# lzhangbj/ASVA

Hardware: AMD Instinct MI355X
Metric: UNet denoising steps/sec, 12x256x256 bf16, CFG on (higher is better)
Workload: dtype bf16; 1 GPU; BASELINE configs[1]: AVSync15 shape, 1 clip(s) per GPU per forward, 12x256x256 (latent 12x32x32), SD1.5-shaped AudioUNet3D 1.17B params random-init, CFG batch 2 (audio guidance 4.0), DDIM-50 schedule, step = UNet forward + guidance + scheduler update; clips_per_gpu=1, unet_batch=2, frames=12, launch=hipGraph replay, parallelism=dp1 (independent clips)

## Files before the change

### asva_amd/_lib.py

```python
from __future__ import annotations

import ctypes as C
import os

import torch

from . import precision as P

_HERE = os.path.dirname(os.path.abspath(__file__))
LIB_PATH = os.environ.get("AVSD_LIB_PATH") or os.path.join(_HERE, "libavsd_hip.so")
LIB_PATHS = {"bf16": LIB_PATH, "fp16": os.environ.get("AVSD_LIB_PATH_F16") or os.path.join(_HERE, "libavsd_hip_f16.so")}

c_void_p, c_int, c_float, c_int64 = C.c_void_p, C.c_int, C.c_float, C.c_int64


class GemmDesc(C.Structure):

    _fields_ = [
        ("A", c_void_p), ("A2", c_void_p), ("W", c_void_p), ("out", c_void_p),
        ("bias", c_void_p), ("rowvec", c_void_p), ("res1", c_void_p), ("res2", c_void_p),
        ("M", C.c_int32), ("N", C.c_int32), ("K", C.c_int32),
        ("lda", C.c_int32), ("lda2", C.c_int32), ("k_split", C.c_int32), ("ldw", C.c_int32),
        ("ldc", C.c_int32), ("ldr1", C.c_int32), ("ldr2", C.c_int32),
        ("rows_per_vec", C.c_int32), ("ldv", C.c_int32),
        ("alpha", C.c_float),
        ("mode", C.c_int32), ("flags", C.c_int32), ("batch", C.c_int32),
        ("batch_stride_a", C.c_int64), ("batch_stride_w", C.c_int64), ("batch_stride_out", C.c_int64),
        ("hw", C.c_int32), ("frames", C.c_int32), ("cseg", C.c_int32),
        ("hs", C.c_int32), ("ws", C.c_int32), ("ho", C.c_int32), ("wo", C.c_int32),
        ("cin", C.c_int32), ("stride", C.c_int32), ("ups", C.c_int32), ("pad", C.c_int32),
        ("tile", C.c_int32),
        ("split_k", C.c_int32), ("splitk_ws", c_void_p),
        ("rowstats", c_void_p), ("ln_stats", c_void_p), ("ln_colsum", c_void_p), ("ln_nblk", C.c_int32), ("ln_eps", C.c_float),
        ("out_master", c_void_p), ("ldm", C.c_int32), ("raster_g", C.c_int32),
        ("a_lo", C.c_int64), ("a2_lo", C.c_int64), ("w_lo", C.c_int64), ("out_lo", C.c_int64), ("res1_lo", C.c_int64),
        ("res2_lo", C.c_int64),
        ("stats_pos", c_void_p), ("ln_rowvec", c_void_p), ("pos_hw", C.c_int32), ("pos_frames", C.c_int32),
    ]


class XAttnDesc(C.Structure):

    _fields_ = [
        ("h", c_void_p), ("ldh", C.c_int32), ("res_f32", C.c_int32),
        ("res", c_void_p), ("ldres", C.c_int32),
        ("M", C.c_int32), ("C", C.c_int32), ("heads", C.c_int32), ("L", C.c_int32),
        ("ln_stats", c_void_p), ("ln_eps", C.c_float), ("scale", C.c_float),
        ("wq", c_void_p), ("ldwq", C.c_int32), ("lk", C.c_int32),
        ("q_colsum", c_void_p), ("q_bias", c_void_p),
        ("k", c_void_p), ("vt", c_void_p),
        ("lk_pad", C.c_int32), ("q_per_kv", C.c_int32),
        ("wo", c_void_p), ("ldwo", C.c_int32), ("ldo", C.c_int32),
        ("o_bias", c_void_p), ("out", c_void_p),
        ("out_master", c_void_p), ("ldm", C.c_int32), ("reserved0", C.c_int32),
        ("rowstats", c_void_p),
        ("stats_pos", c_void_p), ("pos_hw", C.c_int32), ("pos_frames", C.c_int32),
    ]


SIGNATURES = {
    "avsd_abi_version": (c_int, []),
    "avsd_precision": (C.c_char_p, []),
    "avsd_last_error": (C.c_char_p, []),
    "avsd_device_info": (c_int, [C.c_char_p, c_int, C.POINTER(c_int)]),
    "avsd_gemm_bf16": (c_int, [C.POINTER(GemmDesc), c_void_p]),
    "avsd_sizeof_gemm_desc": (c_int, []),
    "avsd_cross_attention_block": (c_int, [C.POINTER(XAttnDesc), c_void_p]),
    "avsd_gemm_conv3r_supported": (c_int, [c_int, c_int, c_int, c_int]),
    "avsd_gemm_conv3r2d_supported": (c_int, [c_int, c_int, c_int, c_int]),
    "avsd_cross_attention_block_supported": (c_int, [c_int, c_int, c_int]),
    "avsd_sizeof_xattn_desc": (c_int, []),
    "avsd_linear_small_m": (c_int, [c_void_p, c_void_p, c_void_p, c_void_p, c_int, c_int, c_int, c_int, c_int, c_int, c_void_p]),
    "avsd_groupnorm_stats": (c_int, [c_void_p, c_int, c_int, c_void_p, c_int, c_int, c_int, c_int, c_int, c_void_p, c_int, c_void_p]),
    "avsd_groupnorm_apply": (c_int, [c_void_p, c_int, c_int, c_void_p, c_int, c_int, c_int, c_int, c_int, c_void_p, c_void_p, c_float,
                                     c_void_p, c_int, c_int, c_void_p, c_int, c_void_p]),
    "avsd_ln_fold": (c_int, [c_void_p, c_int, c_int, c_void_p, c_void_p]),
    "avsd_groupnorm_fused_supported": (c_int, [c_int, c_int, c_int, c_int, c_int, c_int]),
    "avsd_groupnorm_fused": (c_int, [c_void_p, c_int, c_int, c_void_p, c_int, c_int, c_int, c_int, c_int, c_void_p, c_void_p, c_float,
                                     c_int, c_void_p, c_int, c_void_p]),
    "avsd_groupnorm_nchunks": (c_int, [c_int, c_int, c_int]),
    "avsd_groupnorm_scratch_floats": (c_int, [c_int, c_int, c_int, c_int]),
    "avsd_layernorm": (c_int, [c_void_p, c_int, c_void_p, c_int, c_int, c_int, c_void_p, c_void_p, c_float, c_void_p, c_int, c_int, c_void_p]),
    "avsd_softmax_rows": (c_int, [c_void_p, c_int, c_void_p, c_int, c_int, c_int, c_void_p]),
    "avsd_attention": (c_int, [c_void_p, c_int, c_void_p, c_int, c_void_p, c_int, c_void_p, c_int, c_int, c_int, c_int, c_int,
                               c_int, c_int, c_int, c_void_p, c_int, c_float, c_void_p]),
    "avsd_attention_fp8": (c_int, [c_void_p, c_int, c_void_p, c_int, c_void_p, c_int, c_void_p, c_int, c_int, c_int, c_int, c_int,
                                   c_int, c_int, c_int, c_void_p, c_int, c_float, c_float, c_float, c_float, c_void_p]),
    "avsd_temporal_attention": (c_int, [c_void_p, c_int, c_void_p, c_int, c_int, c_int, c_int, c_int, c_int, c_float, c_void_p]),
    "avsd_ncfhw_to_rows": (c_int, [c_void_p, c_void_p, c_int, c_int, c_int, c_int, c_int, c_int, c_float, c_void_p]),
    "avsd_rows_to_ncfhw": (c_int, [c_void_p, c_int, c_void_p, c_int, c_int, c_int, c_int, c_void_p]),
    "avsd_timestep_embedding": (c_int, [c_void_p, c_void_p, c_int, c_int, c_void_p]),
    "avsd_guided_step": (c_int, [c_void_p, c_int, c_float, c_float, c_void_p, c_int, c_float, C.POINTER(C.c_int32), C.POINTER(C.c_float),
                                 c_int, c_void_p, c_void_p, c_float, c_float, c_int, c_int, c_int, c_int, c_void_p]),
    "avsd_guided_multistep": (c_int, [c_void_p, c_int, c_float, c_float, c_void_p, c_int, C.POINTER(C.c_int32), C.POINTER(C.c_float),
                                      c_int, c_void_p, c_void_p, c_float, c_float, c_float, c_float, c_int, c_int, c_int, c_int, c_void_p]),
    "avsd_vae_postprocess":(c_int, [c_void_p, c_int, c_void_p, c_int, c_int, c_void_p]),
    "avsd_vae_postprocess_u8": (c_int, [c_void_p, c_int, c_void_p, c_int, c_int, c_void_p]),
    "avsd_kaldi_fbank": (c_int, [c_void_p, c_int, c_int, C.c_int64, c_void_p, c_void_p, c_int, c_int, c_int, c_int, c_float, c_int,
                                 c_void_p, c_int, c_float, c_float, c_void_p]),
    "avsd_patchify": (c_int, [c_void_p, c_void_p, c_int, c_int, c_int, c_int, c_int, c_int, c_int, c_void_p]),
    "avsd_vit_tokens": (c_int, [c_void_p, c_void_p, c_void_p, c_void_p, c_int, c_int, c_int, c_int, c_void_p]),
    "avsd_copy": (c_int, [c_void_p, c_void_p, c_int64, c_int, c_void_p]),
    "avsd_xattn_pack_kv": (c_int, [c_void_p, c_int, c_int, c_int, c_void_p, c_int, c_int, c_void_p, c_void_p, c_int, c_void_p]),
    "avsd_linear_small_m_x2": (c_int, [c_void_p, c_void_p, c_int64, c_void_p, c_void_p, c_int, c_int, c_int, c_int, c_int, c_int, c_void_p]),
    "avsd_groupnorm_stats_x2": (c_int, [c_void_p, c_int, c_int, c_int64, c_void_p, c_int, c_int, c_int64, c_int, c_int, c_int, c_void_p,
                                        c_int, c_void_p]),
    "avsd_groupnorm_apply_x2": (c_int, [c_void_p, c_int, c_int, c_int64, c_void_p, c_int, c_int, c_int64, c_int, c_int, c_int, c_void_p,
                                        c_void_p, c_float, c_void_p, c_int, c_int, c_void_p, c_int, c_int64, c_void_p]),
    "avsd_groupnorm_fused_x2": (c_int, [c_void_p, c_int, c_int, c_int64, c_void_p, c_int, c_int, c_int64, c_int, c_int, c_int, c_void_p,
                                        c_void_p, c_float, c_int, c_void_p, c_int, c_int64, c_void_p]),
    "avsd_layernorm_x2": (c_int, [c_void_p, c_int, c_int64, c_void_p, c_int, c_int64, c_int, c_int, c_void_p, c_void_p, c_float, c_void_p,
                                  c_int, c_int, c_void_p]),
    "avsd_attention_x2": (c_int, [c_void_p, c_int, c_int64, c_void_p, c_int, c_int64, c_void_p, c_int, c_int64, c_void_p, c_int, c_int64,
                                  c_int, c_int, c_int, c_int, c_int, c_int, c_int, c_void_p, c_int, c_float, c_void_p]),
    "avsd_temporal_attention_x2": (c_int, [c_void_p, c_int, c_int64, c_void_p, c_int, c_int64, c_int, c_int, c_int, c_int, c_int, c_float,
                                           c_void_p]),
    "avsd_softmax_rows_x2": (c_int, [c_void_p, c_int, c_void_p, c_int, c_int64, c_int, c_int, c_void_p]),
    "avsd_ncfhw_to_rows_x2": (c_int, [c_void_p, c_void_p, c_int64, c_int, c_int, c_int, c_int, c_int, c_int, c_float, c_void_p]),
# ... 82 lines not shown
```

### asva_amd/build.py

```python
from __future__ import annotations

import os
import subprocess
import sys
from concurrent.futures import ThreadPoolExecutor

HERE = os.path.dirname(os.path.abspath(__file__))
CSRC = os.path.join(HERE, "csrc")
OBJ = os.path.join(CSRC, "_obj")
LIB = os.path.join(HERE, "libavsd_hip.so")
VARIANTS = {"bf16": ("", LIB, []), "fp16": ("_f16", os.path.join(HERE, "libavsd_hip_f16.so"), ["-DAVSD_F16=1"])}
SOURCES = ["lib.hip", "attention.hip", "attention_x2.hip", "gemm_f32.hip", "gemm4.hip", "nstream.hip", "conv3r.hip", "norm.hip", "groupnorm_fused.hip", "elementwise.hip", "audio.hip", "xattn.hip", "attention_fp8.hip", "avsync.hip", "clip_text.hip", "imagebind_eval.hip", "plan.hip"]
GEMM_UNITS = 7
HEADERS = [os.path.join(CSRC, "avsd_common.h"), os.path.join(CSRC, "gemm_common.h"), os.path.join(CSRC, "gemm4_loops.inc"),
           os.path.join(HERE, "..", "include", "avsd.h")]
FLAGS = ["--offload-arch=gfx950", "-O3", "-std=c++17", "-fPIC", "-Wall", "-Wno-unused-function"]


PLAN_HOST = os.path.join(HERE, "plan_host")


def _hipcc() -> str:
    for cand in (os.environ.get("HIPCC"), "/opt/rocm/bin/hipcc", "hipcc"):
        if cand and (os.path.isabs(cand) and os.path.exists(cand) or not os.path.isabs(cand)):
            return cand
    raise RuntimeError("hipcc not found")


def _stale(target: str, deps: list[str]) -> bool:
    if not os.path.exists(target):
        return True
    t = os.path.getmtime(target)
    return any(os.path.getmtime(d) > t for d in deps)


def build(verbose: bool = False, force: bool = False, variants=("bf16", "fp16")) -> str:
    hipcc = _hipcc()
    jobs = []
    links = []
    for var in variants:
        suffix, lib, defs = VARIANTS[var]
        objdir = OBJ + suffix
        os.makedirs(objdir, exist_ok=True)
        objs = []
        stale = False
        for src in SOURCES:
            s = os.path.join(CSRC, src)
            o = os.path.join(objdir, src.replace(".hip", ".o"))
            objs.append(o)
            if force or _stale(o, [s] + HEADERS):
                jobs.append([hipcc, *FLAGS, *defs, "-c", s, "-o", o])
                stale = True
        gsrc = os.path.join(CSRC, "gemm.hip")
        for u in range(GEMM_UNITS):
            o = os.path.join(objdir, f"gemm_tu{u}.o")
            objs.append(o)
            if force or _stale(o, [gsrc] + HEADERS):
                jobs.insert(0, [hipcc, *FLAGS, *defs, f"-DAVSD_GEMM_TU={u}", "-c", gsrc, "-o", o])
                stale = True
        links.append((lib, objs, stale))

    def run(cmd):
        if verbose:
            print(" ".join(cmd), flush=True)
        r = subprocess.run(cmd, capture_output=True, text=True)
        if r.returncode != 0:
            raise RuntimeError(f"hipcc failed: {' '.join(cmd)}\n{r.stdout}\n{r.stderr}")
# ... 17 lines not shown
```

### asva_amd/csrc/gemm.hip

```cpp
#include "avsd_common.h"
#include "gemm_common.h"

namespace {

constexpr int LDS_STRIDE = BK + 8;

struct RowInfo {
  int64_t o0, o1, o2;
  int hb, wb;
  bool valid;
};

template <int MODE>
__device__ __forceinline__ RowInfo make_row(const avsd_gemm_desc& p, int m) {
  RowInfo r;
  r.valid = m < p.M;
  r.o0 = r.o1 = r.o2 = 0;
  r.hb = r.wb = 0;
  if (!r.valid) return r;
  if (MODE == AVSD_GEMM_PLAIN) {
    r.o0 = (int64_t)m * p.lda;
    r.o1 = (int64_t)m * p.lda2;
  } else if (MODE == AVSD_GEMM_TMIX) {
    const int f = (m / p.hw) % p.frames;
    r.o0 = (int64_t)(m - f * p.hw) * p.lda;
    r.o1 = (int64_t)(f > 0 ? m - p.hw : m) * p.lda;
    r.o2 = (int64_t)m * p.lda;
  } else {
    const int per = p.ho * p.wo;
    const int n = m / per;
    const int rem = m - n * per;
    const int oh = rem / p.wo;
    const int ow = rem - oh * p.wo;
    r.o0 = n;
    r.hb = oh * p.stride - p.pad;
    r.wb = ow * p.stride - p.pad;
  }
  return r;
}

template <int MODE>
__device__ __forceinline__ uint4 load_a(const avsd_gemm_desc& p, const h16_t* A, const h16_t* A2,
                                        const RowInfo& r, int k0) {
  uint4 z = make_uint4(0, 0, 0, 0);
  if (!r.valid || k0 >= p.K) return z;
  const h16_t* ptr;
  if (MODE == AVSD_GEMM_PLAIN) {
    ptr = (k0 < p.k_split) ? (A + r.o0 + k0) : (A2 + r.o1 + (k0 - p.k_split));
  } else if (MODE == AVSD_GEMM_TMIX) {
    const int seg = k0 / p.cseg;
    const int kk = k0 - seg * p.cseg;
    const int64_t o = r.o2 + (seg == 0 ? r.o0 - r.o2 : 0) + (seg == 1 ? r.o1 - r.o2 : 0);
// ... 160 lines not shown
  r.o0 = r.o1 = r.o2 = r.hb = r.wb = 0;
  if (!r.valid) return r;
  if (MODE == AVSD_GEMM_PLAIN) {
    r.o0 = m * p.lda;
    r.o1 = m * p.lda2;
  } else if (MODE == AVSD_GEMM_TMIX) {
    const int f = (m / p.hw) % p.frames;
    r.o0 = (m - f * p.hw) * p.lda;
    r.o1 = (f > 0 ? m - p.hw : m) * p.lda;
    r.o2 = m * p.lda;
  } else {
    const int per = p.ho * p.wo;
    const int n = m / per;
    const int rem = m - n * per;
    const int oh = rem / p.wo;
    r.o0 = n;
    r.hb = oh * p.stride - p.pad;
    r.wb = (rem - oh * p.wo) * p.stride - p.pad;
  }
  return r;
}

template <int MODE>
__device__ __forceinline__ unsigned a_voffset(const avsd_gemm_desc& p, const RowInfo32& r, int k0) {
  if (!r.valid || k0 >= p.K) return OOB;
  if (MODE == AVSD_GEMM_PLAIN) {
    return (unsigned)((k0 < p.k_split) ? (r.o0 + k0) : (r.o1 + (k0 - p.k_split))) * 2u;
  } else if (MODE == AVSD_GEMM_TMIX) {
    const int seg = k0 / p.cseg;
    const int kk = k0 - seg * p.cseg;
    const int o = r.o2 + (seg == 0 ? r.o0 - r.o2 : 0) + (seg == 1 ? r.o1 - r.o2 : 0);
    return (unsigned)(o + kk) * 2u;
  } else {
    const int tap = k0 / p.cin;
    const int c = k0 - tap * p.cin;
    const int kh = tap / 3;
    const int kw = tap - kh * 3;
    const int hi = r.hb + kh;
    const int wi = r.wb + kw;
    if (tap >= 9 || hi < 0 || hi >= (p.hs << p.ups) || wi < 0 || wi >= (p.ws << p.ups)) return OOB;
    return (unsigned)(((r.o0 * p.hs + (hi >> p.ups)) * p.ws + (wi >> p.ups)) * p.lda + c) * 2u;
  }
}

constexpr int gemm2_min_waves(int bm, int bn, int stages, bool x2, int waves) {
  const int lds = stages * (bm + bn) * 128 * (x2 ? 2 : 1);
  const int wgs = (160 * 1024) / lds < 1 ? 1 : (160 * 1024) / lds;
  const int w = (wgs * waves + 3) / 4;
  return w > 3 ? 3 : w;
}
constexpr int MODE_SUBPIX = 3;
template <int BM, int BN, int WM, int WN, int STAGES, int MODE, int LW = 0, bool X2 = false, int EX = EPI_PLAIN>
__global__ __launch_bounds__(64 * (WM * WN + LW), gemm2_min_waves(BM, BN, STAGES, X2, WM * WN + LW)) void gemm2_kernel(const avsd_gemm_desc p) {
  extern __shared__ __attribute__((aligned(1024))) unsigned char smem2[];
  constexpr int NC = WM * WN;
  constexpr int NWAVES = LW > 0 ? LW : NC;
  constexpr int A_BYTES = BM * 128;
  constexpr int W_BYTES = BN * 128;
  constexpr int PLANE_BYTES = A_BYTES + W_BYTES;
  constexpr int STAGE_BYTES = PLANE_BYTES * (X2 ? 2 : 1);
  constexpr int PA = (BM / 8) / NWAVES;
  constexpr int PW = (BN / 8) / NWAVES;
  static_assert(PA * NWAVES * 8 == BM && PW * NWAVES * 8 == BN, "tile rows must split evenly into 1-KiB pieces per wave");
  constexpr int LPT = (PA + PW) * (X2 ? 2 : 1);
  static_assert((STAGES - 2) * LPT < 64, "vmcnt is a 6-bit counter");
  constexpr int FM = BM / WM / 32;
  constexpr int FN = BN / WN / 32;

  const int tid = threadIdx.x;
  const int lane = tid & 63;
  const int wave_all = __builtin_amdgcn_readfirstlane(tid >> 6);
  const bool is_loader = LW == 0 || wave_all >= NC;
  const int wave = LW == 0 ? wave_all : (wave_all >= NC ? wave_all - NC : 0);
  const int wm = wave_all % WM;
  const int wn = (wave_all / WM) % WN;

  const int ntm = (p.M + BM - 1) / BM;
  const int ntn = (p.N + BN - 1) / BN;
  const int nwg = ntm * ntn;
  const int nsplit = p.split_k > 1 ? p.split_k : 1;
  int wg, ksplit;
  {
    const int total = nwg * nsplit;
    const int bid = blockIdx.y * gridDim.x + blockIdx.x;
    const int q = total >> 3, r = total & 7;
    const int xcd = bid & 7, idx = bid >> 3;
    const int c = (xcd < r ? xcd * (q + 1) : r * (q + 1) + (xcd - r) * q) + idx;
    wg = c / nsplit;
    ksplit = c - wg * nsplit;
  }
  int tm, tn;
  tile_of_item(wg, ntm, ntn, (p.flags & AVSD_GEMM_XCD_N) != 0, p.raster_g, tm, tn);
  const int64_t bz = blockIdx.z;
  const int nk_all = (p.K + BK - 1) / BK;
  const int per_split = (nk_all + nsplit - 1) / nsplit;
  const int kt0 = ksplit * per_split;
  const int kt1 = min(nk_all, kt0 + per_split);

  const h16_t* Ab = reinterpret_cast<const h16_t*>(p.A) + bz * p.batch_stride_a;
  const h16_t* A2b = p.A2 ? reinterpret_cast<const h16_t*>(p.A2) + bz * p.batch_stride_a : Ab;
  const h16_t* Wb = reinterpret_cast<const h16_t*>(p.W) + bz * p.batch_stride_w;
  const __amdgpu_buffer_rsrc_t rsA = __builtin_amdgcn_make_buffer_rsrc((void*)Ab, 0, 0x7fffffff, 0x00020000);
  const __amdgpu_buffer_rsrc_t rsA2 = __builtin_amdgcn_make_buffer_rsrc((void*)A2b, 0, 0x7fffffff, 0x00020000);
  const __amdgpu_buffer_rsrc_t rsW = __builtin_amdgcn_make_buffer_rsrc((void*)Wb, 0, 0x7fffffff, 0x00020000);
  const __amdgpu_buffer_rsrc_t rsAr = __builtin_amdgcn_make_buffer_rsrc((void*)(Ab + (X2 ? p.a_lo : 0)), 0, 0x7fffffff, 0x00020000);
  const __amdgpu_buffer_rsrc_t rsA2r = __builtin_amdgcn_make_buffer_rsrc((void*)(A2b + (X2 ? (p.A2 ? p.a2_lo : p.a_lo) : 0)), 0, 0x7fffffff, 0x00020000);
  const __amdgpu_buffer_rsrc_t rsWr = __builtin_amdgcn_make_buffer_rsrc((void*)(Wb + (X2 ? p.w_lo : 0)), 0, 0x7fffffff, 0x00020000);

  int ro0[PA], ro1[PA], ro2[PA], rhb[PA], rwb[PA], kca[PA];
  bool rvalid[PA];
#pragma unroll
  for (int j = 0; j < PA; ++j) {
    const int L = (wave + j * NWAVES) * 4 + (lane >> 4);
    const int x = (lane & 15) ^ (L & 15);
    const RowInfo32 r = make_row32<MODE>(p, tm * BM + 2 * L + (x >> 3));
    ro0[j] = r.o0; ro1[j] = r.o1; ro2[j] = r.o2; rhb[j] = r.hb; rwb[j] = r.wb; rvalid[j] = r.valid;
    kca[j] = (x & 7) * 8;
  }
  int wo[PW], kcw[PW];
  bool wv[PW];
#pragma unroll
  for (int j = 0; j < PW; ++j) {
    const int L = (wave + j * NWAVES) * 4 + (lane >> 4);
    const int x = (lane & 15) ^ (L & 15);
    const int n = tn * BN + 2 * L + (x >> 3);
    wv[j] = n < p.N;
    kcw[j] = (x & 7) * 8;
    wo[j] = n * p.ldw + kcw[j];
  }

  const bool fast = (MODE == AVSD_GEMM_PLAIN) || (MODE == AVSD_GEMM_TMIX && p.cseg % BK == 0) ||
                    ((MODE == AVSD_GEMM_CONV3 || MODE == MODE_SUBPIX) && p.cin % BK == 0);
  const int nk_slice = max(kt1 - kt0, 0);
  const int krot = ((p.flags & AVSD_GEMM_KROT) && nk_slice > 1 && ntm > 1) ? (int)(((long long)tm * nk_slice) / ntm) : 0;
  constexpr bool subpix = MODE == MODE_SUBPIX;
  constexpr int KS = subpix ? 2 : 3;
  const int ush = subpix ? 0 : p.ups;
  const int sub_par = subpix ? (tn * BN) / (p.N >> 2) : 0;
  const int sub_dy = sub_par >> 1, sub_dx = sub_par & 1;
  int i_kbase = 0;
  int i_c0 = 0;
  int i_kh = 0, i_kw = 0, i_seg = 0;
  bool i_second = false;
  auto seek = [&](int kbase) {
    i_kbase = kbase;
    if (MODE == AVSD_GEMM_PLAIN) {
      i_c0 = i_kbase;
      i_second = p.A2 != nullptr && i_kbase >= p.k_split;
    } else if (MODE == AVSD_GEMM_TMIX) {
      i_seg = i_kbase / p.cseg;
      i_c0 = i_kbase - i_seg * p.cseg;
    } else {
      const int tap = i_kbase / p.cin;
      i_c0 = i_kbase - tap * p.cin;
      i_kh = tap / KS;
      i_kw = tap - i_kh * KS;
    }
  };
  seek((kt0 + krot) * BK);
  const int hin = p.hs << ush, win = p.ws << ush;
  int abase[PA];
  bool aok[PA];

  auto rebase = [&]() {
#pragma unroll
    for (int j = 0; j < PA; ++j) {
      if (MODE == AVSD_GEMM_PLAIN) {
        abase[j] = (i_second ? ro1[j] - p.k_split : ro0[j]) + kca[j];
        aok[j] = rvalid[j];
      } else if (MODE == AVSD_GEMM_TMIX) {
        const int o = ro2[j] + (i_seg == 0 ? ro0[j] - ro2[j] : 0) + (i_seg == 1 ? ro1[j] - ro2[j] : 0);
        abase[j] = o + kca[j];
        aok[j] = rvalid[j] && i_seg < 3;
      } else {
        const int hi = rhb[j] + i_kh + sub_dy;
        const int wi = rwb[j] + i_kw + sub_dx;
        aok[j] = rvalid[j] && i_kh < KS && (unsigned)hi < (unsigned)hin && (unsigned)wi < (unsigned)win;
        abase[j] = ((ro0[j] * p.hs + (hi >> ush)) * p.ws + (wi >> ush)) * p.lda + kca[j];
      }
    }
  };
  rebase();

  auto issue = [&](int stage) {
    unsigned char* sb = smem2 + stage * STAGE_BYTES;
    const int kbase = i_kbase;
#pragma unroll
    for (int j = 0; j < PA; ++j) {
      unsigned vo;
      if (!fast) {
        RowInfo32 r;
        r.o0 = ro0[j]; r.o1 = ro1[j]; r.o2 = ro2[j]; r.hb = rhb[j]; r.wb = rwb[j]; r.valid = rvalid[j];
        vo = a_voffset<MODE>(p, r, kbase + kca[j]);
      } else {
        const bool ok = aok[j] && (kbase + kca[j] < p.K);
        vo = ok ? (unsigned)(abase[j] + i_c0) * 2u : OOB;
      }
      lds_ptr_t dst = (lds_ptr_t)(sb + (wave + j * NWAVES) * 1024);
      if (i_second) __builtin_amdgcn_raw_ptr_buffer_load_lds(rsA2, dst, 16, (int)vo, 0, 0, 0);
      else __builtin_amdgcn_raw_ptr_buffer_load_lds(rsA, dst, 16, (int)vo, 0, 0, 0);
      if constexpr (X2) {
        lds_ptr_t dr = (lds_ptr_t)(sb + PLANE_BYTES + (wave + j * NWAVES) * 1024);
        if (i_second) __builtin_amdgcn_raw_ptr_buffer_load_lds(rsA2r, dr, 16, (int)vo, 0, 0, 0);
        else __builtin_amdgcn_raw_ptr_buffer_load_lds(rsAr, dr, 16, (int)vo, 0, 0, 0);
      }
    }
#pragma unroll
    for (int j = 0; j < PW; ++j) {
      const unsigned vo = (wv[j] && kbase + kcw[j] < p.K) ? (unsigned)(wo[j] + kbase) * 2u : OOB;
      lds_ptr_t dst = (lds_ptr_t)(sb + A_BYTES + (wave + j * NWAVES) * 1024);
      __builtin_amdgcn_raw_ptr_buffer_load_lds(rsW, dst, 16, (int)vo, 0, 0, 0);
      if constexpr (X2) {
        lds_ptr_t dr = (lds_ptr_t)(sb + PLANE_BYTES + A_BYTES + (wave + j * NWAVES) * 1024);
        __builtin_amdgcn_raw_ptr_buffer_load_lds(rsWr, dr, 16, (int)vo, 0, 0, 0);
      }
    }
    i_kbase += BK;
    if (krot != 0 && i_kbase >= kt1 * BK) {
      seek(kt0 * BK);
      rebase();
    } else
    if (MODE == AVSD_GEMM_PLAIN) {
      i_c0 = i_kbase;
      if (!i_second && i_kbase >= p.k_split && i_kbase < p.K) { i_second = true; rebase(); }
    } else if (MODE == AVSD_GEMM_TMIX) {
      i_c0 += BK;
      if (i_c0 >= p.cseg) { i_c0 = 0; ++i_seg; rebase(); }
    } else {
      i_c0 += BK;
      if (i_c0 >= p.cin) {
        i_c0 = 0;
        if (++i_kw == KS) { i_kw = 0; ++i_kh; }
        rebase();
      }
    }
  };

  f32x16 acc[FN][FM];
#pragma unroll
  for (int a = 0; a < FN; ++a)
#pragma unroll
    for (int b = 0; b < FM; ++b)
#pragma unroll
      for (int r = 0; r < 16; ++r) acc[a][b][r] = 0.f;

  int a_line[FM], a_sw[FM], a_hi[FM];
#pragma unroll
  for (int b = 0; b < FM; ++b) {
    const int r = wm * (BM / WM) + b * 32 + (lane & 31);
    a_line[b] = (r >> 1) * 256;
    a_sw[b] = (r >> 1) & 15;
    a_hi[b] = (r & 1) << 3;
  }
  int w_line[FN], w_sw[FN], w_hi[FN];
#pragma unroll
  for (int a = 0; a < FN; ++a) {
    const int r = wn * (BN / WN) + a * 32 + (lane & 31);
    w_line[a] = (r >> 1) * 256;
    w_sw[a] = (r >> 1) & 15;
    w_hi[a] = (r & 1) << 3;
  }
  const int chalf = lane >> 5;

  const int nk = max(kt1 - kt0, 0);
  auto wait_stage = [&](int kt) {
    wait_tiles_ahead<STAGES - 2, LPT>(nk - 1 - kt);
  };
  if (is_loader) {
#pragma unroll
    for (int s = 0; s < STAGES - 1; ++s)
      if (s < nk) issue(s);
  }
  float pre_ln[2 * FM] = {};
  const bool pre = (p.flags & AVSD_GEMM_LNFUSE) != 0 && !(LW > 0 && is_loader);
  if (pre) {
#pragma unroll
    for (int b = 0; b < FM; ++b) {
      const int m = tm * BM + wm * (BM / WM) + b * 32 + (lane & 31);
      pre_ln[2 * b] = 1.f; pre_ln[2 * b + 1] = 0.f;
      if (m < p.M) ln_row_stats(p, m, bz, pre_ln[2 * b], pre_ln[2 * b + 1]);
    }
  }
  if (LW > 0 && is_loader) {
    for (int kt = 0; kt < nk; ++kt) {
      wait_stage(kt);
      __builtin_amdgcn_s_barrier();
      if (kt + STAGES - 1 < nk) issue((kt + STAGES - 1) % STAGES);
    }
    return;
  }

  for (int kt = 0; kt < nk; ++kt) {
    if (LW == 0) wait_stage(kt);
    __builtin_amdgcn_s_barrier();
    if (LW == 0 && kt + STAGES - 1 < nk) issue((kt + STAGES - 1) % STAGES);

    const unsigned char* sA = smem2 + (kt % STAGES) * STAGE_BYTES;
    const unsigned char* sW = sA + A_BYTES;
#pragma unroll
    for (int ks = 0; ks < BK / 16; ++ks) {
      const int c = ks * 2 + chalf;
      h16x8 xf[FM], wf[FN];
#pragma unroll
      for (int b = 0; b < FM; ++b)
        xf[b] = *reinterpret_cast<const h16x8*>(sA + a_line[b] + (((a_hi[b] | c) ^ a_sw[b]) << 4));
#pragma unroll
      for (int a = 0; a < FN; ++a)
        wf[a] = *reinterpret_cast<const h16x8*>(sW + w_line[a] + (((w_hi[a] | c) ^ w_sw[a]) << 4));
      if constexpr (X2) {
        h16x8 xr[FM], wr[FN];
#pragma unroll
        for (int b = 0; b < FM; ++b)
          xr[b] = *reinterpret_cast<const h16x8*>(sA + PLANE_BYTES + a_line[b] + (((a_hi[b] | c) ^ a_sw[b]) << 4));
#pragma unroll
        for (int a = 0; a < FN; ++a)
          wr[a] = *reinterpret_cast<const h16x8*>(sW + PLANE_BYTES + w_line[a] + (((w_hi[a] | c) ^ w_sw[a]) << 4));
        __builtin_amdgcn_s_setprio(1);
#pragma unroll
        for (int a = 0; a < FN; ++a)
#pragma unroll
          for (int b = 0; b < FM; ++b) {
            acc[a][b] = mfma32x32x16(wr[a], xf[b], acc[a][b], 0, 0, 0);
            acc[a][b] = mfma32x32x16(wf[a], xr[b], acc[a][b], 0, 0, 0);
            acc[a][b] = mfma32x32x16(wf[a], xf[b], acc[a][b], 0, 0, 0);
          }
        __builtin_amdgcn_s_setprio(0);
      } else {
      __builtin_amdgcn_s_setprio(1);
#pragma unroll
      for (int a = 0; a < FN; ++a)
#pragma unroll
        for (int b = 0; b < FM; ++b)
          acc[a][b] = mfma32x32x16(wf[a], xf[b], acc[a][b], 0, 0, 0);
      __builtin_amdgcn_s_setprio(0);
      }
    }
  }

  if (p.split_k > 1) {
    float* ws = p.splitk_ws + (int64_t)ksplit * p.M * p.N;
    const int hsel = (lane >> 5) * 4;
#pragma unroll
    for (int b = 0; b < FM; ++b) {
      const int m = tm * BM + wm * (BM / WM) + b * 32 + (lane & 31);
      if (m >= p.M) continue;
#pragma unroll
      for (int a = 0; a < FN; ++a)
#pragma unroll
        for (int q = 0; q < 4; ++q) {
          const int n = tn * BN + wn * (BN / WN) + a * 32 + 8 * q + hsel;
          if (n < p.N)
            *reinterpret_cast<float4*>(ws + (int64_t)m * p.N + n) =
                make_float4(acc[a][b][4 * q], acc[a][b][4 * q + 1], acc[a][b][4 * q + 2], acc[a][b][4 * q + 3]);
        }
    }
    if (p.split_k != 0x7fffffff) return;
#pragma unroll
    for (int a = 0; a < FN; ++a)
#pragma unroll
      for (int b = 0; b < FM; ++b)
#pragma unroll
        for (int r = 0; r < 16; ++r) acc[a][b][r] = 0.f;
    for (int sl = 0; sl < nsplit; ++sl) {
      const float* slab = p.splitk_ws + (int64_t)sl * p.M * p.N;
#pragma unroll
      for (int b = 0; b < FM; ++b) {
        const int m = min(tm * BM + wm * (BM / WM) + b * 32 + (lane & 31), p.M - 1);
#pragma unroll
        for (int a = 0; a < FN; ++a)
#pragma unroll
          for (int q = 0; q < 4; ++q) {
            const int n = min(tn * BN + wn * (BN / WN) + a * 32 + 8 * q + hsel, p.N - 4);
            const float4 v = *reinterpret_cast<const float4*>(slab + (int64_t)m * p.N + n);
            acc[a][b][4 * q] += v.x; acc[a][b][4 * q + 1] += v.y; acc[a][b][4 * q + 2] += v.z; acc[a][b][4 * q + 3] += v.w;
          }
      }
    }
  }
  if constexpr (subpix) {
    if constexpr (X2) epilogue_x2<FN, FM, true>(p, acc, tm * BM + wm * (BM / WM), tn * BN + wn * (BN / WN), lane, bz, pre_ln, pre);
    else epilogue_each<FN, FM, (64 * (WM * WN + LW) > 512), EPI_SHUF>(p, acc, tm * BM + wm * (BM / WM), tn * BN + wn * (BN / WN), lane, bz, pre_ln, pre);
  } else if constexpr (X2) epilogue_x2<FN, FM>(p, acc, tm * BM + wm * (BM / WM), tn * BN + wn * (BN / WN), lane, bz, pre_ln, pre);
  else if constexpr (EX == EPI_REST) {
    if constexpr (FN * FM >= 10) epilogue_each<FN, FM, (64 * (WM * WN + LW) > 512), EPI_REST>(p, acc, tm * BM + wm * (BM / WM), tn * BN + wn * (BN / WN), lane, bz, pre_ln, pre);
    else epilogue<FN, FM, (64 * (WM * WN + LW) > 512), EPI_REST>(p, acc, tm * BM + wm * (BM / WM), tn * BN + wn * (BN / WN), lane, bz, pre_ln, pre);
  } else if constexpr (FN * FM >= 10)
    epilogue_each<FN, FM, (64 * (WM * WN + LW) > 512)>(p, acc, tm * BM + wm * (BM / WM), tn * BN + wn * (BN / WN), lane, bz, pre_ln, pre);
  else epilogue<FN, FM, (64 * (WM * WN + LW) > 512)>(p, acc, tm * BM + wm * (BM / WM), tn * BN + wn * (BN / WN), lane, bz, pre_ln, pre);
}

template <int S, bool EXTRA = false>
__global__ __launch_bounds__(256) void splitk_reduce_kernel(const avsd_gemm_desc p) {
  const int nq = p.N / 4;
  const int64_t total = (int64_t)p.M * nq;
  const h16_t* R1 = reinterpret_cast<const h16_t*>(p.res1);
  const h16_t* R2 = reinterpret_cast<const h16_t*>(p.res2);
  const bool x2 = (p.flags & AVSD_GEMM_X2) != 0;
  const bool out_rest = EXTRA && (p.flags & AVSD_GEMM_OUT_REST) != 0;
  for (int64_t i = blockIdx.x * (int64_t)blockDim.x + threadIdx.x; i < total; i += (int64_t)gridDim.x * blockDim.x) {
    const int m = (int)(i / nq);
    const int n = (int)(i - (int64_t)m * nq) * 4;
    float4 acc = make_float4(0.f, 0.f, 0.f, 0.f);
    float4 pre_bias = make_float4(0.f, 0.f, 0.f, 0.f), pre_vec = pre_bias, pre_r1f = pre_bias, pre_r2f = pre_bias;
    uint2 pre_r1 = make_uint2(0, 0), pre_r1lo = pre_r1, pre_r2 = pre_r1, pre_r2lo = pre_r1;
    if (p.bias) pre_bias = *reinterpret_cast<const float4*>(p.bias + n);
    if (p.rowvec) pre_vec = *reinterpret_cast<const float4*>(p.rowvec + (int64_t)(m / p.rows_per_vec) * p.ldv + n);
    if (R1) {
      if (p.flags & AVSD_GEMM_RES1_F32) {
        pre_r1f = *reinterpret_cast<const float4*>(reinterpret_cast<const float*>(p.res1) + (int64_t)m * p.ldr1 + n);
      } else {
        pre_r1 = *reinterpret_cast<const uint2*>(R1 + (int64_t)m * p.ldr1 + n);
        if (x2) pre_r1lo = *reinterpret_cast<const uint2*>(R1 + p.res1_lo + (int64_t)m * p.ldr1 + n);
      }
    }
    if (R2) {
      if (p.flags & AVSD_GEMM_RES2_F32) {
        pre_r2f = *reinterpret_cast<const float4*>(reinterpret_cast<const float*>(p.res2) + (int64_t)m * p.ldr2 + n);
      } else {
        pre_r2 = *reinterpret_cast<const uint2*>(R2 + (int64_t)m * p.ldr2 + n);
        if (x2) pre_r2lo = *reinterpret_cast<const uint2*>(R2 + p.res2_lo + (int64_t)m * p.ldr2 + n);
      }
    }
    if constexpr (S > 0) {
      float4 sv[S];
#pragma unroll
      for (int s = 0; s < S; ++s) sv[s] = *reinterpret_cast<const float4*>(p.splitk_ws + ((int64_t)s * p.M + m) * p.N + n);
#pragma unroll
      for (int s = 0; s < S; ++s) { acc.x += sv[s].x; acc.y += sv[s].y; acc.z += sv[s].z; acc.w += sv[s].w; }
    } else {
      for (int s = 0; s < p.split_k; ++s) {
        const float4 v = *reinterpret_cast<const float4*>(p.splitk_ws + ((int64_t)s * p.M + m) * p.N + n);
        acc.x += v.x; acc.y += v.y; acc.z += v.z; acc.w += v.w;
      }
    }
    float v[4] = {p.alpha * acc.x, p.alpha * acc.y, p.alpha * acc.z, p.alpha * acc.w};
    if (p.flags & AVSD_GEMM_LNFUSE) {
      const float2* st = reinterpret_cast<const float2*>(p.ln_stats) + (int64_t)m * p.ln_nblk;
      float sm = 0.f, sq = 0.f;
      for (int j = 0; j < p.ln_nblk; ++j) { const float2 t = st[j]; sm += t.x; sq += t.y; }
      const float inv_k = 1.0f / (float)p.K;
      const float mean = sm * inv_k;
// ... 65 lines not shown
          sm += __shfl_xor(sm, off, 64);
          sq += __shfl_xor(sq, off, 64);
        }
        if ((threadIdx.x & 7) == 0)
          reinterpret_cast<float2*>(p.rowstats)[(int64_t)m * (p.N >> 5) + (n >> 5)] = make_float2(sm, sq);
      }
    }
  }
}

template <int BM, int BN, int WM, int WN, int STAGES, int MODE, int LW = 0, bool X2 = false, int EX = EPI_PLAIN>
int launch2(const avsd_gemm_desc& d, hipStream_t s) {
  constexpr size_t lds = (size_t)STAGES * (BM + BN) * 128 * (X2 ? 2 : 1);
  static_assert(lds <= 160 * 1024, "tile does not fit the 160 KB of LDS");
  if (MODE == MODE_SUBPIX && (d.N / 4) % BN != 0) {
    avsd_set_error("gemm/conv3: ups = 2 needs whole column tiles per output-pixel parity: cout (%d) %% %d != 0 for this tile", d.N / 4, BN);
    return AVSD_EINVAL;
  }
  static bool attr_set = false;
  if (!attr_set) {
    hipError_t e = hipFuncSetAttribute(reinterpret_cast<const void*>(&gemm2_kernel<BM, BN, WM, WN, STAGES, MODE, LW, X2, EX>),
                                       hipFuncAttributeMaxDynamicSharedMemorySize, (int)lds);
    if (e != hipSuccess) {
      avsd_set_error("gemm2: hipFuncSetAttribute(%zu B LDS): %s", lds, hipGetErrorString(e));
      return AVSD_ELAUNCH;
    }
    attr_set = true;
  }
  const int ntm = (d.M + BM - 1) / BM, ntn = (d.N + BN - 1) / BN;
  const int nsplit = d.split_k > 1 ? d.split_k : 1;
  dim3 grid((unsigned)(ntm * ntn), (unsigned)nsplit, (unsigned)d.batch);
  hipLaunchKernelGGL((gemm2_kernel<BM, BN, WM, WN, STAGES, MODE, LW, X2, EX>), grid, dim3(64 * (WM * WN + LW)), lds, s, d);
  AVSD_CHECK_LAUNCH("gemm2 launch");
  if (nsplit > 1) {
    const int64_t total = (int64_t)d.M * (d.N / 4);
    int64_t g = (total + 255) / 256;
    if (g > 2048) g = 2048;
    if (MODE == MODE_SUBPIX || (d.flags & AVSD_GEMM_OUT_REST)) {
      hipLaunchKernelGGL((splitk_reduce_kernel<0, true>), dim3((unsigned)g), dim3(256), 0, s, d);
    } else
    switch (nsplit) {
      case 2: hipLaunchKernelGGL(splitk_reduce_kernel<2>, dim3((unsigned)g), dim3(256), 0, s, d); break;
      case 4: hipLaunchKernelGGL(splitk_reduce_kernel<4>, dim3((unsigned)g), dim3(256), 0, s, d); break;
      case 8: hipLaunchKernelGGL(splitk_reduce_kernel<8>, dim3((unsigned)g), dim3(256), 0, s, d); break;
      case 3: hipLaunchKernelGGL(splitk_reduce_kernel<3>, dim3((unsigned)g), dim3(256), 0, s, d); break;
      case 5: hipLaunchKernelGGL(splitk_reduce_kernel<5>, dim3((unsigned)g), dim3(256), 0, s, d); break;
      default: hipLaunchKernelGGL(splitk_reduce_kernel<0>, dim3((unsigned)g), dim3(256), 0, s, d); break;
    }
    AVSD_CHECK_LAUNCH("gemm split-K reduce launch");
  }
  return AVSD_OK;
}

template <int MODE, int EX = EPI_PLAIN>
int dispatch_tile(const avsd_gemm_desc& d, int tile, hipStream_t s) {
  switch (tile) {
    case 1: return launch<128, 128, MODE, EX>(d, s);
    case 2: return launch<128, 64, MODE, EX>(d, s);
    case 3: return launch<64, 64, MODE, EX>(d, s);
    case 4: return launch2<128, 64, 2, 2, 3, MODE, 0, false, EX>(d, s);
    case 6: return launch2<128, 128, 2, 4, 3, MODE, 0, false, EX>(d, s);
    case 7: return launch2<64, 64, 2, 2, 4, MODE, 0, false, EX>(d, s);
    case 9: return launch2<256, 128, 4, 2, 3, MODE, 0, false, EX>(d, s);
    case 11: return launch2<128, 128, 2, 2, 2, MODE, 0, false, EX>(d, s);
    case 12: return launch2<128, 64, 2, 2, 2, MODE, 0, false, EX>(d, s);
    case 13: return launch2<64, 64, 2, 2, 2, MODE, 0, false, EX>(d, s);
    case 14: return launch2<256, 128, 4, 2, 2, MODE, 0, false, EX>(d, s);
    case 17: return launch2<128, 320, 4, 2, 2, MODE, 0, false, EX>(d, s);
    case 19: return launch2<256, 320, 4, 2, 2, MODE, 0, false, EX>(d, s);
    case 20: return launch2<256, 128, 4, 2, 3, MODE, 4, false, EX>(d, s);
    case 24: return launch2<128, 64, 2, 2, 3, MODE, 2, false, EX>(d, s);
    case 25: return launch2<64, 64, 2, 2, 4, MODE, 2, false, EX>(d, s);
    case 30: return launch2<128, 128, 2, 4, 4, MODE, 0, false, EX>(d, s);
    case 31: return launch2<128, 256, 2, 4, 3, MODE, 0, false, EX>(d, s);
    case AVSD_GEMM_TILE_256x160_8W: return launch2<256, 160, 8, 1, 3, MODE, 4, false, EX>(d, s);
    default:
      avsd_set_error("gemm: tile id %d is not built (gemm.hip dispatch_tile)", tile);
      return AVSD_EINVAL;
  }
}

template <int MODE>
int dispatch_tile_x2(const avsd_gemm_desc& d, int tile, hipStream_t s) {
  switch (tile) {
    case 7: return launch2<64, 64, 2, 2, 4, MODE, 0, true>(d, s);
    case 11: return launch2<128, 128, 2, 2, 2, MODE, 0, true>(d, s);
    case 13: return launch2<64, 64, 2, 2, 2, MODE, 0, true>(d, s);
    case 24: return launch2<128, 64, 2, 2, 3, MODE, 2, true>(d, s);
    case 25: return launch2<64, 64, 2, 2, 4, MODE, 2, true>(d, s);
    case 34: return launch2<128, 160, 4, 1, 2, MODE, 0, true>(d, s);
    case 35: return launch2<256, 64, 4, 2, 2, MODE, 0, true>(d, s);
    case 36: return launch2<128, 192, 2, 2, 2, MODE, 0, true>(d, s);
    default:
      avsd_set_error("gemm: AVSD_GEMM_X2 runs on tiles 7, 11, 13, 24, 25, 34, 35, 36 (got %d)", tile);
      return AVSD_EINVAL;
  }
}

int pick_tile(int M, int N, int batch) {
  static int num_cu = 0;
  if (num_cu == 0) {
    hipDeviceProp_t prop;
    int dev = 0;
    if (hipGetDevice(&dev) == hipSuccess && hipGetDeviceProperties(&prop, dev) == hipSuccess)
      num_cu = prop.multiProcessorCount;
    if (num_cu <= 0) num_cu = 256;
  }
  const int bm[3] = {128, 128, 64}, bn[3] = {128, 64, 64};
  const double eff[3] = {1.0, 0.85, 0.62};
  const int slots[3] = {2 * num_cu, 3 * num_cu, 4 * num_cu};
  int best = 3;
  double best_cost = 1e300;
  for (int t = 0; t < 3; ++t) {
    const long blocks = (long)((M + bm[t] - 1) / bm[t]) * ((N + bn[t] - 1) / bn[t]) * batch;
    const long waves = (blocks + slots[t] - 1) / slots[t];
    const double cost = (double)waves * bm[t] * bn[t] / eff[t] * slots[t];
    if (cost < best_cost) { best_cost = cost; best = t + 1; }
  }
  return best;
}

}

int avsd_gemm_dispatch_plain(const avsd_gemm_desc& d, int tile, hipStream_t s);
int avsd_gemm_dispatch_tmix(const avsd_gemm_desc& d, int tile, hipStream_t s);
int avsd_gemm_dispatch_conv3(const avsd_gemm_desc& d, int tile, hipStream_t s);
#ifdef AVSD_F16
#define AVSD_DISPATCH_TILE(MODE) ((d.flags & AVSD_GEMM_OUT_REST) ? dispatch_tile<MODE, EPI_REST>(d, tile, s) : dispatch_tile<MODE>(d, tile, s))
#else
#define AVSD_DISPATCH_TILE(MODE) dispatch_tile<MODE>(d, tile, s)
#endif
#if !defined(AVSD_GEMM_TU) || AVSD_GEMM_TU == 0
int avsd_gemm_dispatch_plain(const avsd_gemm_desc& d, int tile, hipStream_t s) { return AVSD_DISPATCH_TILE(AVSD_GEMM_PLAIN); }
#endif
#if !defined(AVSD_GEMM_TU) || AVSD_GEMM_TU == 1
int avsd_gemm_dispatch_tmix(const avsd_gemm_desc& d, int tile, hipStream_t s) { return AVSD_DISPATCH_TILE(AVSD_GEMM_TMIX); }
#endif
#if !defined(AVSD_GEMM_TU) || AVSD_GEMM_TU == 2
int avsd_gemm_dispatch_conv3(const avsd_gemm_desc& d, int tile, hipStream_t s) { return AVSD_DISPATCH_TILE(AVSD_GEMM_CONV3); }
#endif
int avsd_gemm_dispatch_subpix(const avsd_gemm_desc& d, int tile, hipStream_t s);
int avsd_gemm_dispatch_x2_subpix(const avsd_gemm_desc& d, int tile, hipStream_t s);
#if !defined(AVSD_GEMM_TU) || AVSD_GEMM_TU == 6
int avsd_gemm_dispatch_subpix(const avsd_gemm_desc& d, int tile, hipStream_t s) {
  switch (tile) {
    case 4: return launch2<128, 64, 2, 2, 3, MODE_SUBPIX>(d, s);
    case 6: return launch2<128, 128, 2, 4, 3, MODE_SUBPIX>(d, s);
    case 9: return launch2<256, 128, 4, 2, 3, MODE_SUBPIX>(d, s);
    case 11: return launch2<128, 128, 2, 2, 2, MODE_SUBPIX>(d, s);
    case 13: return launch2<64, 64, 2, 2, 2, MODE_SUBPIX>(d, s);
    case 17: return launch2<128, 320, 4, 2, 2, MODE_SUBPIX>(d, s);
    case 20: return launch2<256, 128, 4, 2, 3, MODE_SUBPIX, 4>(d, s);
    case 24: return launch2<128, 64, 2, 2, 3, MODE_SUBPIX, 2>(d, s);
    case 25: return launch2<64, 64, 2, 2, 4, MODE_SUBPIX, 2>(d, s);
    case 30: return launch2<128, 128, 2, 4, 4, MODE_SUBPIX>(d, s);
    case AVSD_GEMM_TILE_256x160_8W: return launch2<256, 160, 8, 1, 3, MODE_SUBPIX, 4>(d, s);
    default:
      avsd_set_error("gemm/conv3: ups = 2 runs on tiles 4, 6, 9, 11, 13, 17, 20, 24, 25, 30, 38 (got %d)", tile);
      return AVSD_EINVAL;
  }
}
int avsd_gemm_dispatch_x2_subpix(const avsd_gemm_desc& d, int tile, hipStream_t s) {
  switch (tile) {
    case 7: return launch2<64, 64, 2, 2, 4, MODE_SUBPIX, 0, true>(d, s);
    case 11: return launch2<128, 128, 2, 2, 2, MODE_SUBPIX, 0, true>(d, s);
    case 13: return launch2<64, 64, 2, 2, 2, MODE_SUBPIX, 0, true>(d, s);
    case 24: return launch2<128, 64, 2, 2, 3, MODE_SUBPIX, 2, true>(d, s);
    case 25: return launch2<64, 64, 2, 2, 4, MODE_SUBPIX, 2, true>(d, s);
    case 34: return launch2<128, 160, 4, 1, 2, MODE_SUBPIX, 0, true>(d, s);
    case 35: return launch2<256, 64, 4, 2, 2, MODE_SUBPIX, 0, true>(d, s);
    default:
      avsd_set_error("gemm/conv3: ups = 2 with AVSD_GEMM_X2 runs on tiles 7, 11, 13, 24, 25, 34, 35 (got %d)", tile);
      return AVSD_EINVAL;
  }
}
#endif

int avsd_gemm_dispatch_x2_plain(const avsd_gemm_desc& d, int tile, hipStream_t s);
int avsd_gemm_dispatch_x2_tmix(const avsd_gemm_desc& d, int tile, hipStream_t s);
int avsd_gemm_dispatch_x2_conv3(const avsd_gemm_desc& d, int tile, hipStream_t s);
#if !defined(AVSD_GEMM_TU) || AVSD_GEMM_TU == 4
int avsd_gemm_dispatch_x2_plain(const avsd_gemm_desc& d, int tile, hipStream_t s) { return dispatch_tile_x2<AVSD_GEMM_PLAIN>(d, tile, s); }
int avsd_gemm_dispatch_x2_tmix(const avsd_gemm_desc& d, int tile, hipStream_t s) { return dispatch_tile_x2<AVSD_GEMM_TMIX>(d, tile, s); }
#endif
#if !defined(AVSD_GEMM_TU) || AVSD_GEMM_TU == 5
int avsd_gemm_dispatch_x2_conv3(const avsd_gemm_desc& d, int tile, hipStream_t s) { return dispatch_tile_x2<AVSD_GEMM_CONV3>(d, tile, s); }
#endif

#if !defined(AVSD_GEMM_TU) || AVSD_GEMM_TU == 3
int avsd_gemm_dispatch_conv3r(const avsd_gemm_desc& d, hipStream_t s);
int avsd_gemm_dispatch_asm(const avsd_gemm_desc& d, hipStream_t s);
int avsd_gemm_dispatch_nstream(const avsd_gemm_desc& d, hipStream_t s);

int avsd_gemm_splitk_reduce(const avsd_gemm_desc& d, hipStream_t s) {
  const int64_t total = (int64_t)d.M * (d.N / 4);
  int64_t g = (total + 255) / 256;
  if (g > 2048) g = 2048;
  if (d.flags & AVSD_GEMM_OUT_REST) {
    hipLaunchKernelGGL((splitk_reduce_kernel<0, true>), dim3((unsigned)g), dim3(256), 0, s, d);
  } else
  switch (d.split_k) {
    case 2: hipLaunchKernelGGL(splitk_reduce_kernel<2>, dim3((unsigned)g), dim3(256), 0, s, d); break;
    case 4: hipLaunchKernelGGL(splitk_reduce_kernel<4>, dim3((unsigned)g), dim3(256), 0, s, d); break;
    case 8: hipLaunchKernelGGL(splitk_reduce_kernel<8>, dim3((unsigned)g), dim3(256), 0, s, d); break;
    case 3: hipLaunchKernelGGL(splitk_reduce_kernel<3>, dim3((unsigned)g), dim3(256), 0, s, d); break;
    case 5: hipLaunchKernelGGL(splitk_reduce_kernel<5>, dim3((unsigned)g), dim3(256), 0, s, d); break;
    case 10: hipLaunchKernelGGL(splitk_reduce_kernel<10>, dim3((unsigned)g), dim3(256), 0, s, d); break;
    default: hipLaunchKernelGGL(splitk_reduce_kernel<0>, dim3((unsigned)g), dim3(256), 0, s, d); break;
  }
  AVSD_CHECK_LAUNCH("gemm split-K reduce launch");
  return AVSD_OK;
}

extern "C" int avsd_gemm_bf16(const avsd_gemm_desc* dp, void* stream) {
  AVSD_REQUIRE(dp != nullptr, "gemm: null descriptor");
  avsd_gemm_desc d = *dp;
  AVSD_REQUIRE(d.A && d.W && d.out, "gemm: A, W and out must be non-null");
  AVSD_REQUIRE(d.M > 0 && d.N > 0 && d.K > 0, "gemm: M,N,K must be positive (got %d,%d,%d)", d.M, d.N, d.K);
  AVSD_REQUIRE(!(d.flags & AVSD_GEMM_W_FRAG) || d.tile == AVSD_GEMM_TILE_NSTREAM, "gemm: fragment-ordered W (AVSD_GEMM_W_FRAG) is read by tile %d only (got %d)", AVSD_GEMM_TILE_NSTREAM, d.tile);
  if (d.flags & AVSD_GEMM_W_FRAG) d.ldw = d.K;
  AVSD_REQUIRE(d.K % 8 == 0 && d.ldw % 8 == 0 && d.ldw >= d.K, "gemm: K (%d) and ldw (%d) must be multiples of 8, ldw >= K", d.K, d.ldw);
  AVSD_REQUIRE(d.N % 4 == 0 && d.ldc % 4 == 0, "gemm: N (%d) and ldc (%d) must be multiples of 4", d.N, d.ldc);
  AVSD_REQUIRE(d.lda % 8 == 0, "gemm: lda (%d) must be a multiple of 8", d.lda);
  if (d.batch <= 0) d.batch = 1;
  AVSD_REQUIRE(d.raster_g >= 0 && d.raster_g <= 64, "gemm: raster_g (%d) must be 0 (library default) .. 64", d.raster_g);
  if (d.flags & AVSD_GEMM_GEGLU) AVSD_REQUIRE(d.N % 32 == 0, "gemm: GEGLU needs N %% 32 == 0 (got %d)", d.N);
  AVSD_REQUIRE(!((d.flags & AVSD_GEMM_GEGLU) && (d.flags & AVSD_GEMM_GELU)), "gemm: GEGLU and GELU are exclusive");
  if (d.flags & AVSD_GEMM_ROWSTATS) {
    AVSD_REQUIRE(d.rowstats, "gemm: ROWSTATS without a rowstats buffer");
    AVSD_REQUIRE(!(d.flags & (AVSD_GEMM_GEGLU | AVSD_GEMM_OUT_F32)) && d.N % 32 == 0 && d.ldc % 8 == 0 &&
                     (!d.res1 || d.ldr1 % 8 == 0) && (!d.res2 || d.ldr2 % 8 == 0),
                 "gemm: ROWSTATS needs bf16 output, N %% 32 == 0 and 16-byte-aligned rows");
  }
  if (d.flags & AVSD_GEMM_LNFUSE) {
    AVSD_REQUIRE(d.ln_stats && d.ln_colsum && d.ln_nblk > 0 && d.mode == AVSD_GEMM_PLAIN && !d.A2,
                 "gemm: LNFUSE needs ln_stats, ln_colsum, ln_nblk and a single-source PLAIN operand");
    AVSD_REQUIRE(d.ln_nblk * 32 == d.K || d.ln_nblk == 1, "gemm: LNFUSE statistics are K / 32 pairs per row or one pre-folded pair (got %d for K = %d)", d.ln_nblk, d.K);
    AVSD_REQUIRE(d.batch == 1 || d.batch_stride_a % d.lda == 0, "gemm: LNFUSE batch stride must be whole rows");
  }
  if (d.stats_pos || d.ln_rowvec) {
    AVSD_REQUIRE(d.pos_hw > 0 && d.pos_frames > 0 && d.batch == 1 && !(d.flags & AVSD_GEMM_X2),
                 "gemm: stats_pos / ln_rowvec need pos_hw > 0, pos_frames > 0, batch 1 and no AVSD_GEMM_X2 (got hw %d, frames %d)", d.pos_hw, d.pos_frames);
    AVSD_REQUIRE(!d.stats_pos || (d.flags & AVSD_GEMM_ROWSTATS), "gemm: stats_pos without AVSD_GEMM_ROWSTATS");
    AVSD_REQUIRE(!d.ln_rowvec || (d.flags & AVSD_GEMM_LNFUSE), "gemm: ln_rowvec without AVSD_GEMM_LNFUSE");
  }
  if (d.res1) AVSD_REQUIRE(d.ldr1 % 4 == 0, "gemm: ldr1 must be a multiple of 4");
  if (d.res2) AVSD_REQUIRE(d.ldr2 % 4 == 0, "gemm: ldr2 must be a multiple of 4");
  if (d.out_master) AVSD_REQUIRE(d.ldm % 4 == 0 && d.ldm >= ((d.mode == AVSD_GEMM_CONV3 && d.ups == 2) ? d.N / 4 : d.N) && !(d.flags & AVSD_GEMM_GEGLU),
                                 "gemm: out_master needs ldm %% 4 == 0, ldm >= N (ups = 2: cout) and no GEGLU");
  if (d.rowvec) AVSD_REQUIRE(d.rows_per_vec > 0 && d.ldv % 4 == 0, "gemm: rowvec needs rows_per_vec > 0 and ldv %% 4 == 0");
  if (d.flags & AVSD_GEMM_OUT_REST) {
#ifndef AVSD_F16
    AVSD_REQUIRE(d.mode == AVSD_GEMM_CONV3 && d.ups == 2,
                 "gemm: OUT_REST is compiled into the IEEE-half build only (libavsd_hip_f16.so: the per-layer precision plan is fp16 storage)");
#endif
    AVSD_REQUIRE(!(d.flags & (AVSD_GEMM_X2 | AVSD_GEMM_OUT_F32 | AVSD_GEMM_GEGLU)) && d.out_lo != 0 && (d.out_lo & 7) == 0 && d.batch == 1 &&
                     d.tile != AVSD_GEMM_TILE_NSTREAM && !(d.tile >= AVSD_GEMM_TILE_CONV3R_FIRST && d.tile <= AVSD_GEMM_TILE_CONV3R2D_LAST),
                 "gemm: OUT_REST is for one-pass 16-bit outputs (no X2 / OUT_F32 / GEGLU / batch, not on tiles 40..54 / 70) and needs out_lo %% 8 == 0, != 0");
  }
  if (d.mode == AVSD_GEMM_PLAIN) {
    if (!d.A2) d.k_split = d.K;
    AVSD_REQUIRE(d.k_split % 8 == 0 && d.k_split <= d.K, "gemm: k_split (%d) must be a multiple of 8 and <= K", d.k_split);
    if (d.A2) AVSD_REQUIRE(d.lda2 % 8 == 0, "gemm: lda2 must be a multiple of 8");
  } else if (d.mode == AVSD_GEMM_TMIX) {
    AVSD_REQUIRE(d.cseg > 0 && d.cseg % 8 == 0 && d.K == 3 * d.cseg, "gemm/tmix: K (%d) must equal 3*cseg (%d)", d.K, d.cseg);
    AVSD_REQUIRE(d.hw > 0 && d.frames > 0 && d.M % (d.hw * d.frames) == 0, "gemm/tmix: M (%d) must be a multiple of frames*hw (%d*%d)", d.M, d.frames, d.hw);
  } else if (d.mode == AVSD_GEMM_CONV3) {
    AVSD_REQUIRE(d.stride == 1 || d.stride == 2, "gemm/conv3: stride must be 1 or 2");
    if (d.ups == 2) {
      AVSD_REQUIRE(d.cin > 0 && d.cin % 64 == 0 && d.K == 4 * d.cin, "gemm/conv3: ups = 2 needs K (%d) == 4*cin (%d), cin %% 64 == 0", d.K, d.cin);
      AVSD_REQUIRE(d.stride == 1 && d.pad == 1 && d.hs > 0 && d.ws > 0 && d.ho == d.hs && d.wo == d.ws && d.M % (d.hs * d.ws) == 0,
                   "gemm/conv3: ups = 2 needs stride 1, pad 1, (ho, wo) = (hs, ws) and whole images");
      AVSD_REQUIRE(d.N % 4 == 0 && (d.N / 4) % 64 == 0 && d.ldc >= d.N / 4, "gemm/conv3: ups = 2 needs N = 4 * cout, cout %% 64 == 0, ldc >= cout");
      AVSD_REQUIRE(!d.A2 && !d.res1 && !d.res2 && !d.rowvec && !(d.flags & (AVSD_GEMM_GEGLU | AVSD_GEMM_GELU | AVSD_GEMM_ROWSTATS | AVSD_GEMM_LNFUSE)) && d.batch == 1,
                   "gemm/conv3: ups = 2 takes bias / out_master / the rest plane only");
      AVSD_REQUIRE((double)d.M * 4.0 * d.ldc < 2147483648.0, "gemm/conv3: ups = 2 output too large");
      AVSD_REQUIRE(d.tile >= 4 && !(d.tile >= AVSD_GEMM_TILE_CONV3R_FIRST && d.tile <= AVSD_GEMM_TILE_CONV3R2D_LAST) && !(d.tile >= AVSD_GEMM_TILE_ASM_FIRST),
                   "gemm/conv3: ups = 2 runs on the LDS-direct tiles (4..38), got %d", d.tile);
    } else {
    AVSD_REQUIRE(d.cin > 0 && d.cin % 8 == 0 && d.K == 9 * d.cin, "gemm/conv3: K (%d) must equal 9*cin (%d), cin %% 8 == 0", d.K, d.cin);
    AVSD_REQUIRE(d.ups == 0 || d.ups == 1, "gemm/conv3: ups must be 0, 1 or 2");
    AVSD_REQUIRE(d.pad == 0 || d.pad == 1, "gemm/conv3: pad must be 0 or 1");
    AVSD_REQUIRE(d.hs > 0 && d.ws > 0 && d.ho > 0 && d.wo > 0 && d.M % (d.ho * d.wo) == 0, "gemm/conv3: bad image geometry");
    const int hin = d.hs << d.ups, win = d.ws << d.ups;
    AVSD_REQUIRE(d.ho == (hin + 2 - 3) / d.stride + 1 && d.wo == (win + 2 - 3) / d.stride + 1, "gemm/conv3: (ho,wo)=(%d,%d) inconsistent with input (%d,%d) stride %d", d.ho, d.wo, hin, win, d.stride);
    }
  } else {
    AVSD_REQUIRE(false, "gemm: unknown mode %d", d.mode);
  }
  if ((d.tile >= AVSD_GEMM_TILE_CONV3R_FIRST && d.tile <= AVSD_GEMM_TILE_CONV3R_LAST) ||
      (d.tile >= AVSD_GEMM_TILE_CONV3R2D_FIRST && d.tile <= AVSD_GEMM_TILE_CONV3R2D_LAST)) {
    if (d.split_k > 1) AVSD_REQUIRE(d.splitk_ws != nullptr, "gemm: split_k needs a workspace");
    return avsd_gemm_dispatch_conv3r(d, reinterpret_cast<hipStream_t>(stream));
  }
  AVSD_REQUIRE(d.mode == AVSD_GEMM_PLAIN || !d.A2, "gemm: a two-source A needs the PLAIN mode or a resident convolution tile (40..54), got mode %d tile %d", d.mode, d.tile);
  if (d.tile == AVSD_GEMM_TILE_NSTREAM) return avsd_gemm_dispatch_nstream(d, reinterpret_cast<hipStream_t>(stream));
  const bool asm_tile = d.tile >= AVSD_GEMM_TILE_ASM_FIRST && d.tile <= AVSD_GEMM_TILE_ASM_LAST;
  if (asm_tile && !(d.flags & AVSD_GEMM_X2)) return avsd_gemm_dispatch_asm(d, reinterpret_cast<hipStream_t>(stream));
  if (d.split_k > 1 && !asm_tile) {
    AVSD_REQUIRE(d.splitk_ws != nullptr, "gemm: split_k needs a workspace");
    AVSD_REQUIRE(!(d.flags & AVSD_GEMM_GEGLU) && d.batch == 1, "gemm: split_k cannot be combined with GEGLU or batching");
    AVSD_REQUIRE((d.tile >= 4 && d.tile <= ((d.flags & AVSD_GEMM_X2) ? AVSD_GEMM_MAX_TILE_X2 : AVSD_GEMM_MAX_TILE)) ||
                     (!(d.flags & AVSD_GEMM_X2) && d.tile == AVSD_GEMM_TILE_256x160_8W),
                 "gemm: split_k needs an LDS-direct tile (4..33; split precision: ..36), got %d", d.tile);
    AVSD_REQUIRE(d.split_k <= (d.K + 63) / 64, "gemm: split_k (%d) exceeds the number of K tiles", d.split_k);
  }
  if (d.flags & AVSD_GEMM_X2) {
    AVSD_REQUIRE(d.a_lo != 0 && d.w_lo != 0 && (!d.A2 || d.a2_lo != 0), "gemm/x2: A, A2 and W need their rest-plane offsets");
    AVSD_REQUIRE((d.flags & AVSD_GEMM_OUT_F32) || d.out_lo != 0, "gemm/x2: a 16-bit output needs out_lo");
    AVSD_REQUIRE(!d.res1 || (d.flags & AVSD_GEMM_RES1_F32) || d.res1_lo != 0, "gemm/x2: a 16-bit res1 needs res1_lo");
    AVSD_REQUIRE(!d.res2 || (d.flags & AVSD_GEMM_RES2_F32) || d.res2_lo != 0, "gemm/x2: a 16-bit res2 needs res2_lo");
    AVSD_REQUIRE(((d.a_lo | d.a2_lo | d.w_lo | d.out_lo | d.res1_lo | d.res2_lo) & 7) == 0, "gemm/x2: plane offsets must be multiples of 8 elements");
    AVSD_REQUIRE(d.mode != AVSD_GEMM_PLAIN || !d.A2 || d.k_split % 64 == 0, "gemm/x2: a two-source A needs k_split %% 64 == 0 (got %d)", d.k_split);
    const double a_rows = d.mode == AVSD_GEMM_CONV3 ? (double)(d.M / (d.ho * d.wo)) * d.hs * d.ws : (double)d.M;
    AVSD_REQUIRE(a_rows * d.lda * 2.0 < 2147483648.0 && (double)d.N * d.ldw * 2.0 < 2147483648.0, "gemm/x2: operands must be < 2 GiB per plane");
    hipStream_t sx = reinterpret_cast<hipStream_t>(stream);
    if (asm_tile) return avsd_gemm_dispatch_asm(d, sx);
    switch (d.mode) {
      case AVSD_GEMM_PLAIN: return avsd_gemm_dispatch_x2_plain(d, d.tile, sx);
      case AVSD_GEMM_TMIX: return avsd_gemm_dispatch_x2_tmix(d, d.tile, sx);
      default: return d.ups == 2 ? avsd_gemm_dispatch_x2_subpix(d, d.tile, sx) : avsd_gemm_dispatch_x2_conv3(d, d.tile, sx);
    }
  }
  int tile = d.tile;
  {
    const double a_rows = d.mode == AVSD_GEMM_CONV3 ? (double)(d.M / (d.ho * d.wo)) * d.hs * d.ws : (double)d.M;
    const bool big = a_rows * d.lda * 2.0 >= 2147483648.0 || (double)d.N * d.ldw * 2.0 >= 2147483648.0 ||
                     (d.A2 && (double)d.M * d.lda2 * 2.0 >= 2147483648.0);
    AVSD_REQUIRE(!(big && d.mode == AVSD_GEMM_CONV3 && d.ups == 2), "gemm/conv3: ups = 2 needs operands < 2 GiB");
    if (big && (tile < 1 || tile > 3)) tile = (d.N > 64 && d.M > 2048) ? 1 : 3;
    if (d.mode == AVSD_GEMM_PLAIN && d.A2 && d.k_split % 64 != 0 && (tile < 1 || tile > 3)) {
      AVSD_REQUIRE(d.split_k <= 1, "gemm: split_k with a two-source A needs k_split %% 64 == 0 (got %d)", d.k_split);
      tile = (d.N > 64 && d.M > 2048) ? 2 : 3;
    }
  }
  if (tile < 1 || (tile > AVSD_GEMM_MAX_TILE && tile != AVSD_GEMM_TILE_256x160_8W)) tile = pick_tile(d.M, (d.flags & AVSD_GEMM_GEGLU) ? d.N : d.N, d.batch);
  hipStream_t s = reinterpret_cast<hipStream_t>(stream);
  switch (d.mode) {
    case AVSD_GEMM_PLAIN: return avsd_gemm_dispatch_plain(d, tile, s);
    case AVSD_GEMM_TMIX: return avsd_gemm_dispatch_tmix(d, tile, s);
    default: return d.ups == 2 ? avsd_gemm_dispatch_subpix(d, tile, s) : avsd_gemm_dispatch_conv3(d, tile, s);
  }
}
#endif
```

### asva_amd/csrc/gemm4.hip

```cpp
#include <utility>

#include "gemm_common.h"

int avsd_gemm_splitk_reduce(const avsd_gemm_desc& d, hipStream_t s);

namespace {

typedef unsigned u32x4 __attribute__((ext_vector_type(4)));

constexpr int ROWB = 144;

#ifdef AVSD_F16
#define AVSD_MFMA_OP "v_mfma_f32_32x32x16_f16"
#else
#define AVSD_MFMA_OP "v_mfma_f32_32x32x16_bf16"
#endif

#include "gemm4_loops.inc"

__device__ __forceinline__ f32x16 from_agpr(const f32x16& a) {
  f32x16 v;
#pragma unroll
  for (int r = 0; r < 16; ++r) {
    float f;
    asm("v_accvgpr_read_b32 %0, %1" : "=v"(f) : "a"(a[r]));
    v[r] = f;
  }
  return v;
}

template <int FM, int FN, int MODE, bool X2 = false, int NS = 2, int EX = EPI_PLAIN>
__global__ __launch_bounds__(256, 1) void gemm4_kernel(const avsd_gemm_desc p) {
  extern __shared__ __attribute__((aligned(1024))) unsigned char smem4[];
  constexpr int BM = 64 * FM, BN = 64 * FN;
  constexpr int A_BYTES = BM * ROWB;
  static_assert(MODE == AVSD_GEMM_PLAIN || MODE == AVSD_GEMM_TMIX, "gemm4: PLAIN or TMIX operands");
  constexpr int NA = BM / 32;
  constexpr int STAGE = (BM + BN) * ROWB * (X2 ? 2 : 1);

  const int tid = threadIdx.x;
  const int lane = tid & 63;
  const int wave = __builtin_amdgcn_readfirstlane(tid >> 6);
  const int wm = wave & 1, wn = wave >> 1;

  const int ntm = (p.M + BM - 1) / BM;
  const int ntn = (p.N + BN - 1) / BN;
  const int nwg = ntm * ntn;
  const int nsplit = p.split_k > 1 ? p.split_k : 1;
  int wg, ksplit;
  {
    const int total = nwg * nsplit;
    const int bid = blockIdx.y * gridDim.x + blockIdx.x;
    const int q = total >> 3, r = total & 7;
    const int xcd = bid & 7, idx = bid >> 3;
    const int c = (xcd < r ? xcd * (q + 1) : r * (q + 1) + (xcd - r) * q) + idx;
    wg = c / nsplit;
    ksplit = c - wg * nsplit;
  }
  int tm, tn;
  tile_of_item(wg, ntm, ntn, (p.flags & AVSD_GEMM_XCD_N) != 0, p.raster_g, tm, tn);
  const int nk_all = p.K / BK;
  const int per_split = (nk_all + nsplit - 1) / nsplit;
  const int kt0 = ksplit * per_split;
  const int nk = max(min(nk_all, kt0 + per_split) - kt0, 0);

  const unsigned long long pa = (unsigned long long)p.A, pw = (unsigned long long)p.W;
  const u32x4 rsA = {(unsigned)pa, (unsigned)(pa >> 32) & 0xffffu, (unsigned)p.M * (unsigned)p.lda * 2u, 0x00020000u};
  const u32x4 rsW = {(unsigned)pw, (unsigned)(pw >> 32) & 0xffffu, (unsigned)p.N * (unsigned)p.ldw * 2u, 0x00020000u};
  const unsigned long long par = pa + (X2 ? (unsigned long long)p.a_lo * 2ull : 0ull), pwr = pw + (X2 ? (unsigned long long)p.w_lo * 2ull : 0ull);
  const u32x4 rsAr = {(unsigned)par, (unsigned)(par >> 32) & 0xffffu, rsA[2], 0x00020000u};
  const u32x4 rsWr = {(unsigned)pwr, (unsigned)(pwr >> 32) & 0xffffu, rsW[2], 0x00020000u};

  using Loop = G4Loop<FM, FN, NS, MODE == AVSD_GEMM_TMIX, X2>;
  const int kst = (Loop::rot && (p.flags & AVSD_GEMM_KROT) && nk > 1 && ntm > 1) ? (int)(((long long)tm * nk) / ntm) : 0;
  const int kfirst = kt0 + kst;
  const int srow = tid >> 3, sch = tid & 7;
  G4Args ga;
  ga.va0 = (unsigned)((tm * BM + srow) * p.lda + kfirst * BK + sch * 8) * 2u;
  ga.vw0 = (unsigned)((tn * BN + srow) * p.ldw + kfirst * BK + sch * 8) * 2u;
  ga.wr0 = (unsigned)(srow * ROWB + sch * 16);
  ga.rda0 = (unsigned)((wm * 32 * FM + (lane & 31)) * ROWB + (lane >> 5) * 16);
  ga.rdw0 = (unsigned)(A_BYTES + (wn * 32 * FN + (lane & 31)) * ROWB + (lane >> 5) * 16);
  ga.rsA = rsA; ga.rsW = rsW; ga.rsAr = rsAr; ga.rsWr = rsWr;
  ga.kst = (unsigned)kst; ga.winc = 128u - 128u * (unsigned)nk;
  ga.sa = 32u * (unsigned)p.lda * 2u; ga.sw = 32u * (unsigned)p.ldw * 2u;
  ga.nk = (unsigned)nk; ga.kt0 = (unsigned)kt0; ga.tps = 0u; ga.tps2 = 0u;

  const bool ln_pre = (p.flags & AVSD_GEMM_LNFUSE) != 0 && p.ln_nblk == 1;
  float2 ln_raw[FM];
#pragma unroll
  for (int b = 0; b < FM; ++b) {
    ln_raw[b] = make_float2(0.f, 0.f);
    const int m = tm * BM + wm * 32 * FM + b * 32 + (lane & 31);
    if (ln_pre && m < p.M) ln_raw[b] = reinterpret_cast<const float2*>(p.ln_stats)[m];
  }

  f32x16 acc[FN][FM];
  if constexpr (MODE == AVSD_GEMM_TMIX) {
    const int tps = p.cseg / BK;
    const int seg0 = min(kfirst / tps, 2), col0 = (kfirst - seg0 * tps) * BK;
    const int ke = kt0 + nk - 1;
    const int seg_e = min(max(ke, 0) / tps, 2), col_e = (ke - seg_e * tps) * BK;
    const int seg_s = min(kt0 / tps, 2), col_s = (kt0 - seg_s * tps) * BK;
    unsigned* tbl = reinterpret_cast<unsigned*>(smem4 + STAGE) + tid * (4 * NA);
#pragma unroll
// ... 10 lines not shown
        dw = (unsigned)(o[seg_s] + col_s - o[seg_e] - col_e - BK) * 2u;
      }
      tbl[i] = v; tbl[NA + i] = d01; tbl[2 * NA + i] = d12; tbl[3 * NA + i] = dw;
    }
    ga.va0 = (unsigned)(STAGE + tid * (4 * NA) * 4);
    ga.tps = (unsigned)tps; ga.tps2 = 2u * (unsigned)tps;
  }
  Loop::run(acc, ga);

  const int m_base = tm * BM + wm * 32 * FM, n_base = tn * BN + wn * 32 * FN;
  if (p.split_k > 1) {
    float* ws = p.splitk_ws + (int64_t)ksplit * p.M * p.N;
    const int hsel = (lane >> 5) * 4;
#pragma unroll
    for (int b = 0; b < FM; ++b) {
      const int m = m_base + b * 32 + (lane & 31);
      if (m >= p.M) continue;
#pragma unroll
      for (int a = 0; a < FN; ++a) {
        const f32x16 v = from_agpr(acc[a][b]);
#pragma unroll
        for (int q = 0; q < 4; ++q) {
          const int n = n_base + a * 32 + 8 * q + hsel;
          if (n < p.N)
            *reinterpret_cast<float4*>(ws + (int64_t)m * p.N + n) = make_float4(v[4 * q], v[4 * q + 1], v[4 * q + 2], v[4 * q + 3]);
        }
      }
    }
    return;
  }
  static_for<FM>([&p, &acc, &ln_raw, ln_pre, m_base, n_base, lane](auto b_c) {
    constexpr int B = decltype(b_c)::value;
    __builtin_amdgcn_sched_barrier(0);
    f32x16 band[FN][1];
#pragma unroll
    for (int a = 0; a < FN; ++a) band[a][0] = from_agpr(acc[a][B]);
    float pre_ln[2] = {1.f, 0.f};
    if (ln_pre) {
      float sm = ln_raw[B].x, sq = ln_raw[B].y;
      asm volatile("" : "+v"(sm), "+v"(sq));
      const float inv_k = 1.0f / (float)p.K;
      const float mean = sm * inv_k;
      const float var = fmaxf(sq * inv_k - mean * mean, 0.f);
      pre_ln[0] = rsqrtf(var + p.ln_eps);
      pre_ln[1] = mean * pre_ln[0];
    }
    if constexpr (X2) epilogue_x2<FN, 1>(p, band, m_base + 32 * B, n_base, lane, 0, pre_ln, ln_pre);
    else if constexpr (FN == 5) epilogue_by_term<FN, 1, EX>(p, band, m_base + 32 * B, n_base, lane, 0, pre_ln, ln_pre);
    else epilogue<FN, 1, false, EX>(p, band, m_base + 32 * B, n_base, lane, 0, pre_ln, ln_pre);
  });
}

template <int FM, int FN, int MODE, bool X2 = false, int NS = 2, int EX = EPI_PLAIN>
int launch4_ex(const avsd_gemm_desc& d, hipStream_t s) {
  constexpr int BM = 64 * FM, BN = 64 * FN;
  constexpr size_t lds = (size_t)2 * (BM + BN) * ROWB * (X2 ? 2 : 1);
  static_assert(lds <= 160 * 1024, "tile does not fit the 160 KB of LDS");
  static bool attr_set = false;
  if (!attr_set) {
    hipError_t e = hipFuncSetAttribute(reinterpret_cast<const void*>(&gemm4_kernel<FM, FN, MODE, X2, NS, EX>), hipFuncAttributeMaxDynamicSharedMemorySize, (int)lds);
    if (e != hipSuccess) {
      avsd_set_error("gemm4: hipFuncSetAttribute(%zu B LDS): %s", lds, hipGetErrorString(e));
      return AVSD_ELAUNCH;
    }
    attr_set = true;
  }
  const int ntm = (d.M + BM - 1) / BM, ntn = (d.N + BN - 1) / BN;
  const int nsplit = d.split_k > 1 ? d.split_k : 1;
  dim3 grid((unsigned)(ntm * ntn), (unsigned)nsplit, 1);
  hipLaunchKernelGGL((gemm4_kernel<FM, FN, MODE, X2, NS, EX>), grid, dim3(256), lds, s, d);
  AVSD_CHECK_LAUNCH("gemm4 launch");
  if (nsplit > 1) return avsd_gemm_splitk_reduce(d, s);
  return AVSD_OK;
}
template <int FM, int FN, int MODE, bool X2 = false, int NS = 2>
int launch4(const avsd_gemm_desc& d, hipStream_t s) {
#ifdef AVSD_F16
  if constexpr (!X2) {
    if (d.flags & AVSD_GEMM_OUT_REST) return launch4_ex<FM, FN, MODE, X2, NS, EPI_REST>(d, s);
  }
#endif
  return launch4_ex<FM, FN, MODE, X2, NS>(d, s);
}

}

int avsd_gemm_dispatch_asm(const avsd_gemm_desc& d, hipStream_t s) {
  AVSD_REQUIRE((d.mode == AVSD_GEMM_PLAIN || d.mode == AVSD_GEMM_TMIX) && !d.A2 && d.batch == 1 && d.K % 64 == 0,
               "gemm/asm tiles: PLAIN single-source or TMIX operands with K %% 64 == 0 (got mode %d, K %d)", d.mode, d.K);
  AVSD_REQUIRE((double)d.M * d.lda * 2.0 < 1073741824.0 && (double)d.N * d.ldw * 2.0 < 1073741824.0, "gemm/asm tiles: operands must be < 1 GiB");
  AVSD_REQUIRE(d.split_k <= 1 || (d.splitk_ws && d.split_k <= d.K / 64 && !(d.flags & AVSD_GEMM_GEGLU)), "gemm/asm tiles: bad split_k %d", d.split_k);
  if (d.split_k > 1) {
    const int nk_all = d.K / 64, per = (nk_all + d.split_k - 1) / d.split_k;
    AVSD_REQUIRE((d.split_k - 1) * per < nk_all, "gemm/asm tiles: split_k %d leaves an empty slice of the %d K tiles", d.split_k, nk_all);
  }
  const int k = d.tile - AVSD_GEMM_TILE_ASM_FIRST;
  const bool tmix = d.mode == AVSD_GEMM_TMIX;
  if (tmix) AVSD_REQUIRE(d.cseg % 64 == 0 && !(d.flags & AVSD_GEMM_LNFUSE), "gemm/asm tiles: TMIX needs cseg %% 64 == 0 (got %d)", d.cseg);
  if (d.flags & AVSD_GEMM_X2) {
    switch (k) {
      case 3: return tmix ? launch4<2, 2, AVSD_GEMM_TMIX, true>(d, s) : launch4<2, 2, AVSD_GEMM_PLAIN, true>(d, s);
      case 4: return tmix ? launch4<2, 1, AVSD_GEMM_TMIX, true>(d, s) : launch4<2, 1, AVSD_GEMM_PLAIN, true>(d, s);
      case 5: return tmix ? launch4<1, 2, AVSD_GEMM_TMIX, true>(d, s) : launch4<1, 2, AVSD_GEMM_PLAIN, true>(d, s);
      case 6: return tmix ? launch4<1, 1, AVSD_GEMM_TMIX, true>(d, s) : launch4<1, 1, AVSD_GEMM_PLAIN, true>(d, s);
      default: AVSD_REQUIRE(false, "gemm/asm tiles: tile %d has no split-precision form (63..66 do)", d.tile);
    }
  }
  if (tmix) {
    switch (k) {
      case 1: return launch4<4, 2, AVSD_GEMM_TMIX>(d, s);
      case 2: return launch4<2, 4, AVSD_GEMM_TMIX>(d, s);
      case 3: return launch4<2, 2, AVSD_GEMM_TMIX>(d, s);
      case 4: return launch4<2, 1, AVSD_GEMM_TMIX>(d, s);
      case 5: return launch4<1, 2, AVSD_GEMM_TMIX>(d, s);
      case 6: return launch4<1, 1, AVSD_GEMM_TMIX>(d, s);
      case 7: return launch4<2, 5, AVSD_GEMM_TMIX>(d, s);
      default: AVSD_REQUIRE(false, "gemm/asm tiles: tile %d has no TMIX form (61..67 do)", d.tile);
    }
  }
  switch (k) {
    case 0: return launch4<4, 4, AVSD_GEMM_PLAIN>(d, s);
    case 1: return launch4<4, 2, AVSD_GEMM_PLAIN>(d, s);
    case 2: return launch4<2, 4, AVSD_GEMM_PLAIN>(d, s);
    case 3: return launch4<2, 2, AVSD_GEMM_PLAIN>(d, s);
    case 4: return launch4<2, 1, AVSD_GEMM_PLAIN>(d, s);
    case 5: return launch4<1, 2, AVSD_GEMM_PLAIN>(d, s);
    case 6: return launch4<1, 1, AVSD_GEMM_PLAIN>(d, s);
    case 7: return launch4<2, 5, AVSD_GEMM_PLAIN>(d, s);
    default: AVSD_REQUIRE(false, "gemm/asm tiles: unknown tile %d", d.tile);
  }
}
```

### asva_amd/csrc/gemm_common.h

```cpp
#pragma once
#include <utility>

#include "avsd_common.h"

namespace {

constexpr int BK = 64;

template <class F, int... I>
__device__ __forceinline__ void static_for_impl(F&& f, std::integer_sequence<int, I...>) {
  (f(std::integral_constant<int, I>{}), ...);
}
template <int N, class F>
__device__ __forceinline__ void static_for(F&& f) {
  static_for_impl(f, std::make_integer_sequence<int, N>{});
}

__device__ __forceinline__ void ln_row_stats(const avsd_gemm_desc& p, int m, int64_t bz, float& rstd, float& mr) {
  const float2* st = reinterpret_cast<const float2*>(p.ln_stats) + ((int64_t)bz * (p.batch_stride_a / p.lda) + m) * p.ln_nblk;
  float sm = 0.f, sq = 0.f;
  int j = 0;
  for (; j + 10 <= p.ln_nblk; j += 10) {
    float2 t[10];
#pragma unroll
    for (int u = 0; u < 10; ++u) t[u] = st[j + u];
#pragma unroll
    for (int u = 0; u < 10; ++u) { sm += t[u].x; sq += t[u].y; }
  }
  for (; j < p.ln_nblk; ++j) {
    const float2 t = st[j];
    sm += t.x;
    sq += t.y;
  }
  const float inv_k = 1.0f / (float)p.K;
  const float mean = sm * inv_k;
  const float var = fmaxf(sq * inv_k - mean * mean, 0.f);
  rstd = rsqrtf(var + p.ln_eps);
  mr = mean * rstd;
}

__device__ __forceinline__ const float* pos_row(const avsd_gemm_desc& p, const float* table, int m) {
  return table + (int64_t)((m / p.pos_hw) % p.pos_frames) * p.N;
}

__device__ __forceinline__ void rowstats16(const unsigned (&w8)[8], const float* pos16, float& sm, float& sq) {
  float pv[16];
#pragma unroll
  for (int i = 0; i < 16; ++i) pv[i] = 0.f;
  if (pos16) {
#pragma unroll
    for (int j = 0; j < 4; ++j) {
      const float4 t = *reinterpret_cast<const float4*>(pos16 + 4 * j);
      pv[4 * j] = t.x; pv[4 * j + 1] = t.y; pv[4 * j + 2] = t.z; pv[4 * j + 3] = t.w;
    }
  }
  sm = 0.f;
// ... 652 lines not shown
#pragma unroll
        for (int q = 0; q < 2; ++q) {
          float v[4], gate[4];
          head(a, q, nb + 8 * q + hsel, v);
          head(a, q + 2, nb + 8 * q + hsel + 16, gate);
#pragma unroll
          for (int i = 0; i < 4; ++i) v[i] *= gelu_erf_f(gate[i]);
          const int64_t o = orow + (nb >> 1) + hsel + 8 * q;
          float sm = 0.f, sq = 0.f;
          if (out_f32) *reinterpret_cast<float4*>(reinterpret_cast<float*>(p.out) + o) = make_float4(v[0], v[1], v[2], v[3]);
          else store4(o, v, sm, sq);
        }
      }
    }
  }
}

template <int N>
__device__ __forceinline__ void wait_vmcnt() {
  static_assert(N >= 0 && N < 64, "vmcnt is a 6-bit counter");
  __builtin_amdgcn_s_waitcnt((N & 15) | ((N >> 4) << 14) | (7 << 4) | (15 << 8));
  asm volatile("" ::: "memory");
}

template <int MAXA, int LPT>
__device__ __forceinline__ void wait_tiles_ahead(int ahead) {
  if constexpr (MAXA <= 0) {
    wait_vmcnt<0>();
  } else {
    if (ahead >= MAXA) wait_vmcnt<MAXA * LPT>();
    else wait_tiles_ahead<MAXA - 1, LPT>(ahead);
  }
}

typedef __attribute__((address_space(3))) void* lds_ptr_t;

__device__ __forceinline__ void tile_of_item(int wg, int ntm, int ntn, bool nmaj, int g_override, int& tm, int& tn) {
  const int nmajor = nmaj ? ntn : ntm, nminor = nmaj ? ntm : ntn;
  int tmaj, tmin;
  if (nminor >= 16 && nmajor >= 8) {
    const int G = g_override > 0 ? g_override : 8;
    const int gsize = G * nminor, grp = wg / gsize, first = grp * G, in = wg - grp * gsize;
    const int gm = min(nmajor - first, G);
    tmaj = first + in % gm;
    tmin = in / gm;
  } else {
    tmaj = wg / nminor;
    tmin = wg - tmaj * nminor;
  }
  tn = nmaj ? tmaj : tmin;
  tm = nmaj ? tmin : tmaj;
}


__device__ __forceinline__ void piece_row_chunk(int piece, int lane, int& row, int& kchunk) {
  const int L = piece * 4 + (lane >> 4);
  const int x = (lane & 15) ^ (L & 15);
  row = 2 * L + (x >> 3);
  kchunk = (x & 7) * 8;
}
__device__ __forceinline__ int frag_offset(int r, int c) {
  return (r >> 1) * 256 + ((((r & 1) << 3) | c) ^ ((r >> 1) & 15)) * 16;
}

}
```

### asva_amd/csrc/plan.hip

```cpp
#include "avsd_common.h"

#include <stdio.h>
#include <string.h>

#include <string>
#include <type_traits>
#include <utility>
#include <vector>

namespace {

struct RArg {
  int64_t i = 0;
  double f = 0.0;
  void* p = nullptr;
};

template <class T>
T conv(const RArg& a) {
  if constexpr (std::is_pointer_v<T>) return reinterpret_cast<T>(a.p);
  else if constexpr (std::is_floating_point_v<T>) return static_cast<T>(a.f);
  else return static_cast<T>(a.i);
}
template <class... A, size_t... I>
int call_impl(int (*fn)(A...), const RArg* a, std::index_sequence<I...>) {
  return fn(conv<A>(a[I])...);
}
template <class... A>
int call(int (*fn)(A...), const RArg* a, int n, const char* name) {
  if (n != (int)sizeof...(A)) {
    avsd_set_error("plan: %s recorded with %d arguments, this library takes %d", name, n, (int)sizeof...(A));
    return AVSD_EINVAL;
  }
  return call_impl(fn, a, std::index_sequence_for<A...>{});
}

typedef int (*thunk_t)(const RArg*, int);
struct Entry {
  const char* name;
  thunk_t thunk;
  size_t desc_bytes;
};
#define AVSD_PLAN_ENTRY(fn) {#fn, [](const RArg* a, int n) { return call(&fn, a, n, #fn); }, 0}
#define AVSD_PLAN_ENTRY_DESC(fn, T) {#fn, [](const RArg* a, int n) { return call(&fn, a, n, #fn); }, sizeof(T)}
const Entry kEntries[] = {
    AVSD_PLAN_ENTRY_DESC(avsd_gemm_bf16, avsd_gemm_desc), AVSD_PLAN_ENTRY_DESC(avsd_cross_attention_block, avsd_xattn_desc), AVSD_PLAN_ENTRY(avsd_linear_small_m),
    AVSD_PLAN_ENTRY(avsd_groupnorm_stats),  AVSD_PLAN_ENTRY(avsd_groupnorm_apply),       AVSD_PLAN_ENTRY(avsd_layernorm),
    AVSD_PLAN_ENTRY(avsd_softmax_rows),     AVSD_PLAN_ENTRY(avsd_attention),             AVSD_PLAN_ENTRY(avsd_attention_fp8),
    AVSD_PLAN_ENTRY(avsd_temporal_attention), AVSD_PLAN_ENTRY(avsd_ncfhw_to_rows),       AVSD_PLAN_ENTRY(avsd_rows_to_ncfhw),
    AVSD_PLAN_ENTRY(avsd_timestep_embedding), AVSD_PLAN_ENTRY(avsd_guided_step),         AVSD_PLAN_ENTRY(avsd_vae_postprocess),
    AVSD_PLAN_ENTRY(avsd_vae_postprocess_u8), AVSD_PLAN_ENTRY(avsd_kaldi_fbank),         AVSD_PLAN_ENTRY(avsd_patchify),
    AVSD_PLAN_ENTRY(avsd_vit_tokens),       AVSD_PLAN_ENTRY(avsd_copy),                  AVSD_PLAN_ENTRY(avsd_xattn_pack_kv),
    AVSD_PLAN_ENTRY(avsd_linear_small_m_x2), AVSD_PLAN_ENTRY(avsd_groupnorm_stats_x2),   AVSD_PLAN_ENTRY(avsd_groupnorm_apply_x2),
    AVSD_PLAN_ENTRY(avsd_layernorm_x2),     AVSD_PLAN_ENTRY(avsd_attention_x2),          AVSD_PLAN_ENTRY(avsd_temporal_attention_x2),
    AVSD_PLAN_ENTRY(avsd_ncfhw_to_rows_x2), AVSD_PLAN_ENTRY(avsd_split_f32),             AVSD_PLAN_ENTRY(avsd_vae_postprocess_x2),
    AVSD_PLAN_ENTRY(avsd_vae_postprocess_u8_x2), AVSD_PLAN_ENTRY(avsd_softmax_rows_x2),
    AVSD_PLAN_ENTRY(avsd_groupnorm_fused),  AVSD_PLAN_ENTRY(avsd_groupnorm_fused_x2),
    AVSD_PLAN_ENTRY(avsd_ln_fold),          AVSD_PLAN_ENTRY(avsd_guided_multistep),
    AVSD_PLAN_ENTRY(avsd_convnd_f32),       AVSD_PLAN_ENTRY(avsd_maxpool_hw_f32),        AVSD_PLAN_ENTRY(avsd_mean_rows_f32),
    AVSD_PLAN_ENTRY(avsd_resize_aa_normalize_f32),
    AVSD_PLAN_ENTRY(avsd_convnd_ld_f32),    AVSD_PLAN_ENTRY(avsd_pool3_hw_f32),
    AVSD_PLAN_ENTRY(avsd_embed_tokens_f32), AVSD_PLAN_ENTRY(avsd_layernorm_f32),         AVSD_PLAN_ENTRY(avsd_attention_causal_f32),
    AVSD_PLAN_ENTRY(avsd_quick_gelu_f32),
    AVSD_PLAN_ENTRY(avsd_attention_f32),    AVSD_PLAN_ENTRY(avsd_gelu_f32),              AVSD_PLAN_ENTRY(avsd_vit_tokens_f32),
    AVSD_PLAN_ENTRY(avsd_cosine_rows_f32),   AVSD_PLAN_ENTRY(avsd_normalize_rows_f32),
};

struct Reloc {
  uint32_t field_off;
  int32_t buf;
  int64_t off;
};
struct Arg {
  uint8_t tag = 0;
  int64_t i = 0;
  double f = 0.0;
  int32_t buf = -1;
  int64_t off = 0;
  std::vector<unsigned char> blob;
  std::vector<Reloc> relocs;
};
struct Call {
  thunk_t thunk = nullptr;
  std::string fn;
  std::vector<Arg> args;
  std::vector<RArg> resolved;
};
struct Buffer {
  int64_t bytes = 0;
  void* ptr = nullptr;
};
struct Region {
  std::string name;
  int32_t buf = -1;
  int64_t off = 0, bytes = 0;
  int kind = 0;
};
struct Plan {
  std::string name;
// ... 94 lines not shown

static int plan_bundle_load_impl(const char* path, avsd_plan_bundle** out) {
  AVSD_REQUIRE(path && out, "plan_bundle_load: null argument");
  *out = nullptr;
  FILE* f = fopen(path, "rb");
  AVSD_REQUIRE(f != nullptr, "plan_bundle_load: cannot open %s", path);
  Reader rd{f};
  char magic[8];
  rd.raw(magic, 8);
  const uint32_t abi = rd.get<uint32_t>();
  char prec[8];
  rd.raw(prec, 8);
  prec[7] = 0;
  struct Guard {
    FILE* f; avsd_plan_bundle* b;
    ~Guard() { if (f) fclose(f); delete b; }
  } guard{f, new avsd_plan_bundle()};
  avsd_plan_bundle* b = guard.b;
  auto fail = [&](const char* why) {
    avsd_set_error("plan_bundle_load: %s: %s", path, why);
    return AVSD_EINVAL;
  };
  if (!rd.ok || memcmp(magic, "AVSDPLN1", 8) != 0) return fail("not a plan bundle");
  if (abi != AVSD_ABI_VERSION) return fail("recorded against another ABI version of the library");
  if (strcmp(prec, AVSD_PRECISION_NAME) != 0) return fail("recorded for the other storage precision (bf16 / fp16 library)");
  const uint32_t nb = rd.get<uint32_t>();
  if (!rd.ok || nb > (1u << 20)) return fail("bad buffer table");
  b->buffers.resize(nb);
  for (Buffer& bf : b->buffers) bf.bytes = rd.get<int64_t>();
  const uint32_t nr = rd.get<uint32_t>();
  if (!rd.ok || nr > (1u << 20)) return fail("bad region table");
  b->regions.resize(nr);
  for (Region& r : b->regions) {
    r.name = rd.str();
    r.buf = rd.get<int32_t>();
    r.off = rd.get<int64_t>();
    r.bytes = rd.get<int64_t>();
    r.kind = (int)rd.get<uint32_t>();
    if (!rd.ok || r.buf < 0 || r.buf >= (int)nb || r.off < 0 || r.bytes < 0 || r.off > b->buffers[r.buf].bytes ||
        r.bytes > b->buffers[r.buf].bytes - r.off)
      return fail("a region lies outside its buffer");
  }
  const uint32_t np = rd.get<uint32_t>();
  if (!rd.ok || np > (1u << 16)) return fail("bad plan table");
  b->plans.resize(np);
  for (Plan& p : b->plans) {
    p.name = rd.str();
    const uint32_t nc = rd.get<uint32_t>();
    if (!rd.ok || nc > (1u << 20)) return fail("bad call count");
    p.calls.resize(nc);
    for (Call& c : p.calls) {
      c.fn = rd.str();
      size_t desc_bytes = 0;
      for (const Entry& e : kEntries)
        if (c.fn == e.name) { c.thunk = e.thunk; desc_bytes = e.desc_bytes; }
      if (!rd.ok || !c.thunk) return fail("a call names an entry point this library does not record");
      const uint32_t na = rd.get<uint32_t>();
      if (!rd.ok || na > 64) return fail("bad argument count");
      c.args.resize(na);
      for (Arg& a : c.args) {
        a.tag = rd.get<uint8_t>();
        if (!rd.ok) return fail("truncated file");
        if (a.tag == 'i') a.i = rd.get<int64_t>();
        else if (a.tag == 'f') a.f = rd.get<double>();
        else if (a.tag == 'p') { a.buf = rd.get<int32_t>(); a.off = rd.get<int64_t>(); }
        else if (a.tag == 'h' || a.tag == 's') {
          const uint32_t n = rd.get<uint32_t>();
          if (!rd.ok || n > (1u << 20)) return fail("bad blob");
          a.blob.resize(n);
          rd.raw(a.blob.data(), n);
          if (a.tag == 's') {
            if (n != desc_bytes) return fail("a descriptor argument does not have the size its entry point reads");
            const uint32_t nr = rd.get<uint32_t>();
            if (!rd.ok || nr > 256) return fail("bad relocation count");
            a.relocs.resize(nr);
            for (Reloc& rl : a.relocs) {
              rl.field_off = rd.get<uint32_t>(); rl.buf = rd.get<int32_t>(); rl.off = rd.get<int64_t>();
              if (!rd.ok || (size_t)rl.field_off + sizeof(void*) > (size_t)n) return fail("a descriptor relocation lies outside the descriptor");
            }
          } else if (c.fn == "avsd_guided_step" && n != 0 && n != 16) {
            return fail("avsd_guided_step history tables are 4 entries of 4 bytes");
          } else if (c.fn == "avsd_guided_multistep" && n != 0 && n != 16) {
            return fail("avsd_guided_multistep history tables are 4 entries of 4 bytes");
          }
        } else if (a.tag != 'S') return fail("unknown argument tag");
      }
    }
  }
  if (!rd.ok) return fail("truncated file");
  guard.b = nullptr;
  *out = b;
  return AVSD_OK;
}

extern "C" void avsd_plan_bundle_free(avsd_plan_bundle* b) { delete b; }

extern "C" int avsd_plan_bundle_num_buffers(const avsd_plan_bundle* b) { return b ? (int)b->buffers.size() : 0; }

extern "C" int64_t avsd_plan_bundle_buffer_bytes(const avsd_plan_bundle* b, int i) {
  return (b && i >= 0 && i < (int)b->buffers.size()) ? b->buffers[i].bytes : -1;
}

extern "C" int avsd_plan_bundle_bind(avsd_plan_bundle* b, int i, void* device_ptr) {
  AVSD_REQUIRE(b && i >= 0 && i < (int)b->buffers.size(), "plan_bundle_bind: bad index");
  AVSD_REQUIRE(device_ptr != nullptr && (uintptr_t)device_ptr % 256 == 0, "plan_bundle_bind: buffer %d needs a 256-byte-aligned device pointer", i);
  b->buffers[i].ptr = device_ptr;
  for (Plan& p : b->plans) p.resolved = false;
  return AVSD_OK;
}

extern "C" int avsd_plan_bundle_num_regions(const avsd_plan_bundle* b) { return b ? (int)b->regions.size() : 0; }

extern "C" int avsd_plan_bundle_region(const avsd_plan_bundle* b, int j, const char** name, int* buffer, int64_t* offset, int64_t* bytes,
                                       int* kind) {
  AVSD_REQUIRE(b && j >= 0 && j < (int)b->regions.size(), "plan_bundle_region: bad index");
  const Region& r = b->regions[j];
  if (name) *name = r.name.c_str();
  if (buffer) *buffer = r.buf;
  if (offset) *offset = r.off;
  if (bytes) *bytes = r.bytes;
  if (kind) *kind = r.kind;
  return AVSD_OK;
}

extern "C" int avsd_plan_bundle_find_region(const avsd_plan_bundle* b, const char* name) {
  if (!b || !name) return -1;
  for (size_t j = 0; j < b->regions.size(); ++j)
    if (b->regions[j].name == name) return (int)j;
  return -1;
}

extern "C" int avsd_plan_bundle_num_plans(const avsd_plan_bundle* b) { return b ? (int)b->plans.size() : 0; }

extern "C" const char* avsd_plan_bundle_plan_name(const avsd_plan_bundle* b, int k) {
  return (b && k >= 0 && k < (int)b->plans.size()) ? b->plans[k].name.c_str() : nullptr;
}

extern "C" int avsd_plan_bundle_find_plan(const avsd_plan_bundle* b, const char* name) {
  if (!b || !name) return -1;
// ... 103 lines not shown
```

### asva_amd/ops.py

```python
from __future__ import annotations

import os
import ctypes as C
from typing import Optional

import torch

from . import _lib
from . import precision as P
from ._lib import GemmDesc, XAttnDesc, check

PLAIN, TMIX, CONV3 = 0, 1, 2
GEGLU, OUT_F32, GELU, XCD_N, ROWSTATS, LNFUSE, RES1_F32, RES2_F32, X2, KROT, W_FRAG, OUT_REST = 1, 2, 4, 8, 16, 32, 64, 128, 256, 512, 1024, 2048
_XCD_MODE = "auto"
F32 = torch.float32


class KernelTimer:

    def __init__(self):
        self.records = []
        self.replays = []

    def start(self):
# ... 404 lines not shown
    off = rest.data_ptr() - main.data_ptr()
    if off == 0 or off % 16:
        raise ValueError("rest plane must be a distinct tensor, a multiple of 8 elements away from its main plane")
    return off // 2


def _req(t: torch.Tensor, dtype, name: str):
    if t.dtype != dtype:
        raise TypeError(f"{name}: expected {dtype}, got {t.dtype}")
    if not t.is_cuda:
        raise ValueError(f"{name}: expected a device tensor (libavsd_hip.so has no host path)")
    if t.dim() >= 1 and t.stride(-1) != 1:
        raise ValueError(f"{name}: innermost dimension must be contiguous")


def _ld(t: torch.Tensor) -> int:
    return t.stride(0) if t.dim() == 2 else t.stride(-2)


def gemm(
    a: torch.Tensor,
    w: torch.Tensor,
    *,
    n: Optional[int] = None,
    k: Optional[int] = None,
    a2: Optional[torch.Tensor] = None,
    bias: Optional[torch.Tensor] = None,
    rowvec: Optional[torch.Tensor] = None,
    rows_per_vec: int = 0,
    res1: Optional[torch.Tensor] = None,
    res2: Optional[torch.Tensor] = None,
    alpha: float = 1.0,
    geglu: bool = False,
    gelu: bool = False,
    rowstats: Optional[torch.Tensor] = None,
    ln: Optional[tuple] = None,
    stats_pos: Optional[tuple] = None,
    ln_pos: Optional[tuple] = None,
    out_f32: bool = False,
    out: Optional[torch.Tensor] = None,
    master: Optional[torch.Tensor] = None,
    mode: int = PLAIN,
    tmix: Optional[tuple] = None,
    conv: Optional[tuple] = None,
    m: Optional[int] = None,
    tile: int = 0,
    split_k: int = 1,
    a_rest: Optional[torch.Tensor] = None,
    a2_rest: Optional[torch.Tensor] = None,
    w_rest: Optional[torch.Tensor] = None,
    out_rest: Optional[torch.Tensor] = None,
    w_frag: Optional[torch.Tensor] = None,
) -> torch.Tensor:
    _req(a, P.ACT, "a")
    _req(w, P.ACT, "w")
    planes = w_rest is not None
    if planes:
        if P.SPLIT:
            raise ValueError("gemm: explicit rest planes are for the non-split modes (split precision carries them implicitly)")
        if a_rest is None or (a2 is not None) != (a2_rest is not None) or rowstats is not None or ln is not None:
            raise ValueError("gemm: a three-pass product needs a_rest and w_rest (a2_rest with a2), no rowstats / LayerNorm fold")
        if out_f32 == (out_rest is not None) or (out_f32 and master is not None):
            raise ValueError("gemm: a three-pass product writes f32 (out_f32) or a (main, rest) pair of planes (out=, out_rest=; optional f32 master)")
        if any(r is not None and r.dtype != F32 for r in (res1, res2)):
            raise ValueError("gemm: a three-pass product reads f32 residuals")
    elif a_rest is not None or a2_rest is not None:
        raise ValueError("gemm: a_rest / a2_rest without w_rest")
    if out_rest is not None and (P.SPLIT or out_f32 or geglu or out is None):
        raise ValueError("gemm: out_rest goes with an explicit 16-bit `out` outside split precision (no GEGLU)")
    x2 = P.SPLIT or planes
    if x2 and mode == PLAIN and a2 is not None and a.shape[1] % 64 != 0:
        if res1 is not None and res2 is not None:
            raise ValueError("gemm: split precision with an unaligned two-source A supports one residual")
        if gelu or geglu or rowstats is not None or ln is not None or stats_pos is not None or ln_pos is not None or (master is not None and not planes) or n is not None \
                or k is not None or m is not None or tile or split_k != 1:
            raise ValueError("gemm: split precision with an unaligned two-source A takes bias / rowvec / one residual / alpha only")
        k1 = a.shape[1]
        part = gemm(a, w[:, :k1], alpha=alpha, out_f32=True, a_rest=a_rest, w_rest=None if w_rest is None else w_rest[:, :k1])
        return gemm(a2, w[:, k1:], bias=bias, rowvec=rowvec, rows_per_vec=rows_per_vec, res1=part, res2=res1 if res1 is not None else res2,
                    alpha=alpha, out_f32=out_f32, out=out, out_rest=out_rest, master=master, a_rest=a2_rest, w_rest=None if w_rest is None else w_rest[:, k1:])
    d = GemmDesc()
    N = w.shape[0] if n is None else n
    lda = _ld(a)
    if mode == PLAIN:
        M = a.shape[0] if m is None else m
        K1 = a.shape[1]
        K = K1 + (a2.shape[1] if a2 is not None else 0)
        if a2 is not None:
            _req(a2, P.ACT, "a2")
            d.A2, d.lda2, d.k_split = _p(a2), _ld(a2), K1
        else:
            d.k_split = K
        if k is not None:
            K = k
    elif mode == TMIX:
        hw, frames = tmix
        M = a.shape[0]
        cseg = a.shape[1]
        K = 3 * cseg
        d.hw, d.frames, d.cseg = hw, frames, cseg
    elif mode == CONV3:
        n_img, hs, ws, stride, ups = conv[:5]
        pad = conv[5] if len(conv) > 5 else 1
        cin = a.shape[1]
        if a2 is not None:
            _req(a2, P.ACT, "a2")
            d.A2, d.lda2, d.k_split = _p(a2), _ld(a2), cin
            cin += a2.shape[1]
        if ups == 2:
            if stride != 1 or pad != 1 or a2 is not None or N % 4 or w.shape[1] != 4 * cin or cin % 64 or (N // 4) % 64:
                raise ValueError("gemm: ups = 2 (sub-pixel upsample convolution) needs stride 1, pad 1, one source, w [4 cout, 4 cin], cin % 64 == 0, cout % 64 == 0")
            if geglu or gelu or rowstats is not None or ln is not None or res1 is not None or res2 is not None or rowvec is not None:
                raise ValueError("gemm: ups = 2 takes bias / master / out_rest only")
            ho, wo = hs, ws
            M = n_img * hs * ws
            K = 4 * cin
        else:
            hin, win = hs << ups, ws << ups
            ho, wo = (hin + 2 - 3) // stride + 1, (win + 2 - 3) // stride + 1
            M = n_img * ho * wo
            K = 9 * cin
        d.hs, d.ws, d.ho, d.wo, d.cin, d.stride, d.ups, d.pad = hs, ws, ho, wo, cin, stride, ups, pad
    else:
        raise ValueError(f"unknown gemm mode {mode}")
    n_out = N // 2 if geglu else N
    m_out = M
    if mode == CONV3 and d.ups == 2:
        m_out, n_out = 4 * M, N // 4
    if out is None:
        out = torch.empty((m_out, n_out), dtype=F32, device=a.device) if out_f32 else alloc16((m_out, n_out), a.device)
    else:
        _req(out, F32 if out_f32 else P.ACT, "out")
        if tuple(out.shape) != (m_out, n_out) and mode == CONV3 and d.ups == 2:
# ... 105 lines not shown
        def _launch(t, sk):
            _set(t, sk)
            check(_lib.lib().avsd_gemm_bf16(C.byref(d), _stream()), "avsd_gemm_bf16")

        cands = X2_TILE_CANDIDATES if x2 else TILE_CANDIDATES
        nk = (K + 63) // 64
        two_src_unaligned = a2 is not None and (a.shape[1] % 64 != 0)
        if not geglu and not two_src_unaligned and ((M + 127) // 128) * ((N + 127) // 128) < 256 and nk >= 16:
            cands = cands + tuple(c for c in (X2_SPLITK_CANDIDATES if x2 else SPLITK_CANDIDATES) if nk // c[1] >= 4)
        splitk_ok = not geglu and not two_src_unaligned
        if mode == CONV3 and d.ups == 2:
            ok_tiles = SUBPIX_X2_TILES if x2 else SUBPIX_TILES
            cands = tuple(c for c in cands if c[0] in ok_tiles and (N // 4) % TILE_BN[c[0]] == 0)
        two_src_conv = mode == CONV3 and a2 is not None
        if two_src_conv:
            cands = conv3r_candidates(d.hs, d.ws, d.cin, M, N)
            if not cands:
                raise ValueError("gemm: no LDS-resident convolution tile takes this two-source geometry")
        elif (_CONV3R and mode == CONV3 and not x2 and d.stride == 1 and d.ups == 0 and d.pad == 1 and ln is None and out_rest is None):
            cands = cands + conv3r_candidates(d.hs, d.ws, d.cin, M, N)
        key = (mode, M, N, K, d.flags if key_flags is None else key_flags, d.stride, d.ups, d.pad, key_master)
        if mode == CONV3 and not x2:
            key = key + (d.hs, d.ws)
        if two_src_conv:
            key = key + ("a2", d.k_split)
        asm = ()
        if (_ASM_TILES and a2 is None and K % 64 == 0 and M * lda < (1 << 29) and N * _ld(w) < (1 << 29) and
                (mode == PLAIN or (mode == TMIX and d.cseg % 64 == 0 and ln is None))):
            asm = ASM_X2_CANDIDATES if x2 else tuple(c for c in ASM_CANDIDATES if mode == PLAIN or c[0] != 60)
            if splitk_ok and ((M + 127) // 128) * ((N + 127) // 128) < 256 and nk >= 8:
                asm = asm + tuple(c for c in (ASM_X2_SPLITK_CANDIDATES if x2 else ASM_SPLITK_CANDIDATES)
                                  if nk // c[1] >= 4 and (c[1] - 1) * -(-nk // c[1]) < nk)
        if RECORD_KEYS is not None:
            rec = RECORD_KEYS.setdefault(key, {"n": 0, "cands": tuple(dict.fromkeys(tuple(cands) + tuple(asm))), "flops": 2.0 * M * N * K})
            rec["n"] += 1
        picked = _pick_tile(key, _launch, cands, warm=(a, a2, res1, res2), challengers=asm)
        if picked is not None and picked[0] in ASM_TILES and not asm:
            picked = None
        if picked is not None and picked[0] in CONV3R_TILES and not ((_CONV3R or two_src_conv) and _lib.lib().avsd_gemm_conv3r_supported(picked[0], d.hs, d.ws, d.cin)):
            picked = None
        if picked is not None and picked[0] in CONV3R2D_TILES and not ((_CONV3R or two_src_conv) and _lib.lib().avsd_gemm_conv3r2d_supported(picked[0], d.hs, d.ws, d.cin)):
            picked = None
        if picked is not None and two_src_conv and picked not in cands:
            picked = None
        if picked is not None and out_rest is not None and not planes and (picked[0] in CONV3R_TILES or picked[0] in CONV3R2D_TILES):
            picked = None
        heur = _heuristic_tile_x2 if x2 else _heuristic_tile
        if picked is None and two_src_conv:
            picked = _heuristic_conv3r(cands, M, N)
        tile, split_k = picked if picked is not None else heur(M, N, K, geglu, splitk_ok)
        if mode == CONV3 and d.ups == 2:
            tile = _subpix_tile(tile, N // 4, x2)
    _set(tile, split_k)
    ev = _TIMER.start() if _TIMER is not None else None
    check(_lib.lib().avsd_gemm_bf16(C.byref(d), _stream()), "avsd_gemm_bf16")
    if ev is not None:
        fam = ("gemm_plain", "gemm_tmix", "gemm_conv3")[mode]
        dc = GemmDesc.from_buffer_copy(d)
        _TIMER.add_replay(fam, lambda dc=dc: check(_lib.lib().avsd_gemm_bf16(C.byref(dc), _stream()), "avsd_gemm_bf16"),
                          (a, a2, w, out, bias, rowvec, res1, res2, ws, rowstats, ln, master, stats_pos, ln_pos, a_rest, a2_rest, w_rest, w_frag, out_rest))
        subpix = mode == CONV3 and d.ups == 2
        _TIMER.stop(ev, fam, 2.0 * M * N * K * (3 if x2 else 1), 2.0 * M * K * (1.0 / (4 if subpix else 9) if mode == CONV3 else 1.0 / 3 if mode == TMIX else 1.0)
                    + 2.0 * N * K + _nbytes(out, res1, res2), flops_once=2.0 * M * N * K, flops_ref=2.0 * M * N * K * (2.25 if subpix else 1.0))
    return out


def gemm_f32(a: torch.Tensor, w: torch.Tensor, bias: Optional[torch.Tensor] = None) -> torch.Tensor:
    _req(a, F32, "a")
    _req(w, F32, "w")
    M, K = a.shape
    N = w.shape[0]
    out = torch.empty((M, N), dtype=F32, device=a.device)
    check(_lib.lib().avsd_gemm_f32(_p(a), _ld(a), _p(w), _ld(w), _p(bias), _p(out), _ld(out), M, N, K, _stream()), "avsd_gemm_f32")
    return out


def gemm_batched(a: torch.Tensor, w: torch.Tensor, *, alpha: float = 1.0, out_f32: bool = False,
                 bias: Optional[torch.Tensor] = None, tile: int = 0, ln: Optional[tuple] = None) -> torch.Tensor:
    _req(a, P.ACT, "a")
    _req(w, P.ACT, "w")
    B, M, K = a.shape
    N = w.shape[1]
    out = torch.empty((B, M, N), dtype=F32, device=a.device) if out_f32 else alloc16((B, M, N), a.device)
    d = GemmDesc()
    d.A, d.W, d.out = _p(a), _p(w), _p(out)
    d.M, d.N, d.K, d.k_split = M, N, K, K
    d.lda, d.ldw, d.ldc = a.stride(1), w.stride(1), out.stride(1)
    d.alpha, d.mode, d.flags, d.batch, d.tile = alpha, PLAIN, (OUT_F32 if out_f32 else 0), B, tile
    d.batch_stride_a, d.batch_stride_w, d.batch_stride_out = a.stride(0), w.stride(0), out.stride(0)
    if bias is not None:
        _req(bias, F32, "bias")
        d.bias = _p(bias)
    if ln is not None:
        st, colsum, eps = ln
        _req(st, F32, "ln stats")
        _req(colsum, F32, "ln colsum")
        d.ln_stats, d.ln_colsum, d.ln_nblk, d.ln_eps = _p(st), _p(colsum), K // 32, float(eps)
        d.flags |= LNFUSE
    if P.SPLIT:
        d.flags |= X2
        d.a_lo, d.w_lo, d.out_lo = _lo(a), _lo(w), (0 if out_f32 else _lo(out))
    if tile == 0:
        def _launch(t):
            d.tile = t
            check(_lib.lib().avsd_gemm_bf16(C.byref(d), _stream()), "avsd_gemm_bf16(batched)")

        picked = _pick_tile(("batched", B, M, N, K, d.flags), lambda t, sk: _launch(t), X2_TILE_CANDIDATES if P.SPLIT else TILE_CANDIDATES)
        d.tile = picked[0] if picked is not None else (_heuristic_tile_x2 if P.SPLIT else _heuristic_tile)(B * M, N, K, False, False)[0]
    dc = GemmDesc.from_buffer_copy(d) if _TIMER is not None else d
    _timed("gemm_plain", 2.0 * B * M * N * K * (3 if P.SPLIT else 1), 2.0 * B * (M * K + N * K) + _nbytes(out), (a, w, out, bias, ln),
           lambda: check(_lib.lib().avsd_gemm_bf16(C.byref(dc), _stream()), "avsd_gemm_bf16(batched)"))
    return out


def linear_small_m(x: torch.Tensor, w: torch.Tensor, bias: Optional[torch.Tensor], *, act_in: bool = False,
                   act_out: bool = False, out: Optional[torch.Tensor] = None) -> torch.Tensor:
    _req(x, F32, "x")
# ... 655 lines not shown
```

### asva_amd/plan.py

```python
from __future__ import annotations

import contextlib
import ctypes as C
import os
import struct
from typing import Dict, List, Optional, Tuple

import torch

from . import _lib
from . import precision as P

CONST, INPUT, OUTPUT = 1, 2, 3
MAGIC = b"AVSDPLN1"
_NOT_RECORDED = {"avsd_abi_version", "avsd_precision", "avsd_last_error", "avsd_device_info", "avsd_sizeof_gemm_desc",
                 "avsd_sizeof_xattn_desc", "avsd_cross_attention_block_supported", "avsd_groupnorm_nchunks",
                 "avsd_groupnorm_scratch_floats", "avsd_groupnorm_fused_supported", "avsd_gemm_conv3r_supported", "avsd_gemm_conv3r2d_supported"}


def _ptr_fields(struct_type) -> List[Tuple[str, int]]:
    return [(name, getattr(struct_type, name).offset) for name, tp in struct_type._fields_ if tp is C.c_void_p]


class _Proxy:

    def __init__(self, real, sink):
        self._real, self._sink = real, sink

    def __getattr__(self, name):
        fn = getattr(self._real, name)
        if (name in _NOT_RECORDED or name.startswith("avsd_plan_") or name.startswith("avsd_unet_") or name == "avsd_vae_decode"
                or name not in _lib.SIGNATURES):
            return fn
        argtypes = _lib.SIGNATURES[name][1]

        def call(*args):
            rc = fn(*args)
            if rc == 0:
                self._sink.append((name, self._convert(name, argtypes, args)))
            return rc

        return call

    @staticmethod
    def _convert(name, argtypes, args):
        out = []
        last = len(argtypes) - 1
        for k, (tp, a) in enumerate(zip(argtypes, args)):
            if tp is C.c_void_p:
                out.append(("S",) if k == last else ("p", 0 if a is None else int(a)))
            elif tp in (C.c_int, C.c_int64, C.c_int32):
                out.append(("i", int(a)))
            elif tp is C.c_float:
                out.append(("f", float(a)))
            elif isinstance(tp, type) and issubclass(tp, C._Pointer):
                target = tp._type_
                if issubclass(target, C.Structure):
                    desc = a._obj
                    relocs = [(off, int(getattr(desc, f) or 0)) for f, off in _ptr_fields(target)]
                    out.append(("s", bytes(desc), relocs))
                else:
                    out.append(("h", b"" if a is None else bytes(a)))
            else:
                raise TypeError(f"{name}: cannot record an argument of type {tp}")
        return out


class Recorder:
    def __init__(self):
        self.named: List[dict] = []
        self.plans: Dict[str, list] = {}
        self._live: Optional[list] = None

    def region(self, name: str, tensor: torch.Tensor, kind: int, data: Optional[bool] = None) -> None:
        if not tensor.is_cuda or not tensor.is_contiguous():
            raise ValueError(f"{name}: plan regions are contiguous device tensors")
        if any(b["name"] == name for b in self.named):
            raise ValueError(f"region {name} declared twice")
        self.named.append(dict(name=name, ptr=tensor.data_ptr(), bytes=tensor.numel() * tensor.element_size(), kind=kind,
                               tensor=tensor, data=(kind == CONST) if data is None else data))

    @contextlib.contextmanager
    def record(self, plan: str):
        if torch.cuda.is_current_stream_capturing():
            raise RuntimeError("record a plan eagerly, not under graph capture")
        if self._live is None:
            self._live = []
            for seg in torch.cuda.memory_snapshot():
                addr = seg["address"]
                for blk in seg["blocks"]:
                    if blk["state"] == "active_allocated":
                        self._live.append((addr, blk["size"]))
                    addr += blk["size"]
        real = _lib.lib()
        sink = self.plans.setdefault(plan, [])
        _lib._libs[P.NAME] = _Proxy(real, sink)
        try:
            yield self
        finally:
            _lib._libs[P.NAME] = real
        torch.cuda.synchronize()

    def _resolve(self):
        segs = sorted((s["address"], s["total_size"]) for s in torch.cuda.memory_snapshot())
        starts = [a for a, _ in segs]
        used: Dict[int, int] = {}
        import bisect

        def find(ptr: int) -> Tuple[int, int]:
            if ptr == 0:
                return -1, 0
            k = bisect.bisect_right(starts, ptr) - 1
# ... 144 lines not shown
```

### asva_amd/unet.py

```python
from __future__ import annotations

import inspect
import json
import math
import os
from typing import Any, Dict, Optional, Tuple, Union

import torch
from torch import nn

from . import precision as P

from . import ops
from .conditioning import mask_to_key_index
from .weights import Blob, _Pk, _Ref, from_act, pack_conv1x1, pack_device, pack_frag, pack_geglu, pack_linear, subpixel_ups, to_act, to_planes

CONFIG_NAME = "config.json"
SAFETENSORS_NAME = "diffusion_pytorch_model.safetensors"
BIN_NAME = "diffusion_pytorch_model.bin"

DOWN_TYPES = ("FFSpatioAudioTempCrossAttnDownBlock3D", "FFSpatioTempCrossAttnDownBlock3D", "FFSpatioTempResDownBlock3D")
UP_TYPES = ("FFSpatioAudioTempCrossAttnUpBlock3D", "FFSpatioTempCrossAttnUpBlock3D", "FFSpatioTempResUpBlock3D")
MID_TYPES = ("FFSpatioAudioTempCrossAttnUNetMidBlock3D", "FFSpatioTempCrossAttnUNetMidBlock3D")

# ... 794 lines not shown
                 fp8=(tuple(getattr(self, "fp8_scales", (1.0, 1.0, 1.0))) if getattr(self, "fp8_attention", _ATTN_FP8) else None))

        pre = rep if (_SHARE_PREFIX and rep > 1 and t.numel() == 1 and getattr(cond, "share", {}).get(rep, False)
                      and pk.down[0].attentions and pk.down[0].attentions[0].audio) else 1
        st.B = B // pre
        if pk.conv_in.w_r is not None:
            hm, hr = ops.ncfhw_to_rows_planes(x32, cpad=pk.conv_in.cin, rep=rep // pre)
            h = _Act(hm, None, hr)
        else:
            h = _Act(ops.ncfhw_to_rows(x32, cpad=pk.conv_in.cin, rep=rep // pre))
        hw = (H, W)
        pr = P.PLAN is not None
        h = _ffconv(st, h, pk.conv_in, hw, rest=pr)
        skips = [h]
        for i, blk in enumerate(pk.down):
            for j, r in enumerate(blk.resnets):
                h = _resblock(st, h, None, r, hw, rest=pr and not blk.attentions)
                if blk.attentions:
                    h = _transformer(st, h, blk.attentions[j], hw, st.heads[i], split=pre, rest=pr)
                    if pre > 1:
                        skips[0] = _replicate(skips[0], pre)
                        pre = 1
                skips.append(h)
            if blk.down is not None:
                h = _ffconv(st, h, blk.down, hw, stride=2, rest=pr)
                hw = (hw[0] // 2, hw[1] // 2)
                skips.append(h)
        h = _resblock(st, h, None, pk.mid.resnets[0], hw)
        h = _transformer(st, h, pk.mid.attentions[0], hw, st.heads[-1])
        h = _resblock(st, h, None, pk.mid.resnets[1], hw, rest=pr)
        rheads = st.heads[::-1]
        for i, blk in enumerate(pk.up):
            for j, r in enumerate(blk.resnets):
                h = _resblock(st, h, skips.pop(), r, hw, rest=pr and not blk.attentions)
                if blk.attentions:
                    h = _transformer(st, h, blk.attentions[j], hw, rheads[i], rest=pr)
            if blk.up is not None:
                h = _ffconv(st, h, blk.up, hw, ups=1, rest=pr)
                hw = (hw[0] * 2, hw[1] * 2)
        rows_b = Fr * hw[0] * hw[1]
        if pk.conv_out.w_r is not None:
            am, ar = ops.groupnorm_planes(*h.planes(), B, rows_b, st.groups, pk.norm_out.g, pk.norm_out.b, st.eps, True)
            a = _Act(am, None, ar)
        else:
            a = _Act(ops.groupnorm(h.lo, None, B, rows_b, st.groups, pk.norm_out.g, pk.norm_out.b, st.eps, True))
        o = _ffconv(st, a, pk.conv_out, hw, out_f32=True)
        return ops.rows_to_ncfhw(o.lo, B, self.config.out_channels, Fr, H, W)


def _master(st, like: torch.Tensor, cols: int):
    return torch.empty((like.shape[0], cols), dtype=torch.float32, device=like.device) if st.f32_stream else None


def _ffconv(st, x: _Act, p, hw, stride=1, ups=0, temb=None, res: Optional[_Act] = None, out_f32=False,
            x2: Optional[_Act] = None, master=True, rest=False) -> _Act:
    n_img = st.B * st.F
    if p.k == 3:
        ho = ((hw[0] << ups) + 2 - 3) // stride + 1
        wo = ((hw[1] << ups) + 2 - 3) // stride + 1
        rows = n_img * ho * wo
    else:
        ho, wo = hw
        rows = x.lo.shape[0]
    dev = x.lo.device
    x3, x3t = getattr(p, "w_r", None) is not None, getattr(p, "wt_r", None) is not None
    if ups and getattr(p, "subpixel", False):
        ups = 2
    ym = torch.empty((rows, p.cout), dtype=torch.float32, device=dev) if (st.f32_stream and _F32_CONV_Y) or x3 or x3t else None
    yr = None
    if x3:
        xm, xr = x.planes()
        y, yr = ops.alloc_planes((rows, p.cout), dev)
        if p.k == 3:
            ops.gemm(xm, p.w, bias=p.b, mode=ops.CONV3, conv=(n_img, hw[0], hw[1], stride, ups), out=y, out_rest=yr, master=ym, a_rest=xr, w_rest=p.w_r)
        else:
            x2m, x2r = (None, None) if x2 is None else x2.planes()
            ops.gemm(xm, p.w, a2=x2m, bias=p.b, out=y, out_rest=yr, master=ym, a_rest=xr, a2_rest=x2r, w_rest=p.w_r)
    else:
        if x3t:
            y, yr = ops.alloc_planes((rows, p.cout), dev)
        else:
            y = None
        if p.k == 3:
            y = ops.gemm(x.lo, p.w, bias=p.b, mode=ops.CONV3, conv=(n_img, hw[0], hw[1], stride, ups), master=ym, out=y, out_rest=yr)
        else:
            y = ops.gemm(x.lo, p.w, a2=None if x2 is None else x2.lo, bias=p.b, master=ym, out=y, out_rest=yr)
    if x3t:
        if res is not None and res.hi is None:
            raise RuntimeError("a three-pass temporal mix adds f32 residuals only")
        kw = dict(bias=p.bt, res1=ym, res2=None if res is None else res.hi, rowvec=temb, rows_per_vec=(st.temb_rows * ho * wo) if temb is not None else 0,
                  mode=ops.TMIX, tmix=(ho * wo, st.F), a_rest=yr, w_rest=p.wt_r)
        if out_f32:
            return _Act(ops.gemm(y, p.wt, out_f32=True, **kw))
        o16, o16r = ops.alloc_planes((rows, p.cout), dev)
        outm = torch.empty((rows, p.cout), dtype=torch.float32, device=dev) if master else None
        ops.gemm(y, p.wt, out=o16, out_rest=o16r, master=outm, **kw)
        return _Act(o16, outm, o16r)
    m = _master(st, y, p.cout) if (master and not out_f32) else None
    o16 = o16r = None
    if rest and m is not None:
        o16, o16r = ops.alloc_planes((rows, p.cout), dev)
    out = ops.gemm(y, p.wt, bias=p.bt, res1=y if ym is None else ym, res2=None if res is None else res.res, rowvec=temb,
                   rows_per_vec=(st.temb_rows * ho * wo) if temb is not None else 0,
                   mode=ops.TMIX, tmix=(ho * wo, st.F), out_f32=out_f32, master=m, out=o16, out_rest=o16r)
    return _Act(out, m, o16r)


def _resblock(st, x: _Act, skip: Optional[_Act], p, hw, rest=False) -> _Act:
    rows_b = st.F * hw[0] * hw[1]
    if p.shortcut is not None:
        s = _ffconv(st, x, p.shortcut, hw, x2=skip, out_f32=getattr(p.shortcut, "wt_r", None) is not None)
    else:
        assert skip is None
        s = x
    tv = st.temb[:, p.temb_off:p.temb_off + p.cout]
    a = ops.groupnorm(x.lo, None if skip is None else skip.lo, st.B, rows_b, st.groups, p.norm1.g, p.norm1.b, st.eps, True)
    h = _ffconv(st, _Act(a), p.conv1, hw, temb=tv, master=False)
    a2 = ops.groupnorm(h.lo, None, st.B, rows_b, st.groups, p.norm2.g, p.norm2.b, st.eps, True)
    return _ffconv(st, _Act(a2), p.conv2, hw, res=s, rest=rest)


def _transformer(st, x: _Act, p, hw, heads, split: int = 1, rest=False) -> _Act:
    B, Fr = st.B, st.F
    L = hw[0] * hw[1]
    C = p.dim
    c = st.cond.blocks[st.tr_i]
    st.tr_i += 1
    n = ops.groupnorm(x.lo, None, B * Fr, L, st.groups, p.norm.g, p.norm.b, 1e-6, False)
    fused = C % 32 == 0 and st.fuse_ln
    eps = 1e-5
    M = B * Fr * L
    stats = [torch.empty((M, C // 32, 2), dtype=torch.float32, device=n.device) for _ in range(2)] if fused else None
    si = 0

    def stream(a, w, bias, res, want_stats=True, stats_pos=None, rest=False):
        nonlocal si
        m = _master(st, a, w.shape[0])
        if fused and want_stats:
            si ^= 1
            return _Act(ops.gemm(a, w, bias=bias, res1=None if res is None else res.res, rowstats=stats[si], master=m, stats_pos=stats_pos), m)
        o16 = o16r = None
        if rest and m is not None:
            o16, o16r = ops.alloc_planes((a.shape[0], w.shape[0]), a.device)
        return _Act(ops.gemm(a, w, bias=bias, res1=None if res is None else res.res, master=m, out=o16, out_rest=o16r), m, o16r)

    def cross(h, a, norm, xa, want_stats, unfused, stats_pos=None):
        nonlocal si
        if fused and st.fp8 is None and xa is not None and ops.cross_attention_block_supported(C, heads, xa.k.shape[1], M, L):
            m = _master(st, h.lo, C)
            s_in = stats[si]
            s_out = None
            if want_stats:
                si ^= 1
                s_out = stats[si]
            out = ops.cross_attention_block(h.lo, s_in, a.wq_ln, a.sq_ln, a.bq_ln, xa.k, xa.vt, xa.lk, a.wo, a.bo, res=h.res,
                                            heads=heads, L=L, q_per_kv=xa.q_per_kv, eps=eps, rowstats=s_out, master=m, stats_pos=stats_pos)
            return _Act(out, m)
        return stream(unfused(), a.wo, a.bo, h, want_stats=want_stats, stats_pos=stats_pos)

    def proj(h, norm, wl, bl, sl, w_plain):
        if fused:
            return ops.gemm(h.lo, wl, bias=bl, ln=(stats[si], sl, eps))
# ... 66 lines not shown
```

### include/avsd.h

```cpp
#ifndef AVSD_H
#define AVSD_H

#include <stddef.h>
#include <stdint.h>

#ifdef __cplusplus
extern "C" {
#endif

#define AVSD_OK 0
#define AVSD_EINVAL (-1)
#define AVSD_ELAUNCH (-2)
#define AVSD_ENODEV (-3)

#define AVSD_ABI_VERSION 10

int avsd_abi_version(void);
const char* avsd_precision(void);
const char* avsd_last_error(void);
int avsd_device_info(char* name_host, int len, int* num_cu_host);

enum { AVSD_GEMM_PLAIN = 0, AVSD_GEMM_TMIX = 1, AVSD_GEMM_CONV3 = 2 };
enum { AVSD_GEMM_GEGLU = 1, AVSD_GEMM_OUT_F32 = 2, AVSD_GEMM_GELU = 4, AVSD_GEMM_XCD_N = 8, AVSD_GEMM_ROWSTATS = 16,
       AVSD_GEMM_LNFUSE = 32, AVSD_GEMM_RES1_F32 = 64, AVSD_GEMM_RES2_F32 = 128, AVSD_GEMM_X2 = 256, AVSD_GEMM_KROT = 512, AVSD_GEMM_W_FRAG = 1024,
       AVSD_GEMM_OUT_REST = 2048 };
#define AVSD_GEMM_MAX_TILE 33
#define AVSD_GEMM_MAX_TILE_X2 36
#define AVSD_GEMM_TILE_256x160_8W 38
#define AVSD_GEMM_TILE_ASM_FIRST 60
#define AVSD_GEMM_TILE_ASM_LAST 67
#define AVSD_GEMM_TILE_NSTREAM 70
#define AVSD_GEMM_TILE_CONV3R_FIRST 40
#define AVSD_GEMM_TILE_CONV3R_LAST 49
#define AVSD_GEMM_TILE_CONV3R2D_FIRST 51
#define AVSD_GEMM_TILE_CONV3R2D_LAST 54
typedef struct avsd_gemm_desc {
  const void* A;
  const void* A2;
  const void* W;
  void* out;
  const float* bias;
  const float* rowvec;
  const void* res1;
  const void* res2;
  int32_t M, N, K;
  int32_t lda, lda2, k_split, ldw, ldc, ldr1, ldr2;
  int32_t rows_per_vec, ldv;
  float alpha;
  int32_t mode, flags;
  int32_t batch;
  int64_t batch_stride_a, batch_stride_w, batch_stride_out;
  int32_t hw, frames, cseg;
  int32_t hs, ws, ho, wo, cin, stride, ups;
  int32_t pad;
  int32_t tile;
  int32_t split_k;
  float* splitk_ws;
  float* rowstats;
  const float* ln_stats;
  const float* ln_colsum;
  int32_t ln_nblk;
  float ln_eps;
  float* out_master;
  int32_t ldm;
  int32_t raster_g;
  int64_t a_lo, a2_lo, w_lo, out_lo, res1_lo, res2_lo;
  const float* stats_pos;
  const float* ln_rowvec;
  int32_t pos_hw, pos_frames;
} avsd_gemm_desc;

int avsd_gemm_bf16(const avsd_gemm_desc* desc_host, void* stream);
int avsd_gemm_conv3r_supported(int tile, int hs, int ws, int cin);
int avsd_gemm_conv3r2d_supported(int tile, int hs, int ws, int cin);
int avsd_sizeof_gemm_desc(void);

typedef struct avsd_xattn_desc {
  const void* h;        int32_t ldh;
  int32_t res_f32;
  const void* res;      int32_t ldres;
  int32_t M, C, heads, L;
  const float* ln_stats; float ln_eps;
  float scale;
  const void* wq;       int32_t ldwq;  int32_t lk;
  const float* q_colsum;
  const float* q_bias;
  const void* k;        const void* vt;
  int32_t lk_pad, q_per_kv;
  const void* wo;       int32_t ldwo;  int32_t ldo;
  const float* o_bias;
  void* out;
  float* out_master;    int32_t ldm;   int32_t reserved0;
  float* rowstats;
  const float* stats_pos;
  int32_t pos_hw, pos_frames;
} avsd_xattn_desc;
int avsd_cross_attention_block_supported(int C, int heads, int lk_pad);
int avsd_cross_attention_block(const avsd_xattn_desc* desc_host, void* stream);
int avsd_sizeof_xattn_desc(void);

int avsd_linear_small_m(const float* x, const void* W_bf16, const float* bias, float* out,
                        int M, int N, int K, int ldw, int act_in, int act_out, void* stream);

int avsd_groupnorm_stats(const void* x1, int ld1, int c1, const void* x2, int ld2, int c2,
                         int nb, int rows_per_batch, int groups, float* scratch, int nchunks, void* stream);
int avsd_groupnorm_apply(const void* x1, int ld1, int c1, const void* x2, int ld2, int c2,
                         int nb, int rows_per_batch, int groups, const float* gamma, const float* beta, float eps,
                         const float* scratch, int nchunks, int act, void* y, int ldy, void* stream);
int avsd_groupnorm_fused_supported(int nb, int rows_per_batch, int groups, int c1, int c2, int split);
int avsd_groupnorm_fused(const void* x1, int ld1, int c1, const void* x2, int ld2, int c2, int nb, int rows_per_batch,
                         int groups, const float* gamma, const float* beta, float eps, int act, void* y, int ldy, void* stream);
int avsd_groupnorm_nchunks(int nb, int rows_per_batch, int channels);
int avsd_groupnorm_scratch_floats(int nb, int nchunks, int groups, int channels);

int avsd_ln_fold(const float* stats, int M, int nblk, float* out, void* stream);
int avsd_layernorm(const void* x, int ldx, void* y, int ldy, int M, int C,
                   const float* gamma, const float* beta, float eps,
                   const float* pos, int hw, int frames, void* stream);

int avsd_softmax_rows(const float* S, int lds, void* P, int ldp, int rows, int L, void* stream);

int avsd_attention(const void* Q, int ldq, const void* K, int ldk, const void* V, int ldv,
                   void* O, int ldo, int Bq, int Lq, int Lk, int kv_rows, int heads, int d,
                   int q_per_kv, const int32_t* key_index, int frames, float scale, void* stream);

// ... 124 lines not shown
```

Measured before the change: 88.51 steps/s.

## Add grouped GEMM launch to run resblock shortcut and conv1 GEMMs together

Moves the gemm2 kernel body into a shared include and adds a grouped kernel that runs up to eight independent GEMM descriptors in one launch, each block finding its member from a start table. In resblocks that have a shortcut, the shortcut temporal-mix GEMM and the conv1 temporal-mix GEMM are deferred and issued as one group when their tiles and modes match. The goal is to fill the GPU better and cut launch count for small GEMMs that would otherwise run back to back. This adds member-lookup overhead and restricts grouping to a subset of tile configs, falling back to separate launches otherwise.

```diff
diff --git a/asva_amd/_lib.py b/asva_amd/_lib.py
--- a/asva_amd/_lib.py
+++ b/asva_amd/_lib.py
@@ -12,6 +12,7 @@
 LIB_PATHS = {"bf16": LIB_PATH, "fp16": os.environ.get("AVSD_LIB_PATH_F16") or os.path.join(_HERE, "libavsd_hip_f16.so")}
 
 c_void_p, c_int, c_float, c_int64 = C.c_void_p, C.c_int, C.c_float, C.c_int64
+GEMM_GROUP_MAX = 8
 
 
 class GemmDesc(C.Structure):
@@ -64,6 +65,7 @@
     "avsd_last_error": (C.c_char_p, []),
     "avsd_device_info": (c_int, [C.c_char_p, c_int, C.POINTER(c_int)]),
     "avsd_gemm_bf16": (c_int, [C.POINTER(GemmDesc), c_void_p]),
+    "avsd_gemm_group": (c_int, [C.POINTER(GemmDesc), c_int, c_void_p]),
     "avsd_sizeof_gemm_desc": (c_int, []),
     "avsd_cross_attention_block": (c_int, [C.POINTER(XAttnDesc), c_void_p]),
     "avsd_gemm_conv3r_supported": (c_int, [c_int, c_int, c_int, c_int]),
diff --git a/asva_amd/build.py b/asva_amd/build.py
--- a/asva_amd/build.py
+++ b/asva_amd/build.py
@@ -12,7 +12,7 @@
 VARIANTS = {"bf16": ("", LIB, []), "fp16": ("_f16", os.path.join(HERE, "libavsd_hip_f16.so"), ["-DAVSD_F16=1"])}
 SOURCES = ["lib.hip", "attention.hip", "attention_x2.hip", "gemm_f32.hip", "gemm4.hip", "nstream.hip", "conv3r.hip", "norm.hip", "groupnorm_fused.hip", "elementwise.hip", "audio.hip", "xattn.hip", "attention_fp8.hip", "avsync.hip", "clip_text.hip", "imagebind_eval.hip", "plan.hip"]
 GEMM_UNITS = 7
-HEADERS = [os.path.join(CSRC, "avsd_common.h"), os.path.join(CSRC, "gemm_common.h"), os.path.join(CSRC, "gemm4_loops.inc"),
+HEADERS = [os.path.join(CSRC, "avsd_common.h"), os.path.join(CSRC, "gemm_common.h"), os.path.join(CSRC, "gemm4_loops.inc"), os.path.join(CSRC, "gemm2_body.inc"),
            os.path.join(HERE, "..", "include", "avsd.h")]
 FLAGS = ["--offload-arch=gfx950", "-O3", "-std=c++17", "-fPIC", "-Wall", "-Wno-unused-function"]
 
diff --git a/asva_amd/csrc/gemm.hip b/asva_amd/csrc/gemm.hip
--- a/asva_amd/csrc/gemm.hip
+++ b/asva_amd/csrc/gemm.hip
@@ -1,3 +1,5 @@
+#include <string.h>
+
 #include "avsd_common.h"
 #include "gemm_common.h"
 
@@ -264,341 +266,21 @@
 constexpr int MODE_SUBPIX = 3;
 template <int BM, int BN, int WM, int WN, int STAGES, int MODE, int LW = 0, bool X2 = false, int EX = EPI_PLAIN>
 __global__ __launch_bounds__(64 * (WM * WN + LW), gemm2_min_waves(BM, BN, STAGES, X2, WM * WN + LW)) void gemm2_kernel(const avsd_gemm_desc p) {
-  extern __shared__ __attribute__((aligned(1024))) unsigned char smem2[];
-  constexpr int NC = WM * WN;
-  constexpr int NWAVES = LW > 0 ? LW : NC;
-  constexpr int A_BYTES = BM * 128;
-  constexpr int W_BYTES = BN * 128;
-  constexpr int PLANE_BYTES = A_BYTES + W_BYTES;
-  constexpr int STAGE_BYTES = PLANE_BYTES * (X2 ? 2 : 1);
-  constexpr int PA = (BM / 8) / NWAVES;
-  constexpr int PW = (BN / 8) / NWAVES;
-  static_assert(PA * NWAVES * 8 == BM && PW * NWAVES * 8 == BN, "tile rows must split evenly into 1-KiB pieces per wave");
-  constexpr int LPT = (PA + PW) * (X2 ? 2 : 1);
-  static_assert((STAGES - 2) * LPT < 64, "vmcnt is a 6-bit counter");
-  constexpr int FM = BM / WM / 32;
-  constexpr int FN = BN / WN / 32;
-
-  const int tid = threadIdx.x;
-  const int lane = tid & 63;
-  const int wave_all = __builtin_amdgcn_readfirstlane(tid >> 6);
-  const bool is_loader = LW == 0 || wave_all >= NC;
-  const int wave = LW == 0 ? wave_all : (wave_all >= NC ? wave_all - NC : 0);
-  const int wm = wave_all % WM;
-  const int wn = (wave_all / WM) % WN;
-
-  const int ntm = (p.M + BM - 1) / BM;
-  const int ntn = (p.N + BN - 1) / BN;
-  const int nwg = ntm * ntn;
-  const int nsplit = p.split_k > 1 ? p.split_k : 1;
-  int wg, ksplit;
-  {
-    const int total = nwg * nsplit;
-    const int bid = blockIdx.y * gridDim.x + blockIdx.x;
-    const int q = total >> 3, r = total & 7;
-    const int xcd = bid & 7, idx = bid >> 3;
-    const int c = (xcd < r ? xcd * (q + 1) : r * (q + 1) + (xcd - r) * q) + idx;
-    wg = c / nsplit;
-    ksplit = c - wg * nsplit;
-  }
-  int tm, tn;
-  tile_of_item(wg, ntm, ntn, (p.flags & AVSD_GEMM_XCD_N) != 0, p.raster_g, tm, tn);
+  const int bid = blockIdx.y * gridDim.x + blockIdx.x;
   const int64_t bz = blockIdx.z;
-  const int nk_all = (p.K + BK - 1) / BK;
-  const int per_split = (nk_all + nsplit - 1) / nsplit;
-  const int kt0 = ksplit * per_split;
-  const int kt1 = min(nk_all, kt0 + per_split);
-
-  const h16_t* Ab = reinterpret_cast<const h16_t*>(p.A) + bz * p.batch_stride_a;
-  const h16_t* A2b = p.A2 ? reinterpret_cast<const h16_t*>(p.A2) + bz * p.batch_stride_a : Ab;
-  const h16_t* Wb = reinterpret_cast<const h16_t*>(p.W) + bz * p.batch_stride_w;
-  const __amdgpu_buffer_rsrc_t rsA = __builtin_amdgcn_make_buffer_rsrc((void*)Ab, 0, 0x7fffffff, 0x00020000);
-  const __amdgpu_buffer_rsrc_t rsA2 = __builtin_amdgcn_make_buffer_rsrc((void*)A2b, 0, 0x7fffffff, 0x00020000);
-  const __amdgpu_buffer_rsrc_t rsW = __builtin_amdgcn_make_buffer_rsrc((void*)Wb, 0, 0x7fffffff, 0x00020000);
-  const __amdgpu_buffer_rsrc_t rsAr = __builtin_amdgcn_make_buffer_rsrc((void*)(Ab + (X2 ? p.a_lo : 0)), 0, 0x7fffffff, 0x00020000);
-  const __amdgpu_buffer_rsrc_t rsA2r = __builtin_amdgcn_make_buffer_rsrc((void*)(A2b + (X2 ? (p.A2 ? p.a2_lo : p.a_lo) : 0)), 0, 0x7fffffff, 0x00020000);
-  const __amdgpu_buffer_rsrc_t rsWr = __builtin_amdgcn_make_buffer_rsrc((void*)(Wb + (X2 ? p.w_lo : 0)), 0, 0x7fffffff, 0x00020000);
-
-  int ro0[PA], ro1[PA], ro2[PA], rhb[PA], rwb[PA], kca[PA];
-  bool rvalid[PA];
-#pragma unroll
-  for (int j = 0; j < PA; ++j) {
-    const int L = (wave + j * NWAVES) * 4 + (lane >> 4);
-    const int x = (lane & 15) ^ (L & 15);
-    const RowInfo32 r = make_row32<MODE>(p, tm * BM + 2 * L + (x >> 3));
-    ro0[j] = r.o0; ro1[j] = r.o1; ro2[j] = r.o2; rhb[j] = r.hb; rwb[j] = r.wb; rvalid[j] = r.valid;
-    kca[j] = (x & 7) * 8;
-  }
-  int wo[PW], kcw[PW];
-  bool wv[PW];
-#pragma unroll
-  for (int j = 0; j < PW; ++j) {
-    const int L = (wave + j * NWAVES) * 4 + (lane >> 4);
-    const int x = (lane & 15) ^ (L & 15);
-    const int n = tn * BN + 2 * L + (x >> 3);
-    wv[j] = n < p.N;
-    kcw[j] = (x & 7) * 8;
-    wo[j] = n * p.ldw + kcw[j];
-  }
-
-  const bool fast = (MODE == AVSD_GEMM_PLAIN) || (MODE == AVSD_GEMM_TMIX && p.cseg % BK == 0) ||
-                    ((MODE == AVSD_GEMM_CONV3 || MODE == MODE_SUBPIX) && p.cin % BK == 0);
-  const int nk_slice = max(kt1 - kt0, 0);
-  const int krot = ((p.flags & AVSD_GEMM_KROT) && nk_slice > 1 && ntm > 1) ? (int)(((long long)tm * nk_slice) / ntm) : 0;
-  constexpr bool subpix = MODE == MODE_SUBPIX;
-  constexpr int KS = subpix ? 2 : 3;
-  const int ush = subpix ? 0 : p.ups;
-  const int sub_par = subpix ? (tn * BN) / (p.N >> 2) : 0;
-  const int sub_dy = sub_par >> 1, sub_dx = sub_par & 1;
-  int i_kbase = 0;
-  int i_c0 = 0;
-  int i_kh = 0, i_kw = 0, i_seg = 0;
-  bool i_second = false;
-  auto seek = [&](int kbase) {
-    i_kbase = kbase;
-    if (MODE == AVSD_GEMM_PLAIN) {
-      i_c0 = i_kbase;
-      i_second = p.A2 != nullptr && i_kbase >= p.k_split;
-    } else if (MODE == AVSD_GEMM_TMIX) {
-      i_seg = i_kbase / p.cseg;
-      i_c0 = i_kbase - i_seg * p.cseg;
-    } else {
-      const int tap = i_kbase / p.cin;
-      i_c0 = i_kbase - tap * p.cin;
-      i_kh = tap / KS;
-      i_kw = tap - i_kh * KS;
-    }
-  };
-  seek((kt0 + krot) * BK);
-  const int hin = p.hs << ush, win = p.ws << ush;
-  int abase[PA];
-  bool aok[PA];
-
-  auto rebase = [&]() {
-#pragma unroll
-    for (int j = 0; j < PA; ++j) {
-      if (MODE == AVSD_GEMM_PLAIN) {
-        abase[j] = (i_second ? ro1[j] - p.k_split : ro0[j]) + kca[j];
-        aok[j] = rvalid[j];
-      } else if (MODE == AVSD_GEMM_TMIX) {
-        const int o = ro2[j] + (i_seg == 0 ? ro0[j] - ro2[j] : 0) + (i_seg == 1 ? ro1[j] - ro2[j] : 0);
-        abase[j] = o + kca[j];
-        aok[j] = rvalid[j] && i_seg < 3;
-      } else {
-        const int hi = rhb[j] + i_kh + sub_dy;
-        const int wi = rwb[j] + i_kw + sub_dx;
-        aok[j] = rvalid[j] && i_kh < KS && (unsigned)hi < (unsigned)hin && (unsigned)wi < (unsigned)win;
-        abase[j] = ((ro0[j] * p.hs + (hi >> ush)) * p.ws + (wi >> ush)) * p.lda + kca[j];
-      }
-    }
-  };
-  rebase();
-
-  auto issue = [&](int stage) {
-    unsigned char* sb = smem2 + stage * STAGE_BYTES;
-    const int kbase = i_kbase;
-#pragma unroll
-    for (int j = 0; j < PA; ++j) {
-      unsigned vo;
-      if (!fast) {
-        RowInfo32 r;
-        r.o0 = ro0[j]; r.o1 = ro1[j]; r.o2 = ro2[j]; r.hb = rhb[j]; r.wb = rwb[j]; r.valid = rvalid[j];
-        vo = a_voffset<MODE>(p, r, kbase + kca[j]);
-      } else {
-        const bool ok = aok[j] && (kbase + kca[j] < p.K);
-        vo = ok ? (unsigned)(abase[j] + i_c0) * 2u : OOB;
-      }
-      lds_ptr_t dst = (lds_ptr_t)(sb + (wave + j * NWAVES) * 1024);
-      if (i_second) __builtin_amdgcn_raw_ptr_buffer_load_lds(rsA2, dst, 16, (int)vo, 0, 0, 0);
-      else __builtin_amdgcn_raw_ptr_buffer_load_lds(rsA, dst, 16, (int)vo, 0, 0, 0);
-      if constexpr (X2) {
-        lds_ptr_t dr = (lds_ptr_t)(sb + PLANE_BYTES + (wave + j * NWAVES) * 1024);
-        if (i_second) __builtin_amdgcn_raw_ptr_buffer_load_lds(rsA2r, dr, 16, (int)vo, 0, 0, 0);
-        else __builtin_amdgcn_raw_ptr_buffer_load_lds(rsAr, dr, 16, (int)vo, 0, 0, 0);
-      }
-    }
-#pragma unroll
-    for (int j = 0; j < PW; ++j) {
-      const unsigned vo = (wv[j] && kbase + kcw[j] < p.K) ? (unsigned)(wo[j] + kbase) * 2u : OOB;
-      lds_ptr_t dst = (lds_ptr_t)(sb + A_BYTES + (wave + j * NWAVES) * 1024);
-      __builtin_amdgcn_raw_ptr_buffer_load_lds(rsW, dst, 16, (int)vo, 0, 0, 0);
-      if constexpr (X2) {
-        lds_ptr_t dr = (lds_ptr_t)(sb + PLANE_BYTES + A_BYTES + (wave + j * NWAVES) * 1024);
-        __builtin_amdgcn_raw_ptr_buffer_load_lds(rsWr, dr, 16, (int)vo, 0, 0, 0);
-      }
-    }
-    i_kbase += BK;
-    if (krot != 0 && i_kbase >= kt1 * BK) {
-      seek(kt0 * BK);
-      rebase();
-    } else
-    if (MODE == AVSD_GEMM_PLAIN) {
-      i_c0 = i_kbase;
-      if (!i_second && i_kbase >= p.k_split && i_kbase < p.K) { i_second = true; rebase(); }
-    } else if (MODE == AVSD_GEMM_TMIX) {
-      i_c0 += BK;
-      if (i_c0 >= p.cseg) { i_c0 = 0; ++i_seg; rebase(); }
-    } else {
-      i_c0 += BK;
-      if (i_c0 >= p.cin) {
-        i_c0 = 0;
-        if (++i_kw == KS) { i_kw = 0; ++i_kh; }
-        rebase();
-      }
-    }
-  };
-
-  f32x16 acc[FN][FM];
-#pragma unroll
-  for (int a = 0; a < FN; ++a)
-#pragma unroll
-    for (int b = 0; b < FM; ++b)
-#pragma unroll
-      for (int r = 0; r < 16; ++r) acc[a][b][r] = 0.f;
-
-  int a_line[FM], a_sw[FM], a_hi[FM];
-#pragma unroll
-  for (int b = 0; b < FM; ++b) {
-    const int r = wm * (BM / WM) + b * 32 + (lane & 31);
-    a_line[b] = (r >> 1) * 256;
-    a_sw[b] = (r >> 1) & 15;
-    a_hi[b] = (r & 1) << 3;
-  }
-  int w_line[FN], w_sw[FN], w_hi[FN];
-#pragma unroll
-  for (int a = 0; a < FN; ++a) {
-    const int r = wn * (BN / WN) + a * 32 + (lane & 31);
-    w_line[a] = (r >> 1) * 256;
-    w_sw[a] = (r >> 1) & 15;
-    w_hi[a] = (r & 1) << 3;
-  }
-  const int chalf = lane >> 5;
-
-  const int nk = max(kt1 - kt0, 0);
-  auto wait_stage = [&](int kt) {
-    wait_tiles_ahead<STAGES - 2, LPT>(nk - 1 - kt);
-  };
-  if (is_loader) {
-#pragma unroll
-    for (int s = 0; s < STAGES - 1; ++s)
-      if (s < nk) issue(s);
-  }
-  float pre_ln[2 * FM] = {};
-  const bool pre = (p.flags & AVSD_GEMM_LNFUSE) != 0 && !(LW > 0 && is_loader);
-  if (pre) {
-#pragma unroll
-    for (int b = 0; b < FM; ++b) {
-      const int m = tm * BM + wm * (BM / WM) + b * 32 + (lane & 31);
-      pre_ln[2 * b] = 1.f; pre_ln[2 * b + 1] = 0.f;
-      if (m < p.M) ln_row_stats(p, m, bz, pre_ln[2 * b], pre_ln[2 * b + 1]);
-    }
-  }
-  if (LW > 0 && is_loader) {
-    for (int kt = 0; kt < nk; ++kt) {
-      wait_stage(kt);
-      __builtin_amdgcn_s_barrier();
-      if (kt + STAGES - 1 < nk) issue((kt + STAGES - 1) % STAGES);
-    }
-    return;
-  }
-
-  for (int kt = 0; kt < nk; ++kt) {
-    if (LW == 0) wait_stage(kt);
-    __builtin_amdgcn_s_barrier();
-    if (LW == 0 && kt + STAGES - 1 < nk) issue((kt + STAGES - 1) % STAGES);
-
-    const unsigned char* sA = smem2 + (kt % STAGES) * STAGE_BYTES;
-    const unsigned char* sW = sA + A_BYTES;
-#pragma unroll
-    for (int ks = 0; ks < BK / 16; ++ks) {
-      const int c = ks * 2 + chalf;
-      h16x8 xf[FM], wf[FN];
-#pragma unroll
-      for (int b = 0; b < FM; ++b)
-        xf[b] = *reinterpret_cast<const h16x8*>(sA + a_line[b] + (((a_hi[b] | c) ^ a_sw[b]) << 4));
-#pragma unroll
-      for (int a = 0; a < FN; ++a)
-        wf[a] = *reinterpret_cast<const h16x8*>(sW + w_line[a] + (((w_hi[a] | c) ^ w_sw[a]) << 4));
-      if constexpr (X2) {
-        h16x8 xr[FM], wr[FN];
-#pragma unroll
-        for (int b = 0; b < FM; ++b)
-          xr[b] = *reinterpret_cast<const h16x8*>(sA + PLANE_BYTES + a_line[b] + (((a_hi[b] | c) ^ a_sw[b]) << 4));
-#pragma unroll
-        for (int a = 0; a < FN; ++a)
-          wr[a] = *reinterpret_cast<const h16x8*>(sW + PLANE_BYTES + w_line[a] + (((w_hi[a] | c) ^ w_sw[a]) << 4));
-        __builtin_amdgcn_s_setprio(1);
-#pragma unroll
-        for (int a = 0; a < FN; ++a)
-#pragma unroll
-          for (int b = 0; b < FM; ++b) {
-            acc[a][b] = mfma32x32x16(wr[a], xf[b], acc[a][b], 0, 0, 0);
-            acc[a][b] = mfma32x32x16(wf[a], xr[b], acc[a][b], 0, 0, 0);
-            acc[a][b] = mfma32x32x16(wf[a], xf[b], acc[a][b], 0, 0, 0);
-          }
-        __builtin_amdgcn_s_setprio(0);
-      } else {
-      __builtin_amdgcn_s_setprio(1);
-#pragma unroll
-      for (int a = 0; a < FN; ++a)
-#pragma unroll
-        for (int b = 0; b < FM; ++b)
-          acc[a][b] = mfma32x32x16(wf[a], xf[b], acc[a][b], 0, 0, 0);
-      __builtin_amdgcn_s_setprio(0);
-      }
-    }
-  }
-
-  if (p.split_k > 1) {
-    float* ws = p.splitk_ws + (int64_t)ksplit * p.M * p.N;
-    const int hsel = (lane >> 5) * 4;
-#pragma unroll
-    for (int b = 0; b < FM; ++b) {
-      const int m = tm * BM + wm * (BM / WM) + b * 32 + (lane & 31);
-      if (m >= p.M) continue;
-#pragma unroll
-      for (int a = 0; a < FN; ++a)
-#pragma unroll
-        for (int q = 0; q < 4; ++q) {
-          const int n = tn * BN + wn * (BN / WN) + a * 32 + 8 * q + hsel;
-          if (n < p.N)
-            *reinterpret_cast<float4*>(ws + (int64_t)m * p.N + n) =
-                make_float4(acc[a][b][4 * q], acc[a][b][4 * q + 1], acc[a][b][4 * q + 2], acc[a][b][4 * q + 3]);
-        }
-    }
-    if (p.split_k != 0x7fffffff) return;
-#pragma unroll
-    for (int a = 0; a < FN; ++a)
-#pragma unroll
-      for (int b = 0; b < FM; ++b)
-#pragma unroll
-        for (int r = 0; r < 16; ++r) acc[a][b][r] = 0.f;
-    for (int sl = 0; sl < nsplit; ++sl) {
-      const float* slab = p.splitk_ws + (int64_t)sl * p.M * p.N;
-#pragma unroll
-      for (int b = 0; b < FM; ++b) {
-        const int m = min(tm * BM + wm * (BM / WM) + b * 32 + (lane & 31), p.M - 1);
-#pragma unroll
-        for (int a = 0; a < FN; ++a)
-#pragma unroll
-          for (int q = 0; q < 4; ++q) {
-            const int n = min(tn * BN + wn * (BN / WN) + a * 32 + 8 * q + hsel, p.N - 4);
-            const float4 v = *reinterpret_cast<const float4*>(slab + (int64_t)m * p.N + n);
-            acc[a][b][4 * q] += v.x; acc[a][b][4 * q + 1] += v.y; acc[a][b][4 * q + 2] += v.z; acc[a][b][4 * q + 3] += v.w;
-          }
-      }
-    }
-  }
-  if constexpr (subpix) {
-    if constexpr (X2) epilogue_x2<FN, FM, true>(p, acc, tm * BM + wm * (BM / WM), tn * BN + wn * (BN / WN), lane, bz, pre_ln, pre);
-    else epilogue_each<FN, FM, (64 * (WM * WN + LW) > 512), EPI_SHUF>(p, acc, tm * BM + wm * (BM / WM), tn * BN + wn * (BN / WN), lane, bz, pre_ln, pre);
-  } else if constexpr (X2) epilogue_x2<FN, FM>(p, acc, tm * BM + wm * (BM / WM), tn * BN + wn * (BN / WN), lane, bz, pre_ln, pre);
-  else if constexpr (EX == EPI_REST) {
-    if constexpr (FN * FM >= 10) epilogue_each<FN, FM, (64 * (WM * WN + LW) > 512), EPI_REST>(p, acc, tm * BM + wm * (BM / WM), tn * BN + wn * (BN / WN), lane, bz, pre_ln, pre);
-    else epilogue<FN, FM, (64 * (WM * WN + LW) > 512), EPI_REST>(p, acc, tm * BM + wm * (BM / WM), tn * BN + wn * (BN / WN), lane, bz, pre_ln, pre);
-  } else if constexpr (FN * FM >= 10)
-    epilogue_each<FN, FM, (64 * (WM * WN + LW) > 512)>(p, acc, tm * BM + wm * (BM / WM), tn * BN + wn * (BN / WN), lane, bz, pre_ln, pre);
-  else epilogue<FN, FM, (64 * (WM * WN + LW) > 512)>(p, acc, tm * BM + wm * (BM / WM), tn * BN + wn * (BN / WN), lane, bz, pre_ln, pre);
+#include "gemm2_body.inc"
+}
+
+template <int BM, int BN, int WM, int WN, int STAGES, int MODE, int LW = 0>
+__global__ __launch_bounds__(64 * (WM * WN + LW), gemm2_min_waves(BM, BN, STAGES, false, WM * WN + LW)) void gemm2_group_kernel(const avsd_gemm_group_args g) {
+  const int mbr = group_member(g, (int)blockIdx.x);
+  const avsd_gemm_desc& p = g.d[mbr];
+  const int bid = (int)blockIdx.x - g.start[mbr];
+  if (bid >= group_items<BM, BN>(p)) return;
+  constexpr bool X2 = false;
+  constexpr int EX = EPI_PLAIN;
+  const int64_t bz = 0;
+#include "gemm2_body.inc"
 }
 
 template <int S, bool EXTRA = false>
@@ -770,6 +452,42 @@
   return AVSD_OK;
 }
 
+template <int BM, int BN, int WM, int WN, int STAGES, int MODE, int LW = 0>
+int launch2_group(avsd_gemm_group_args& g, hipStream_t s) {
+  constexpr size_t lds = (size_t)STAGES * (BM + BN) * 128;
+  static bool attr_set = false;
+  if (!attr_set) {
+    hipError_t e = hipFuncSetAttribute(reinterpret_cast<const void*>(&gemm2_group_kernel<BM, BN, WM, WN, STAGES, MODE, LW>),
+                                       hipFuncAttributeMaxDynamicSharedMemorySize, (int)lds);
+    if (e != hipSuccess) {
+      avsd_set_error("gemm2 group: hipFuncSetAttribute(%zu B LDS): %s", lds, hipGetErrorString(e));
+      return AVSD_ELAUNCH;
+    }
+    attr_set = true;
+  }
+  long long at = 0;
+  for (int i = 0; i < g.count; ++i) {
+    g.start[i] = (int)at;
+    at += (group_items<BM, BN>(g.d[i]) + 7) & ~7;
+    AVSD_REQUIRE(at < 2147483647LL, "gemm_group: the grid overflows (%lld blocks)", at);
+  }
+  for (int i = g.count; i <= AVSD_GEMM_GROUP_MAX; ++i) g.start[i] = (int)at;
+  hipLaunchKernelGGL((gemm2_group_kernel<BM, BN, WM, WN, STAGES, MODE, LW>), dim3((unsigned)at), dim3(64 * (WM * WN + LW)), lds, s, g);
+  AVSD_CHECK_LAUNCH("gemm2 group launch");
+  return AVSD_OK;
+}
+template <int MODE>
+int dispatch_group_tile(avsd_gemm_group_args& g, hipStream_t s) {
+  switch (g.d[0].tile) {
+    case 7: return launch2_group<64, 64, 2, 2, 4, MODE>(g, s);
+    case 13: return launch2_group<64, 64, 2, 2, 2, MODE>(g, s);
+    case 25: return launch2_group<64, 64, 2, 2, 4, MODE, 2>(g, s);
+    default:
+      avsd_set_error("gemm_group: tile %d has no grouped form (7, 13, 25, 63..66 do)", g.d[0].tile);
+      return AVSD_EINVAL;
+  }
+}
+
 template <int MODE, int EX = EPI_PLAIN>
 int dispatch_tile(const avsd_gemm_desc& d, int tile, hipStream_t s) {
   switch (tile) {
@@ -848,6 +566,14 @@
 #else
 #define AVSD_DISPATCH_TILE(MODE) dispatch_tile<MODE>(d, tile, s)
 #endif
+int avsd_gemm_group_dispatch_plain(avsd_gemm_group_args& g, hipStream_t s);
+int avsd_gemm_group_dispatch_tmix(avsd_gemm_group_args& g, hipStream_t s);
+#if !defined(AVSD_GEMM_TU) || AVSD_GEMM_TU == 0
+int avsd_gemm_group_dispatch_plain(avsd_gemm_group_args& g, hipStream_t s) { return dispatch_group_tile<AVSD_GEMM_PLAIN>(g, s); }
+#endif
+#if !defined(AVSD_GEMM_TU) || AVSD_GEMM_TU == 1
+int avsd_gemm_group_dispatch_tmix(avsd_gemm_group_args& g, hipStream_t s) { return dispatch_group_tile<AVSD_GEMM_TMIX>(g, s); }
+#endif
 #if !defined(AVSD_GEMM_TU) || AVSD_GEMM_TU == 0
 int avsd_gemm_dispatch_plain(const avsd_gemm_desc& d, int tile, hipStream_t s) { return AVSD_DISPATCH_TILE(AVSD_GEMM_PLAIN); }
 #endif
@@ -930,9 +656,7 @@
   return AVSD_OK;
 }
 
-extern "C" int avsd_gemm_bf16(const avsd_gemm_desc* dp, void* stream) {
-  AVSD_REQUIRE(dp != nullptr, "gemm: null descriptor");
-  avsd_gemm_desc d = *dp;
+static int gemm_check_desc(avsd_gemm_desc& d) {
   AVSD_REQUIRE(d.A && d.W && d.out, "gemm: A, W and out must be non-null");
   AVSD_REQUIRE(d.M > 0 && d.N > 0 && d.K > 0, "gemm: M,N,K must be positive (got %d,%d,%d)", d.M, d.N, d.K);
   AVSD_REQUIRE(!(d.flags & AVSD_GEMM_W_FRAG) || d.tile == AVSD_GEMM_TILE_NSTREAM, "gemm: fragment-ordered W (AVSD_GEMM_W_FRAG) is read by tile %d only (got %d)", AVSD_GEMM_TILE_NSTREAM, d.tile);
@@ -1006,6 +730,16 @@
   } else {
     AVSD_REQUIRE(false, "gemm: unknown mode %d", d.mode);
   }
+  return AVSD_OK;
+}
+
+extern "C" int avsd_gemm_bf16(const avsd_gemm_desc* dp, void* stream) {
+  AVSD_REQUIRE(dp != nullptr, "gemm: null descriptor");
+  avsd_gemm_desc d = *dp;
+  {
+    const int rc = gemm_check_desc(d);
+    if (rc != AVSD_OK) return rc;
+  }
   if ((d.tile >= AVSD_GEMM_TILE_CONV3R_FIRST && d.tile <= AVSD_GEMM_TILE_CONV3R_LAST) ||
       (d.tile >= AVSD_GEMM_TILE_CONV3R2D_FIRST && d.tile <= AVSD_GEMM_TILE_CONV3R2D_LAST)) {
     if (d.split_k > 1) AVSD_REQUIRE(d.splitk_ws != nullptr, "gemm: split_k needs a workspace");
@@ -1060,4 +794,49 @@
     default: return d.ups == 2 ? avsd_gemm_dispatch_subpix(d, tile, s) : avsd_gemm_dispatch_conv3(d, tile, s);
   }
 }
-#endif
+
+int avsd_gemm_group_dispatch_asm(avsd_gemm_group_args& g, hipStream_t s);
+
+extern "C" int avsd_gemm_group(const avsd_gemm_desc* descs, int count, void* stream) {
+  AVSD_REQUIRE(descs != nullptr, "gemm_group: null descriptor array");
+  AVSD_REQUIRE(count >= 1 && count <= AVSD_GEMM_GROUP_MAX, "gemm_group: 1..%d members (got %d)", AVSD_GEMM_GROUP_MAX, count);
+  avsd_gemm_group_args g;
+  memset(&g, 0, sizeof(g));
+  g.count = count;
+  for (int i = 0; i < count; ++i) {
+    avsd_gemm_desc& d = g.d[i];
+    d = descs[i];
+    const int rc = gemm_check_desc(d);
+    if (rc != AVSD_OK) return rc;
+    AVSD_REQUIRE(d.mode == AVSD_GEMM_PLAIN || d.mode == AVSD_GEMM_TMIX, "gemm_group: member %d: PLAIN or TMIX products only (mode %d)", i, d.mode);
+    AVSD_REQUIRE(!d.A2 && d.batch == 1 && d.K % 64 == 0, "gemm_group: member %d: one source, no batching, K %% 64 == 0 (got K %d, batch %d)", i, d.K, d.batch);
+    AVSD_REQUIRE(!(d.flags & (AVSD_GEMM_X2 | AVSD_GEMM_OUT_REST | AVSD_GEMM_W_FRAG)), "gemm_group: member %d: one-pass products without a rest plane only (flags %#x)", i, d.flags);
+    AVSD_REQUIRE(d.mode != AVSD_GEMM_TMIX || d.cseg % 64 == 0, "gemm_group: member %d: TMIX needs cseg %% 64 == 0 (got %d)", i, d.cseg);
+    AVSD_REQUIRE(d.tile == g.d[0].tile && d.mode == g.d[0].mode && (d.split_k > 1 ? d.split_k : 1) == (g.d[0].split_k > 1 ? g.d[0].split_k : 1),
+                 "gemm_group: member %d differs from member 0 in tile (%d / %d), mode (%d / %d) or split_k (%d / %d)", i, d.tile, g.d[0].tile, d.mode,
+                 g.d[0].mode, d.split_k, g.d[0].split_k);
+    const bool asm_tile = d.tile >= AVSD_GEMM_TILE_ASM_FIRST && d.tile <= AVSD_GEMM_TILE_ASM_LAST;
+    AVSD_REQUIRE((asm_tile && d.tile >= AVSD_GEMM_TILE_ASM_FIRST + 3 && d.tile <= AVSD_GEMM_TILE_ASM_FIRST + 6) || d.tile == 7 || d.tile == 13 || d.tile == 25,
+                 "gemm_group: tile %d has no grouped form (7, 13, 25, 63..66 do)", d.tile);
+    AVSD_REQUIRE((double)d.M * d.lda * 2.0 < 1073741824.0 && (double)d.N * d.ldw * 2.0 < 1073741824.0, "gemm_group: member %d: operands must be < 1 GiB", i);
+    AVSD_REQUIRE(!(asm_tile && d.mode == AVSD_GEMM_TMIX && (d.flags & AVSD_GEMM_LNFUSE)), "gemm_group: member %d: no LNFUSE on a TMIX asm tile", i);
+    if (d.split_k > 1) {
+      const int nk_all = d.K / 64, per = (nk_all + d.split_k - 1) / d.split_k;
+      AVSD_REQUIRE(d.splitk_ws && d.split_k <= nk_all && !(d.flags & AVSD_GEMM_GEGLU), "gemm_group: member %d: bad split_k %d (workspace, <= K tiles, no GEGLU)", i, d.split_k);
+      AVSD_REQUIRE((d.split_k - 1) * per < nk_all, "gemm_group: member %d: split_k %d leaves an empty slice of the %d K tiles", i, d.split_k, nk_all);
+    }
+    AVSD_REQUIRE((double)((d.M + 63) / 64) * ((d.N + 63) / 64) * (d.split_k > 1 ? d.split_k : 1) < 2147483647.0, "gemm_group: member %d: the grid overflows", i);
+  }
+  hipStream_t s = reinterpret_cast<hipStream_t>(stream);
+  const bool asm_tile = g.d[0].tile >= AVSD_GEMM_TILE_ASM_FIRST;
+  const int rc = asm_tile ? avsd_gemm_group_dispatch_asm(g, s)
+                          : (g.d[0].mode == AVSD_GEMM_TMIX ? avsd_gemm_group_dispatch_tmix(g, s) : avsd_gemm_group_dispatch_plain(g, s));
+  if (rc != AVSD_OK) return rc;
+  if (g.d[0].split_k > 1)
+    for (int i = 0; i < count; ++i) {
+      const int r2 = avsd_gemm_splitk_reduce(g.d[i], s);
+      if (r2 != AVSD_OK) return r2;
+    }
+  return AVSD_OK;
+}
+#endif
diff --git a/asva_amd/csrc/gemm2_body.inc b/asva_amd/csrc/gemm2_body.inc
--- /dev/null
+++ b/asva_amd/csrc/gemm2_body.inc
@@ -0,0 +1,333 @@
+  extern __shared__ __attribute__((aligned(1024))) unsigned char smem2[];
+  constexpr int NC = WM * WN;
+  constexpr int NWAVES = LW > 0 ? LW : NC;
+  constexpr int A_BYTES = BM * 128;
+  constexpr int W_BYTES = BN * 128;
+  constexpr int PLANE_BYTES = A_BYTES + W_BYTES;
+  constexpr int STAGE_BYTES = PLANE_BYTES * (X2 ? 2 : 1);
+  constexpr int PA = (BM / 8) / NWAVES;
+  constexpr int PW = (BN / 8) / NWAVES;
+  static_assert(PA * NWAVES * 8 == BM && PW * NWAVES * 8 == BN, "tile rows must split evenly into 1-KiB pieces per wave");
+  constexpr int LPT = (PA + PW) * (X2 ? 2 : 1);
+  static_assert((STAGES - 2) * LPT < 64, "vmcnt is a 6-bit counter");
+  constexpr int FM = BM / WM / 32;
+  constexpr int FN = BN / WN / 32;
+
+  const int tid = threadIdx.x;
+  const int lane = tid & 63;
+  const int wave_all = __builtin_amdgcn_readfirstlane(tid >> 6);
+  const bool is_loader = LW == 0 || wave_all >= NC;
+  const int wave = LW == 0 ? wave_all : (wave_all >= NC ? wave_all - NC : 0);
+  const int wm = wave_all % WM;
+  const int wn = (wave_all / WM) % WN;
+
+  const int ntm = (p.M + BM - 1) / BM;
+  const int ntn = (p.N + BN - 1) / BN;
+  const int nwg = ntm * ntn;
+  const int nsplit = p.split_k > 1 ? p.split_k : 1;
+  int wg, ksplit;
+  {
+    const int total = nwg * nsplit;
+    const int q = total >> 3, r = total & 7;
+    const int xcd = bid & 7, idx = bid >> 3;
+    const int c = (xcd < r ? xcd * (q + 1) : r * (q + 1) + (xcd - r) * q) + idx;
+    wg = c / nsplit;
+    ksplit = c - wg * nsplit;
+  }
+  int tm, tn;
+  tile_of_item(wg, ntm, ntn, (p.flags & AVSD_GEMM_XCD_N) != 0, p.raster_g, tm, tn);
+  const int nk_all = (p.K + BK - 1) / BK;
+  const int per_split = (nk_all + nsplit - 1) / nsplit;
+  const int kt0 = ksplit * per_split;
+  const int kt1 = min(nk_all, kt0 + per_split);
+
+  const h16_t* Ab = reinterpret_cast<const h16_t*>(p.A) + bz * p.batch_stride_a;
+  const h16_t* A2b = p.A2 ? reinterpret_cast<const h16_t*>(p.A2) + bz * p.batch_stride_a : Ab;
+  const h16_t* Wb = reinterpret_cast<const h16_t*>(p.W) + bz * p.batch_stride_w;
+  const __amdgpu_buffer_rsrc_t rsA = __builtin_amdgcn_make_buffer_rsrc((void*)Ab, 0, 0x7fffffff, 0x00020000);
+  const __amdgpu_buffer_rsrc_t rsA2 = __builtin_amdgcn_make_buffer_rsrc((void*)A2b, 0, 0x7fffffff, 0x00020000);
+  const __amdgpu_buffer_rsrc_t rsW = __builtin_amdgcn_make_buffer_rsrc((void*)Wb, 0, 0x7fffffff, 0x00020000);
+  const __amdgpu_buffer_rsrc_t rsAr = __builtin_amdgcn_make_buffer_rsrc((void*)(Ab + (X2 ? p.a_lo : 0)), 0, 0x7fffffff, 0x00020000);
+  const __amdgpu_buffer_rsrc_t rsA2r = __builtin_amdgcn_make_buffer_rsrc((void*)(A2b + (X2 ? (p.A2 ? p.a2_lo : p.a_lo) : 0)), 0, 0x7fffffff, 0x00020000);
+  const __amdgpu_buffer_rsrc_t rsWr = __builtin_amdgcn_make_buffer_rsrc((void*)(Wb + (X2 ? p.w_lo : 0)), 0, 0x7fffffff, 0x00020000);
+
+  int ro0[PA], ro1[PA], ro2[PA], rhb[PA], rwb[PA], kca[PA];
+  bool rvalid[PA];
+#pragma unroll
+  for (int j = 0; j < PA; ++j) {
+    const int L = (wave + j * NWAVES) * 4 + (lane >> 4);
+    const int x = (lane & 15) ^ (L & 15);
+    const RowInfo32 r = make_row32<MODE>(p, tm * BM + 2 * L + (x >> 3));
+    ro0[j] = r.o0; ro1[j] = r.o1; ro2[j] = r.o2; rhb[j] = r.hb; rwb[j] = r.wb; rvalid[j] = r.valid;
+    kca[j] = (x & 7) * 8;
+  }
+  int wo[PW], kcw[PW];
+  bool wv[PW];
+#pragma unroll
+  for (int j = 0; j < PW; ++j) {
+    const int L = (wave + j * NWAVES) * 4 + (lane >> 4);
+    const int x = (lane & 15) ^ (L & 15);
+    const int n = tn * BN + 2 * L + (x >> 3);
+    wv[j] = n < p.N;
+    kcw[j] = (x & 7) * 8;
+    wo[j] = n * p.ldw + kcw[j];
+  }
+
+  const bool fast = (MODE == AVSD_GEMM_PLAIN) || (MODE == AVSD_GEMM_TMIX && p.cseg % BK == 0) ||
+                    ((MODE == AVSD_GEMM_CONV3 || MODE == MODE_SUBPIX) && p.cin % BK == 0);
+  const int nk_slice = max(kt1 - kt0, 0);
+  const int krot = ((p.flags & AVSD_GEMM_KROT) && nk_slice > 1 && ntm > 1) ? (int)(((long long)tm * nk_slice) / ntm) : 0;
+  constexpr bool subpix = MODE == MODE_SUBPIX;
+  constexpr int KS = subpix ? 2 : 3;
+  const int ush = subpix ? 0 : p.ups;
+  const int sub_par = subpix ? (tn * BN) / (p.N >> 2) : 0;
+  const int sub_dy = sub_par >> 1, sub_dx = sub_par & 1;
+  int i_kbase = 0;
+  int i_c0 = 0;
+  int i_kh = 0, i_kw = 0, i_seg = 0;
+  bool i_second = false;
+  auto seek = [&](int kbase) {
+    i_kbase = kbase;
+    if (MODE == AVSD_GEMM_PLAIN) {
+      i_c0 = i_kbase;
+      i_second = p.A2 != nullptr && i_kbase >= p.k_split;
+    } else if (MODE == AVSD_GEMM_TMIX) {
+      i_seg = i_kbase / p.cseg;
+      i_c0 = i_kbase - i_seg * p.cseg;
+    } else {
+      const int tap = i_kbase / p.cin;
+      i_c0 = i_kbase - tap * p.cin;
+      i_kh = tap / KS;
+      i_kw = tap - i_kh * KS;
+    }
+  };
+  seek((kt0 + krot) * BK);
+  const int hin = p.hs << ush, win = p.ws << ush;
+  int abase[PA];
+  bool aok[PA];
+
+  auto rebase = [&]() {
+#pragma unroll
+    for (int j = 0; j < PA; ++j) {
+      if (MODE == AVSD_GEMM_PLAIN) {
+        abase[j] = (i_second ? ro1[j] - p.k_split : ro0[j]) + kca[j];
+        aok[j] = rvalid[j];
+      } else if (MODE == AVSD_GEMM_TMIX) {
+        const int o = ro2[j] + (i_seg == 0 ? ro0[j] - ro2[j] : 0) + (i_seg == 1 ? ro1[j] - ro2[j] : 0);
+        abase[j] = o + kca[j];
+        aok[j] = rvalid[j] && i_seg < 3;
+      } else {
+        const int hi = rhb[j] + i_kh + sub_dy;
+        const int wi = rwb[j] + i_kw + sub_dx;
+        aok[j] = rvalid[j] && i_kh < KS && (unsigned)hi < (unsigned)hin && (unsigned)wi < (unsigned)win;
+        abase[j] = ((ro0[j] * p.hs + (hi >> ush)) * p.ws + (wi >> ush)) * p.lda + kca[j];
+      }
+    }
+  };
+  rebase();
+
+  auto issue = [&](int stage) {
+    unsigned char* sb = smem2 + stage * STAGE_BYTES;
+    const int kbase = i_kbase;
+#pragma unroll
+    for (int j = 0; j < PA; ++j) {
+      unsigned vo;
+      if (!fast) {
+        RowInfo32 r;
+        r.o0 = ro0[j]; r.o1 = ro1[j]; r.o2 = ro2[j]; r.hb = rhb[j]; r.wb = rwb[j]; r.valid = rvalid[j];
+        vo = a_voffset<MODE>(p, r, kbase + kca[j]);
+      } else {
+        const bool ok = aok[j] && (kbase + kca[j] < p.K);
+        vo = ok ? (unsigned)(abase[j] + i_c0) * 2u : OOB;
+      }
+      lds_ptr_t dst = (lds_ptr_t)(sb + (wave + j * NWAVES) * 1024);
+      if (i_second) __builtin_amdgcn_raw_ptr_buffer_load_lds(rsA2, dst, 16, (int)vo, 0, 0, 0);
+      else __builtin_amdgcn_raw_ptr_buffer_load_lds(rsA, dst, 16, (int)vo, 0, 0, 0);
+      if constexpr (X2) {
+        lds_ptr_t dr = (lds_ptr_t)(sb + PLANE_BYTES + (wave + j * NWAVES) * 1024);
+        if (i_second) __builtin_amdgcn_raw_ptr_buffer_load_lds(rsA2r, dr, 16, (int)vo, 0, 0, 0);
+        else __builtin_amdgcn_raw_ptr_buffer_load_lds(rsAr, dr, 16, (int)vo, 0, 0, 0);
+      }
+    }
+#pragma unroll
+    for (int j = 0; j < PW; ++j) {
+      const unsigned vo = (wv[j] && kbase + kcw[j] < p.K) ? (unsigned)(wo[j] + kbase) * 2u : OOB;
+      lds_ptr_t dst = (lds_ptr_t)(sb + A_BYTES + (wave + j * NWAVES) * 1024);
+      __builtin_amdgcn_raw_ptr_buffer_load_lds(rsW, dst, 16, (int)vo, 0, 0, 0);
+      if constexpr (X2) {
+        lds_ptr_t dr = (lds_ptr_t)(sb + PLANE_BYTES + A_BYTES + (wave + j * NWAVES) * 1024);
+        __builtin_amdgcn_raw_ptr_buffer_load_lds(rsWr, dr, 16, (int)vo, 0, 0, 0);
+      }
+    }
+    i_kbase += BK;
+    if (krot != 0 && i_kbase >= kt1 * BK) {
+      seek(kt0 * BK);
+      rebase();
+    } else
+    if (MODE == AVSD_GEMM_PLAIN) {
+      i_c0 = i_kbase;
+      if (!i_second && i_kbase >= p.k_split && i_kbase < p.K) { i_second = true; rebase(); }
+    } else if (MODE == AVSD_GEMM_TMIX) {
+      i_c0 += BK;
+      if (i_c0 >= p.cseg) { i_c0 = 0; ++i_seg; rebase(); }
+    } else {
+      i_c0 += BK;
+      if (i_c0 >= p.cin) {
+        i_c0 = 0;
+        if (++i_kw == KS) { i_kw = 0; ++i_kh; }
+        rebase();
+      }
+    }
+  };
+
+  f32x16 acc[FN][FM];
+#pragma unroll
+  for (int a = 0; a < FN; ++a)
+#pragma unroll
+    for (int b = 0; b < FM; ++b)
+#pragma unroll
+      for (int r = 0; r < 16; ++r) acc[a][b][r] = 0.f;
+
+  int a_line[FM], a_sw[FM], a_hi[FM];
+#pragma unroll
+  for (int b = 0; b < FM; ++b) {
+    const int r = wm * (BM / WM) + b * 32 + (lane & 31);
+    a_line[b] = (r >> 1) * 256;
+    a_sw[b] = (r >> 1) & 15;
+    a_hi[b] = (r & 1) << 3;
+  }
+  int w_line[FN], w_sw[FN], w_hi[FN];
+#pragma unroll
+  for (int a = 0; a < FN; ++a) {
+    const int r = wn * (BN / WN) + a * 32 + (lane & 31);
+    w_line[a] = (r >> 1) * 256;
+    w_sw[a] = (r >> 1) & 15;
+    w_hi[a] = (r & 1) << 3;
+  }
+  const int chalf = lane >> 5;
+
+  const int nk = max(kt1 - kt0, 0);
+  auto wait_stage = [&](int kt) {
+    wait_tiles_ahead<STAGES - 2, LPT>(nk - 1 - kt);
+  };
+  if (is_loader) {
+#pragma unroll
+    for (int s = 0; s < STAGES - 1; ++s)
+      if (s < nk) issue(s);
+  }
+  float pre_ln[2 * FM] = {};
+  const bool pre = (p.flags & AVSD_GEMM_LNFUSE) != 0 && !(LW > 0 && is_loader);
+  if (pre) {
+#pragma unroll
+    for (int b = 0; b < FM; ++b) {
+      const int m = tm * BM + wm * (BM / WM) + b * 32 + (lane & 31);
+      pre_ln[2 * b] = 1.f; pre_ln[2 * b + 1] = 0.f;
+      if (m < p.M) ln_row_stats(p, m, bz, pre_ln[2 * b], pre_ln[2 * b + 1]);
+    }
+  }
+  if (LW > 0 && is_loader) {
+    for (int kt = 0; kt < nk; ++kt) {
+      wait_stage(kt);
+      __builtin_amdgcn_s_barrier();
+      if (kt + STAGES - 1 < nk) issue((kt + STAGES - 1) % STAGES);
+    }
+    return;
+  }
+
+  for (int kt = 0; kt < nk; ++kt) {
+    if (LW == 0) wait_stage(kt);
+    __builtin_amdgcn_s_barrier();
+    if (LW == 0 && kt + STAGES - 1 < nk) issue((kt + STAGES - 1) % STAGES);
+
+    const unsigned char* sA = smem2 + (kt % STAGES) * STAGE_BYTES;
+    const unsigned char* sW = sA + A_BYTES;
+#pragma unroll
+    for (int ks = 0; ks < BK / 16; ++ks) {
+      const int c = ks * 2 + chalf;
+      h16x8 xf[FM], wf[FN];
+#pragma unroll
+      for (int b = 0; b < FM; ++b)
+        xf[b] = *reinterpret_cast<const h16x8*>(sA + a_line[b] + (((a_hi[b] | c) ^ a_sw[b]) << 4));
+#pragma unroll
+      for (int a = 0; a < FN; ++a)
+        wf[a] = *reinterpret_cast<const h16x8*>(sW + w_line[a] + (((w_hi[a] | c) ^ w_sw[a]) << 4));
+      if constexpr (X2) {
+        h16x8 xr[FM], wr[FN];
+#pragma unroll
+        for (int b = 0; b < FM; ++b)
+          xr[b] = *reinterpret_cast<const h16x8*>(sA + PLANE_BYTES + a_line[b] + (((a_hi[b] | c) ^ a_sw[b]) << 4));
+#pragma unroll
+        for (int a = 0; a < FN; ++a)
+          wr[a] = *reinterpret_cast<const h16x8*>(sW + PLANE_BYTES + w_line[a] + (((w_hi[a] | c) ^ w_sw[a]) << 4));
+        __builtin_amdgcn_s_setprio(1);
+#pragma unroll
+        for (int a = 0; a < FN; ++a)
+#pragma unroll
+          for (int b = 0; b < FM; ++b) {
+            acc[a][b] = mfma32x32x16(wr[a], xf[b], acc[a][b], 0, 0, 0);
+            acc[a][b] = mfma32x32x16(wf[a], xr[b], acc[a][b], 0, 0, 0);
+            acc[a][b] = mfma32x32x16(wf[a], xf[b], acc[a][b], 0, 0, 0);
+          }
+        __builtin_amdgcn_s_setprio(0);
+      } else {
+      __builtin_amdgcn_s_setprio(1);
+#pragma unroll
+      for (int a = 0; a < FN; ++a)
+#pragma unroll
+        for (int b = 0; b < FM; ++b)
+          acc[a][b] = mfma32x32x16(wf[a], xf[b], acc[a][b], 0, 0, 0);
+      __builtin_amdgcn_s_setprio(0);
+      }
+    }
+  }
+
+  if (p.split_k > 1) {
+    float* ws = p.splitk_ws + (int64_t)ksplit * p.M * p.N;
+    const int hsel = (lane >> 5) * 4;
+#pragma unroll
+    for (int b = 0; b < FM; ++b) {
+      const int m = tm * BM + wm * (BM / WM) + b * 32 + (lane & 31);
+      if (m >= p.M) continue;
+#pragma unroll
+      for (int a = 0; a < FN; ++a)
+#pragma unroll
+        for (int q = 0; q < 4; ++q) {
+          const int n = tn * BN + wn * (BN / WN) + a * 32 + 8 * q + hsel;
+          if (n < p.N)
+            *reinterpret_cast<float4*>(ws + (int64_t)m * p.N + n) =
+                make_float4(acc[a][b][4 * q], acc[a][b][4 * q + 1], acc[a][b][4 * q + 2], acc[a][b][4 * q + 3]);
+        }
+    }
+    if (p.split_k != 0x7fffffff) return;
+#pragma unroll
+    for (int a = 0; a < FN; ++a)
+#pragma unroll
+      for (int b = 0; b < FM; ++b)
+#pragma unroll
+        for (int r = 0; r < 16; ++r) acc[a][b][r] = 0.f;
+    for (int sl = 0; sl < nsplit; ++sl) {
+      const float* slab = p.splitk_ws + (int64_t)sl * p.M * p.N;
+#pragma unroll
+      for (int b = 0; b < FM; ++b) {
+        const int m = min(tm * BM + wm * (BM / WM) + b * 32 + (lane & 31), p.M - 1);
+#pragma unroll
+        for (int a = 0; a < FN; ++a)
+#pragma unroll
+          for (int q = 0; q < 4; ++q) {
+            const int n = min(tn * BN + wn * (BN / WN) + a * 32 + 8 * q + hsel, p.N - 4);
+            const float4 v = *reinterpret_cast<const float4*>(slab + (int64_t)m * p.N + n);
+            acc[a][b][4 * q] += v.x; acc[a][b][4 * q + 1] += v.y; acc[a][b][4 * q + 2] += v.z; acc[a][b][4 * q + 3] += v.w;
+          }
+      }
+    }
+  }
+  if constexpr (subpix) {
+    if constexpr (X2) epilogue_x2<FN, FM, true>(p, acc, tm * BM + wm * (BM / WM), tn * BN + wn * (BN / WN), lane, bz, pre_ln, pre);
+    else epilogue_each<FN, FM, (64 * (WM * WN + LW) > 512), EPI_SHUF>(p, acc, tm * BM + wm * (BM / WM), tn * BN + wn * (BN / WN), lane, bz, pre_ln, pre);
+  } else if constexpr (X2) epilogue_x2<FN, FM>(p, acc, tm * BM + wm * (BM / WM), tn * BN + wn * (BN / WN), lane, bz, pre_ln, pre);
+  else if constexpr (EX == EPI_REST) {
+    if constexpr (FN * FM >= 10) epilogue_each<FN, FM, (64 * (WM * WN + LW) > 512), EPI_REST>(p, acc, tm * BM + wm * (BM / WM), tn * BN + wn * (BN / WN), lane, bz, pre_ln, pre);
+    else epilogue<FN, FM, (64 * (WM * WN + LW) > 512), EPI_REST>(p, acc, tm * BM + wm * (BM / WM), tn * BN + wn * (BN / WN), lane, bz, pre_ln, pre);
+  } else if constexpr (FN * FM >= 10)
+    epilogue_each<FN, FM, (64 * (WM * WN + LW) > 512)>(p, acc, tm * BM + wm * (BM / WM), tn * BN + wn * (BN / WN), lane, bz, pre_ln, pre);
+  else epilogue<FN, FM, (64 * (WM * WN + LW) > 512)>(p, acc, tm * BM + wm * (BM / WM), tn * BN + wn * (BN / WN), lane, bz, pre_ln, pre);
diff --git a/asva_amd/csrc/gemm4.hip b/asva_amd/csrc/gemm4.hip
--- a/asva_amd/csrc/gemm4.hip
+++ b/asva_amd/csrc/gemm4.hip
@@ -29,8 +29,8 @@
   return v;
 }
 
-template <int FM, int FN, int MODE, bool X2 = false, int NS = 2, int EX = EPI_PLAIN>
-__global__ __launch_bounds__(256, 1) void gemm4_kernel(const avsd_gemm_desc p) {
+template <int FM, int FN, int MODE, bool X2, int NS, int EX>
+__device__ __forceinline__ void gemm4_body(const avsd_gemm_desc& p, const int bid) {
   extern __shared__ __attribute__((aligned(1024))) unsigned char smem4[];
   constexpr int BM = 64 * FM, BN = 64 * FN;
   constexpr int A_BYTES = BM * ROWB;
@@ -50,7 +50,6 @@
   int wg, ksplit;
   {
     const int total = nwg * nsplit;
-    const int bid = blockIdx.y * gridDim.x + blockIdx.x;
     const int q = total >> 3, r = total & 7;
     const int xcd = bid & 7, idx = bid >> 3;
     const int c = (xcd < r ? xcd * (q + 1) : r * (q + 1) + (xcd - r) * q) + idx;
@@ -167,6 +166,37 @@
 }
 
 template <int FM, int FN, int MODE, bool X2 = false, int NS = 2, int EX = EPI_PLAIN>
+__global__ __launch_bounds__(256, 1) void gemm4_kernel(const avsd_gemm_desc p) {
+  gemm4_body<FM, FN, MODE, X2, NS, EX>(p, blockIdx.y * gridDim.x + blockIdx.x);
+}
+
+template <int FM, int FN, int MODE>
+__global__ __launch_bounds__(256, 1) void gemm4_group_kernel(const avsd_gemm_group_args g) {
+  const int mbr = group_member(g, (int)blockIdx.x);
+  const avsd_gemm_desc& p = g.d[mbr];
+  const int bid = (int)blockIdx.x - g.start[mbr];
+  if (bid >= group_items<64 * FM, 64 * FN>(p)) return;
+  gemm4_body<FM, FN, MODE, false, 2, EPI_PLAIN>(p, bid);
+}
+
+template <int FM, int FN, int MODE>
+int launch4_group(const avsd_gemm_group_args& g, hipStream_t s) {
+  constexpr size_t lds = (size_t)2 * (64 * FM + 64 * FN) * ROWB;
+  static bool attr_set = false;
+  if (!attr_set) {
+    hipError_t e = hipFuncSetAttribute(reinterpret_cast<const void*>(&gemm4_group_kernel<FM, FN, MODE>), hipFuncAttributeMaxDynamicSharedMemorySize, (int)lds);
+    if (e != hipSuccess) {
+      avsd_set_error("gemm4 group: hipFuncSetAttribute(%zu B LDS): %s", lds, hipGetErrorString(e));
+      return AVSD_ELAUNCH;
+    }
+    attr_set = true;
+  }
+  hipLaunchKernelGGL((gemm4_group_kernel<FM, FN, MODE>), dim3((unsigned)g.start[g.count]), dim3(256), lds, s, g);
+  AVSD_CHECK_LAUNCH("gemm4 group launch");
+  return AVSD_OK;
+}
+
+template <int FM, int FN, int MODE, bool X2 = false, int NS = 2, int EX = EPI_PLAIN>
 int launch4_ex(const avsd_gemm_desc& d, hipStream_t s) {
   constexpr int BM = 64 * FM, BN = 64 * FN;
   constexpr size_t lds = (size_t)2 * (BM + BN) * ROWB * (X2 ? 2 : 1);
@@ -245,3 +275,25 @@
     default: AVSD_REQUIRE(false, "gemm/asm tiles: unknown tile %d", d.tile);
   }
 }
+
+template <int FM, int FN>
+static int group4(avsd_gemm_group_args& g, bool tmix, hipStream_t s) {
+  long long at = 0;
+  for (int i = 0; i < g.count; ++i) {
+    g.start[i] = (int)at;
+    at += (group_items<64 * FM, 64 * FN>(g.d[i]) + 7) & ~7;
+    AVSD_REQUIRE(at < 2147483647LL, "gemm_group: the grid overflows (%lld blocks)", at);
+  }
+  for (int i = g.count; i <= AVSD_GEMM_GROUP_MAX; ++i) g.start[i] = (int)at;
+  return tmix ? launch4_group<FM, FN, AVSD_GEMM_TMIX>(g, s) : launch4_group<FM, FN, AVSD_GEMM_PLAIN>(g, s);
+}
+int avsd_gemm_group_dispatch_asm(avsd_gemm_group_args& g, hipStream_t s) {
+  const bool tmix = g.d[0].mode == AVSD_GEMM_TMIX;
+  switch (g.d[0].tile - AVSD_GEMM_TILE_ASM_FIRST) {
+    case 3: return group4<2, 2>(g, tmix, s);
+    case 4: return group4<2, 1>(g, tmix, s);
+    case 5: return group4<1, 2>(g, tmix, s);
+    case 6: return group4<1, 1>(g, tmix, s);
+    default: AVSD_REQUIRE(false, "gemm_group: asm tile %d has no grouped form (63..66 do)", g.d[0].tile);
+  }
+}
diff --git a/asva_amd/csrc/gemm_common.h b/asva_amd/csrc/gemm_common.h
--- a/asva_amd/csrc/gemm_common.h
+++ b/asva_amd/csrc/gemm_common.h
@@ -2,6 +2,13 @@
 #include <utility>
 
 #include "avsd_common.h"
+
+struct avsd_gemm_group_args {
+  avsd_gemm_desc d[AVSD_GEMM_GROUP_MAX];
+  int start[AVSD_GEMM_GROUP_MAX + 1];
+  int count;
+};
+static_assert(sizeof(avsd_gemm_group_args) <= 4096, "the argument block of a grouped launch must fit HIP's 4 KB");
 
 namespace {
 
@@ -760,6 +767,16 @@
   tm = nmaj ? tmin : tmaj;
 }
 
+__device__ __forceinline__ int group_member(const avsd_gemm_group_args& g, int block) {
+  int mbr = 0;
+#pragma unroll
+  for (int i = 1; i < AVSD_GEMM_GROUP_MAX; ++i) mbr += (i < g.count && block >= g.start[i]) ? 1 : 0;
+  return __builtin_amdgcn_readfirstlane(mbr);
+}
+template <int BM, int BN>
+__host__ __device__ __forceinline__ int group_items(const avsd_gemm_desc& p) {
+  return ((p.M + BM - 1) / BM) * ((p.N + BN - 1) / BN) * (p.split_k > 1 ? p.split_k : 1);
+}
 
 __device__ __forceinline__ void piece_row_chunk(int piece, int lane, int& row, int& kchunk) {
   const int L = piece * 4 + (lane >> 4);
diff --git a/asva_amd/csrc/plan.hip b/asva_amd/csrc/plan.hip
--- a/asva_amd/csrc/plan.hip
+++ b/asva_amd/csrc/plan.hip
@@ -40,11 +40,13 @@
   const char* name;
   thunk_t thunk;
   size_t desc_bytes;
-};
-#define AVSD_PLAN_ENTRY(fn) {#fn, [](const RArg* a, int n) { return call(&fn, a, n, #fn); }, 0}
-#define AVSD_PLAN_ENTRY_DESC(fn, T) {#fn, [](const RArg* a, int n) { return call(&fn, a, n, #fn); }, sizeof(T)}
+  int desc_max;
+};
+#define AVSD_PLAN_ENTRY(fn) {#fn, [](const RArg* a, int n) { return call(&fn, a, n, #fn); }, 0, 0}
+#define AVSD_PLAN_ENTRY_DESC(fn, T, MAXN) {#fn, [](const RArg* a, int n) { return call(&fn, a, n, #fn); }, sizeof(T), MAXN}
 const Entry kEntries[] = {
-    AVSD_PLAN_ENTRY_DESC(avsd_gemm_bf16, avsd_gemm_desc), AVSD_PLAN_ENTRY_DESC(avsd_cross_attention_block, avsd_xattn_desc), AVSD_PLAN_ENTRY(avsd_linear_small_m),
+    AVSD_PLAN_ENTRY_DESC(avsd_gemm_bf16, avsd_gemm_desc, 1), AVSD_PLAN_ENTRY_DESC(avsd_gemm_group, avsd_gemm_desc, AVSD_GEMM_GROUP_MAX),
+    AVSD_PLAN_ENTRY_DESC(avsd_cross_attention_block, avsd_xattn_desc, 1), AVSD_PLAN_ENTRY(avsd_linear_small_m),
     AVSD_PLAN_ENTRY(avsd_groupnorm_stats),  AVSD_PLAN_ENTRY(avsd_groupnorm_apply),       AVSD_PLAN_ENTRY(avsd_layernorm),
     AVSD_PLAN_ENTRY(avsd_softmax_rows),     AVSD_PLAN_ENTRY(avsd_attention),             AVSD_PLAN_ENTRY(avsd_attention_fp8),
     AVSD_PLAN_ENTRY(avsd_temporal_attention), AVSD_PLAN_ENTRY(avsd_ncfhw_to_rows),       AVSD_PLAN_ENTRY(avsd_rows_to_ncfhw),
@@ -245,8 +247,9 @@
     for (Call& c : p.calls) {
       c.fn = rd.str();
       size_t desc_bytes = 0;
+      int desc_max = 0;
       for (const Entry& e : kEntries)
-        if (c.fn == e.name) { c.thunk = e.thunk; desc_bytes = e.desc_bytes; }
+        if (c.fn == e.name) { c.thunk = e.thunk; desc_bytes = e.desc_bytes; desc_max = e.desc_max; }
       if (!rd.ok || !c.thunk) return fail("a call names an entry point this library does not record");
       const uint32_t na = rd.get<uint32_t>();
       if (!rd.ok || na > 64) return fail("bad argument count");
@@ -263,7 +266,8 @@
           a.blob.resize(n);
           rd.raw(a.blob.data(), n);
           if (a.tag == 's') {
-            if (n != desc_bytes) return fail("a descriptor argument does not have the size its entry point reads");
+            if (desc_bytes == 0 || n == 0 || n % desc_bytes != 0 || n / desc_bytes > (size_t)(desc_max > 1 ? desc_max : 1))
+              return fail("a descriptor argument does not have the size its entry point reads");
             const uint32_t nr = rd.get<uint32_t>();
             if (!rd.ok || nr > 256) return fail("bad relocation count");
             a.relocs.resize(nr);
@@ -278,6 +282,10 @@
           }
         } else if (a.tag != 'S') return fail("unknown argument tag");
       }
+      if (desc_max > 1) {
+        if (na < 2 || c.args[0].tag != 's' || c.args[1].tag != 'i' || c.args[1].i != (int64_t)(c.args[0].blob.size() / desc_bytes))
+          return fail("a descriptor array and its count disagree");
+      }
     }
   }
   if (!rd.ok) return fail("truncated file");
diff --git a/asva_amd/ops.py b/asva_amd/ops.py
--- a/asva_amd/ops.py
+++ b/asva_amd/ops.py
@@ -480,6 +480,73 @@
     out_rest: Optional[torch.Tensor] = None,
     w_frag: Optional[torch.Tensor] = None,
 ) -> torch.Tensor:
+    return _gemm_launch(_gemm_prepare(a, w, n=n, k=k, a2=a2, bias=bias, rowvec=rowvec, rows_per_vec=rows_per_vec, res1=res1, res2=res2, alpha=alpha, geglu=geglu, gelu=gelu, rowstats=rowstats, ln=ln, stats_pos=stats_pos, ln_pos=ln_pos, out_f32=out_f32, out=out, master=master, mode=mode, tmix=tmix, conv=conv, m=m, tile=tile, split_k=split_k, a_rest=a_rest, a2_rest=a2_rest, w_rest=w_rest, out_rest=out_rest, w_frag=w_frag))
+
+
+class _GemmCall:
+    __slots__ = ("d", "out", "M", "N", "K", "mode", "x2", "keep", "res")
+
+    def __init__(self, d, out, M=0, N=0, K=0, mode=0, x2=False, keep=(), res=()):
+        self.d, self.out, self.M, self.N, self.K, self.mode, self.x2, self.keep, self.res = d, out, M, N, K, mode, x2, keep, res
+
+    def family(self):
+        return ("gemm_plain", "gemm_tmix", "gemm_conv3")[self.mode]
+
+    def flops_bytes(self):
+        M, N, K, mode = self.M, self.N, self.K, self.mode
+        subpix = mode == CONV3 and self.d.ups == 2
+        once = 2.0 * M * N * K
+        nb = 2.0 * M * K * (1.0 / (4 if subpix else 9) if mode == CONV3 else 1.0 / 3 if mode == TMIX else 1.0) + 2.0 * N * K + _nbytes(self.out, *self.res)
+        return once * (3 if self.x2 else 1), nb, once, once * (2.25 if subpix else 1.0)
+
+
+def _gemm_launch(c: "_GemmCall") -> torch.Tensor:
+    if c.d is None:
+        return c.out
+    ev = _TIMER.start() if _TIMER is not None else None
+    check(_lib.lib().avsd_gemm_bf16(C.byref(c.d), _stream()), "avsd_gemm_bf16")
+    if ev is not None:
+        dc = GemmDesc.from_buffer_copy(c.d)
+        _TIMER.add_replay(c.family(), lambda dc=dc: check(_lib.lib().avsd_gemm_bf16(C.byref(dc), _stream()), "avsd_gemm_bf16"), c.keep)
+        fl, nb, once, ref = c.flops_bytes()
+        _TIMER.stop(ev, c.family(), fl, nb, flops_once=once, flops_ref=ref)
+    return c.out
+
+
+def _gemm_prepare(
+    a: torch.Tensor,
+    w: torch.Tensor,
+    *,
+    n: Optional[int] = None,
+    k: Optional[int] = None,
+    a2: Optional[torch.Tensor] = None,
+    bias: Optional[torch.Tensor] = None,
+    rowvec: Optional[torch.Tensor] = None,
+    rows_per_vec: int = 0,
+    res1: Optional[torch.Tensor] = None,
+    res2: Optional[torch.Tensor] = None,
+    alpha: float = 1.0,
+    geglu: bool = False,
+    gelu: bool = False,
+    rowstats: Optional[torch.Tensor] = None,
+    ln: Optional[tuple] = None,
+    stats_pos: Optional[tuple] = None,
+    ln_pos: Optional[tuple] = None,
+    out_f32: bool = False,
+    out: Optional[torch.Tensor] = None,
+    master: Optional[torch.Tensor] = None,
+    mode: int = PLAIN,
+    tmix: Optional[tuple] = None,
+    conv: Optional[tuple] = None,
+    m: Optional[int] = None,
+    tile: int = 0,
+    split_k: int = 1,
+    a_rest: Optional[torch.Tensor] = None,
+    a2_rest: Optional[torch.Tensor] = None,
+    w_rest: Optional[torch.Tensor] = None,
+    out_rest: Optional[torch.Tensor] = None,
+    w_frag: Optional[torch.Tensor] = None,
+) -> "_GemmCall":
     _req(a, P.ACT, "a")
     _req(w, P.ACT, "w")
     planes = w_rest is not None
@@ -505,8 +572,9 @@
             raise ValueError("gemm: split precision with an unaligned two-source A takes bias / rowvec / one residual / alpha only")
         k1 = a.shape[1]
         part = gemm(a, w[:, :k1], alpha=alpha, out_f32=True, a_rest=a_rest, w_rest=None if w_rest is None else w_rest[:, :k1])
-        return gemm(a2, w[:, k1:], bias=bias, rowvec=rowvec, rows_per_vec=rows_per_vec, res1=part, res2=res1 if res1 is not None else res2,
-                    alpha=alpha, out_f32=out_f32, out=out, out_rest=out_rest, master=master, a_rest=a2_rest, w_rest=None if w_rest is None else w_rest[:, k1:])
+        return _GemmCall(None, gemm(a2, w[:, k1:], bias=bias, rowvec=rowvec, rows_per_vec=rows_per_vec, res1=part, res2=res1 if res1 is not None else res2,
+                                    alpha=alpha, out_f32=out_f32, out=out, out_rest=out_rest, master=master, a_rest=a2_rest,
+                                    w_rest=None if w_rest is None else w_rest[:, k1:]))
     d = GemmDesc()
     N = w.shape[0] if n is None else n
     lda = _ld(a)
@@ -718,17 +786,51 @@
         if mode == CONV3 and d.ups == 2:
             tile = _subpix_tile(tile, N // 4, x2)
     _set(tile, split_k)
+    return _GemmCall(d, out, M, N, K, mode, x2, (a, a2, w, out, bias, rowvec, res1, res2, ws, rowstats, ln, master, stats_pos, ln_pos, a_rest, a2_rest, w_rest,
+                                                  w_frag, out_rest), (res1, res2))
+
+
+GROUP_MAX = _lib.GEMM_GROUP_MAX
+GROUP_TILES = (7, 13, 25, 63, 64, 65, 66)
+
+
+def _groupable(c: "_GemmCall") -> bool:
+    d = c.d
+    return (d is not None and d.tile in GROUP_TILES and c.mode in (PLAIN, TMIX) and not d.A2 and c.K % 64 == 0 and (c.mode != TMIX or d.cseg % 64 == 0)
+            and not (d.flags & (X2 | OUT_REST | W_FRAG)) and not (c.mode == TMIX and d.tile >= 60 and (d.flags & LNFUSE))
+            and 2 * c.M * d.lda < (1 << 30) and 2 * c.N * d.ldw < (1 << 30))
+
+
+def gemm_group(calls, dependents=None) -> list:
+    prepared = [_gemm_prepare(**kw) for kw in calls]
+    if dependents is not None and all(_groupable(c) and c.d.split_k <= 1 for c in prepared):
+        for kw in dependents():
+            kw = dict(kw)
+            lead, krot = prepared[kw.pop("tile_of")], kw.pop("krot", True)
+            c = _gemm_prepare(tile=lead.d.tile, split_k=1, **kw)
+            if not krot:
+                c.d.flags &= ~KROT
+            prepared.append(c)
+    d0 = prepared[0].d if prepared else None
+    same = 2 <= len(prepared) <= GROUP_MAX and all(
+        _groupable(c) and c.d.tile == d0.tile and c.d.mode == d0.mode and max(c.d.split_k, 1) == max(d0.split_k, 1) for c in prepared)
+    if not same:
+        return [_gemm_launch(c) for c in prepared]
+    arr = (GemmDesc * len(prepared))()
+    for i, c in enumerate(prepared):
+        arr[i] = c.d
+
+    def launch(arr=arr):
+        check(_lib.lib().avsd_gemm_group(arr, len(arr), _stream()), "avsd_gemm_group")
+
     ev = _TIMER.start() if _TIMER is not None else None
-    check(_lib.lib().avsd_gemm_bf16(C.byref(d), _stream()), "avsd_gemm_bf16")
+    launch()
     if ev is not None:
-        fam = ("gemm_plain", "gemm_tmix", "gemm_conv3")[mode]
-        dc = GemmDesc.from_buffer_copy(d)
-        _TIMER.add_replay(fam, lambda dc=dc: check(_lib.lib().avsd_gemm_bf16(C.byref(dc), _stream()), "avsd_gemm_bf16"),
-                          (a, a2, w, out, bias, rowvec, res1, res2, ws, rowstats, ln, master, stats_pos, ln_pos, a_rest, a2_rest, w_rest, w_frag, out_rest))
-        subpix = mode == CONV3 and d.ups == 2
-        _TIMER.stop(ev, fam, 2.0 * M * N * K * (3 if x2 else 1), 2.0 * M * K * (1.0 / (4 if subpix else 9) if mode == CONV3 else 1.0 / 3 if mode == TMIX else 1.0)
-                    + 2.0 * N * K + _nbytes(out, res1, res2), flops_once=2.0 * M * N * K, flops_ref=2.0 * M * N * K * (2.25 if subpix else 1.0))
-    return out
+        fam = prepared[0].family()
+        _TIMER.add_replay(fam, launch, tuple(c.keep for c in prepared))
+        tot = [sum(v) for v in zip(*(c.flops_bytes() for c in prepared))]
+        _TIMER.stop(ev, fam, tot[0], tot[1], flops_once=tot[2], flops_ref=tot[3])
+    return [c.out for c in prepared]
 
 
 def gemm_f32(a: torch.Tensor, w: torch.Tensor, bias: Optional[torch.Tensor] = None) -> torch.Tensor:
diff --git a/asva_amd/plan.py b/asva_amd/plan.py
--- a/asva_amd/plan.py
+++ b/asva_amd/plan.py
@@ -56,8 +56,9 @@
             elif isinstance(tp, type) and issubclass(tp, C._Pointer):
                 target = tp._type_
                 if issubclass(target, C.Structure):
-                    desc = a._obj
-                    relocs = [(off, int(getattr(desc, f) or 0)) for f, off in _ptr_fields(target)]
+                    desc = a if isinstance(a, C.Array) else a._obj
+                    members = list(desc) if isinstance(desc, C.Array) else [desc]
+                    relocs = [(i * C.sizeof(target) + off, int(getattr(d, f) or 0)) for i, d in enumerate(members) for f, off in _ptr_fields(target)]
                     out.append(("s", bytes(desc), relocs))
                 else:
                     out.append(("h", b"" if a is None else bytes(a)))
diff --git a/asva_amd/unet.py b/asva_amd/unet.py
--- a/asva_amd/unet.py
+++ b/asva_amd/unet.py
@@ -870,8 +870,15 @@
     return torch.empty((like.shape[0], cols), dtype=torch.float32, device=like.device) if st.f32_stream else None
 
 
+def _gemm_group(site: str):
+    fn = getattr(ops, "gemm_group", None)
+    if fn is None or P.SPLIT or os.environ.get("AVSD_GEMM_GROUP", "all") not in ("all", site):
+        return None
+    return fn
+
+
 def _ffconv(st, x: _Act, p, hw, stride=1, ups=0, temb=None, res: Optional[_Act] = None, out_f32=False,
-            x2: Optional[_Act] = None, master=True, rest=False) -> _Act:
+            x2: Optional[_Act] = None, master=True, rest=False, defer=False):
     n_img = st.B * st.F
     if p.k == 3:
         ho = ((hw[0] << ups) + 2 - 3) // stride + 1
@@ -904,6 +911,8 @@
         else:
             y = ops.gemm(x.lo, p.w, a2=None if x2 is None else x2.lo, bias=p.b, master=ym, out=y, out_rest=yr)
     if x3t:
+        if defer:
+            raise RuntimeError("a three-pass temporal mix cannot be deferred")
         if res is not None and res.hi is None:
             raise RuntimeError("a three-pass temporal mix adds f32 residuals only")
         kw = dict(bias=p.bt, res1=ym, res2=None if res is None else res.hi, rowvec=temb, rows_per_vec=(st.temb_rows * ho * wo) if temb is not None else 0,
@@ -918,14 +927,26 @@
     o16 = o16r = None
     if rest and m is not None:
         o16, o16r = ops.alloc_planes((rows, p.cout), dev)
-    out = ops.gemm(y, p.wt, bias=p.bt, res1=y if ym is None else ym, res2=None if res is None else res.res, rowvec=temb,
-                   rows_per_vec=(st.temb_rows * ho * wo) if temb is not None else 0,
-                   mode=ops.TMIX, tmix=(ho * wo, st.F), out_f32=out_f32, master=m, out=o16, out_rest=o16r)
-    return _Act(out, m, o16r)
+    kw = dict(bias=p.bt, res1=y if ym is None else ym, res2=None if res is None else res.res, rowvec=temb,
+              rows_per_vec=(st.temb_rows * ho * wo) if temb is not None else 0,
+              mode=ops.TMIX, tmix=(ho * wo, st.F), out_f32=out_f32, master=m, out=o16, out_rest=o16r)
+    if defer:
+        return dict(a=y, w=p.wt, **kw), lambda out: _Act(out, m, o16r)
+    return _Act(ops.gemm(y, p.wt, **kw), m, o16r)
 
 
 def _resblock(st, x: _Act, skip: Optional[_Act], p, hw, rest=False) -> _Act:
     rows_b = st.F * hw[0] * hw[1]
+    group = _gemm_group("tmix") if p.shortcut is not None else None
+    if group is not None and not any(getattr(q, nm, None) is not None for q in (p.shortcut, p.conv1) for nm in ("w_r", "wt_r")):
+        s_kw, s_fin = _ffconv(st, x, p.shortcut, hw, x2=skip, defer=True)
+        tv = st.temb[:, p.temb_off:p.temb_off + p.cout]
+        a = ops.groupnorm(x.lo, None if skip is None else skip.lo, st.B, rows_b, st.groups, p.norm1.g, p.norm1.b, st.eps, True)
+        h_kw, h_fin = _ffconv(st, _Act(a), p.conv1, hw, temb=tv, master=False, defer=True)
+        s_out, h_out = group([s_kw, h_kw])
+        s, h = s_fin(s_out), h_fin(h_out)
+        a2 = ops.groupnorm(h.lo, None, st.B, rows_b, st.groups, p.norm2.g, p.norm2.b, st.eps, True)
+        return _ffconv(st, _Act(a2), p.conv2, hw, res=s, rest=rest)
     if p.shortcut is not None:
         s = _ffconv(st, x, p.shortcut, hw, x2=skip, out_f32=getattr(p.shortcut, "wt_r", None) is not None)
     else:
diff --git a/include/avsd.h b/include/avsd.h
--- a/include/avsd.h
+++ b/include/avsd.h
@@ -71,6 +71,8 @@
 } avsd_gemm_desc;
 
 int avsd_gemm_bf16(const avsd_gemm_desc* desc_host, void* stream);
+#define AVSD_GEMM_GROUP_MAX 8
+int avsd_gemm_group(const avsd_gemm_desc* descs_host, int count, void* stream);
 int avsd_gemm_conv3r_supported(int tile, int hs, int ws, int cin);
 int avsd_gemm_conv3r2d_supported(int tile, int hs, int ws, int cin);
 int avsd_sizeof_gemm_desc(void);
```

After: 89.31 steps/s, median of 6. Within noise of the previous version (+0.9%).
